# doubleailes/crust-render

Measured on AMD Instinct MI355X. Metric: Mray/s (closest-hit + shadow queries) of the path-tracing integrator, higher is better.
Workload: dtype f32; 1 GPU; samples/cornellbox.usda 1920x1080, 512 spp per step per GPU-share (x1 GPUs), depth 32, triangle r=1, variance 0; 14 steps = 7168 spp; rays_total=33550217735, closest_hit=33550217735, camera_rays=14863564800, target_spp=1024

## Files before the change

crust-render_amd/__init__.py:

```python
import ctypes as C
import os
import subprocess

import numpy as np

_HERE = os.path.dirname(os.path.abspath(__file__))
LIB_PATH = os.environ.get("CRT_AMD_LIB") or os.path.join(_HERE, "libcrt_amd.so")
CSRC = os.path.join(_HERE, "csrc")

MASK_CAMERA, MASK_SHADOW, MASK_INDIRECT, MASK_ALL = 1, 2, 4, 0xFFFFFFFF
INVALID_ID = 0xFFFFFFFF
INF = float("inf")

CRT_OK = 0
_ERRORS = {-1: "CRT_ERR_BAD_ARG", -2: "CRT_ERR_BAD_ID", -3: "CRT_ERR_NO_DEVICE", -4: "CRT_ERR_STACK",
           -5: "CRT_ERR_UNSUPPORTED", -6: "CRT_ERR_NO_MEMORY"}


class CrtError(RuntimeError):
    def __init__(self, code, what=""):
        detail = ""
        try:
            detail = _lib.crt_last_error().decode() if _lib is not None else ""
        except Exception:
            pass
        super().__init__(f"{what}: {_ERRORS.get(code, code)}" + (f" [{detail}]" if detail else ""))
        self.code = code


def build_native(force=False):
    if force:
        subprocess.check_call(["make", "-C", CSRC, "clean"], stdout=subprocess.DEVNULL)
    subprocess.check_call(["make", "-C", CSRC, "-j8", "-s"])
    return LIB_PATH


class CrtRay(C.Structure):
    _fields_ = [("origin", C.c_float * 3), ("_pad0", C.c_float), ("dir", C.c_float * 3), ("_pad1", C.c_float),
                ("time", C.c_float), ("mask", C.c_uint32), ("_pad2", C.c_uint32 * 2)]


class CrtRayHit(C.Structure):
    _fields_ = [("t", C.c_float), ("normal", C.c_float * 3), ("front_face", C.c_uint32), ("u", C.c_float),
                ("v", C.c_float), ("geom_id", C.c_uint32), ("prim_id", C.c_uint32), ("_pad", C.c_uint32)]


class CrtTravStats(C.Structure):
    _fields_ = [("queries", C.c_uint64 * 2), ("nodes", C.c_uint64 * 2), ("leaves", C.c_uint64 * 2),
                ("packets", C.c_uint64 * 2), ("prims", C.c_uint64 * 2), ("accepted_hits", C.c_uint64),
                ("instance_descents", C.c_uint64), ("rays", C.c_uint64),
                ("phase_waves", C.c_uint64 * 8), ("phase_lanes", C.c_uint64 * 8),
                ("phase_cycles", C.c_uint64 * 8)]

    PHASES = ("loop", "fetch+setup", "node", "packet", "scalar prim", "instance exit", "emit", "f64 fallback")

    def utilisation(self):
        return {n: (int(self.phase_waves[k]), (self.phase_lanes[k] / (64.0 * self.phase_waves[k])) if self.phase_waves[k] else 0.0)
                for k, n in enumerate(self.PHASES)}

    def as_dict(self):
        d = {k: [int(getattr(self, k)[0]), int(getattr(self, k)[1])] for k in ("queries", "nodes", "leaves", "packets",
                                                                                "prims")}
        d.update(accepted_hits=int(self.accepted_hits), instance_descents=int(self.instance_descents),
                 rays=int(self.rays))
        return d

    def algorithmic_bytes(self):
        n = sum
        return (80 * int(self.rays) + 128 * n(self.nodes) + 16 * n(self.leaves) + 192 * n(self.packets) +
                128 * int(self.accepted_hits) + 112 * int(self.instance_descents))


_MAT_FIELDS = [
    ("kind", C.c_uint32), ("thin_walled", C.c_uint32),
    ("base_weight", C.c_float), ("base_color", C.c_float * 3), ("base_diffuse_roughness", C.c_float),
    ("base_metalness", C.c_float),
    ("specular_weight", C.c_float), ("specular_color", C.c_float * 3), ("specular_roughness", C.c_float),
    ("specular_ior", C.c_float), ("specular_roughness_anisotropy", C.c_float),
    ("transmission_weight", C.c_float), ("transmission_color", C.c_float * 3), ("transmission_depth", C.c_float),
    ("transmission_scatter", C.c_float * 3), ("transmission_scatter_anisotropy", C.c_float),
    ("transmission_dispersion_scale", C.c_float), ("transmission_dispersion_abbe_number", C.c_float),
    ("subsurface_weight", C.c_float), ("subsurface_color", C.c_float * 3), ("subsurface_radius", C.c_float),
    ("subsurface_radius_scale", C.c_float * 3), ("subsurface_scatter_anisotropy", C.c_float),
    ("fuzz_weight", C.c_float), ("fuzz_color", C.c_float * 3), ("fuzz_roughness", C.c_float),
    ("coat_weight", C.c_float), ("coat_color", C.c_float * 3), ("coat_roughness", C.c_float),
    ("coat_roughness_anisotropy", C.c_float), ("coat_ior", C.c_float), ("coat_darkening", C.c_float),
    ("thin_film_weight", C.c_float), ("thin_film_thickness", C.c_float), ("thin_film_ior", C.c_float),
    ("emission_luminance", C.c_float), ("emission_color", C.c_float * 3),
    ("geometry_opacity", C.c_float),
]


class CrtMaterial(C.Structure):
    _fields_ = _MAT_FIELDS


MAT_OPENPBR, MAT_EMISSIVE = 0, 1
LIGHT_SPHERE, LIGHT_RECT, LIGHT_DISTANT, LIGHT_DOME = 0, 1, 2, 3
STRATEGY = {"power": 0, "mis": 0, "balance": 1, "light": 2, "bsdf": 3}
FILTER = {"box": 0, "triangle": 1}


class CrtLight(C.Structure):
    _fields_ = [("kind", C.c_uint32), ("geom_id", C.c_uint32), ("radiance", C.c_float * 3),
                ("center", C.c_float * 3), ("radius", C.c_float), ("origin", C.c_float * 3),
                ("edge_u", C.c_float * 3), ("edge_v", C.c_float * 3), ("normal", C.c_float * 3)]


class CrtCamera(C.Structure):
    _fields_ = [("origin", C.c_float * 3), ("lower_left", C.c_float * 3), ("horizontal", C.c_float * 3),
                ("vertical", C.c_float * 3), ("u", C.c_float * 3), ("v", C.c_float * 3), ("lens_radius", C.c_float)]


class CrtRenderSettings(C.Structure):
    _fields_ = [("width", C.c_uint32), ("height", C.c_uint32), ("max_depth", C.c_uint32), ("frame", C.c_int32),
                ("strategy", C.c_int32), ("filter_kind", C.c_int32), ("filter_radius", C.c_float),
                ("variance_threshold", C.c_float), ("min_spp", C.c_uint32)]


class CrtRayStats(C.Structure):
    _fields_ = [(n, C.c_uint64) for n in ("camera_rays", "closest_hit", "shadow_rays", "vertices", "rr_tested",
                                          "rr_killed", "ended_escaped", "ended_depth")]

    def total_rays(self):
        return int(self.closest_hit) + int(self.shadow_rays)

    def as_dict(self):
        return {n: int(getattr(self, n)) for n, _ in self._fields_}


ABI_SYMBOLS = [
    "crt_builder_new", "crt_builder_free", "crt_reserve", "crt_count", "crt_attach_triangles", "crt_attach_sphere",
    "crt_attach_instance", "crt_attach_empty", "crt_set_triangles", "crt_set_sphere", "crt_set_instance", "crt_commit",
    "crt_scene_retain", "crt_scene_release", "crt_scene_bounds", "crt_scene_geometry_count", "crt_scene_has_motion",
    "crt_scene_primitive_count", "crt_scene_primitive_breakdown", "crt_scene_unique_primitive_breakdown", "crt_scene_memory_footprint", "crt_scene_tree",
    "crt_shard_pixels", "crt_intersect1", "crt_occluded1", "crt_intersect_n", "crt_occluded_n", "crt_intersect_n_stats",
    "crt_occluded_n_stats", "crt_material_default", "crt_camera_new", "crt_renderer_new", "crt_renderer_free",
    "crt_renderer_pixel_count", "crt_renderer_pixel_indices", "crt_render_samples", "crt_film_resolve",
    "crt_film_read", "crt_film_clear", "crt_renderer_active_pixels", "crt_renderer_sample_counts", "crt_render_stats", "crt_renderer_profile", "crt_renderer_profile_read",
    "crt_render_samples_stats", "crt_version", "crt_last_error", "crt_device_info",
    "crt_scene_primitive_extents", "crt_scene_traversal_error", "crt_thread_release", "crt_renderer_shade_class_stats", "crt_renderer_pipeline", "crt_renderer_lanes", "crt_scene_image_check",
    "crt_scene_engine_select",
    "crt_material_scatter_n", "crt_material_eval_n", "crt_material_emitted_n", "crt_light_sample_n", "crt_light_pdf_n",
    "crt_light_escaped_n",
    "crt_shard_padded_count", "crt_gather_plan_new", "crt_gather_plan_free", "crt_gather_plan_padded_count",
    "crt_gather_plan_assemble", "crt_renderer_set_lanes",
]

_lib = None


def lib():
    global _lib
    if _lib is not None:
        return _lib
    if not os.path.exists(LIB_PATH):
        raise RuntimeError(f"{LIB_PATH} is missing: run __graft_entry__.build() (hipcc, gfx950). "
                           "crust-render_amd has no CPU fallback.")
    import torch
    L = C.CDLL(LIB_PATH)
    fp, up, vp = C.POINTER(C.c_float), C.POINTER(C.c_uint32), C.c_void_p
    L.crt_version.restype = C.c_char_p
    L.crt_last_error.restype = C.c_char_p
    L.crt_device_info.argtypes = [C.c_char_p, C.c_size_t, C.POINTER(C.c_int), C.POINTER(C.c_size_t)]
    L.crt_builder_new.restype = vp
    L.crt_builder_free.argtypes = [vp]
    L.crt_reserve.argtypes = [vp, C.c_size_t]
    L.crt_count.restype = C.c_size_t
    L.crt_count.argtypes = [vp]
    L.crt_attach_triangles.argtypes = [vp, fp, C.c_size_t, up, C.c_size_t, fp, C.c_size_t, C.c_uint32, up]
    L.crt_attach_sphere.argtypes = [vp, fp, C.c_float, C.c_uint32, up]
    L.crt_attach_instance.argtypes = [vp, vp, fp, fp, C.c_uint32, up]
    L.crt_attach_empty.argtypes = [vp, C.c_uint32, up]
    L.crt_set_triangles.argtypes = [vp, C.c_uint32, fp, C.c_size_t, up, C.c_size_t, fp, C.c_size_t]
    L.crt_set_sphere.argtypes = [vp, C.c_uint32, fp, C.c_float]
    L.crt_set_instance.argtypes = [vp, C.c_uint32, vp, fp, fp]
    L.crt_commit.restype = vp
    L.crt_commit.argtypes = [vp]
    L.crt_scene_retain.argtypes = [vp]
    L.crt_scene_release.argtypes = [vp]
    L.crt_scene_bounds.argtypes = [vp, fp]
    L.crt_scene_geometry_count.restype = C.c_uint32
    L.crt_scene_geometry_count.argtypes = [vp]
    L.crt_scene_has_motion.argtypes = [vp]
    L.crt_scene_primitive_count.restype = C.c_size_t
    L.crt_scene_primitive_count.argtypes = [vp]
    L.crt_scene_primitive_breakdown.argtypes = [vp, C.POINTER(C.c_size_t)]
    L.crt_scene_primitive_extents.argtypes = [vp, C.POINTER(C.c_size_t), fp, fp, fp]
    L.crt_scene_traversal_error.argtypes = [vp, vp]
    L.crt_thread_release.restype = None
    L.crt_scene_unique_primitive_breakdown.argtypes = [vp, C.POINTER(C.c_size_t)]
    L.crt_scene_memory_footprint.argtypes = [vp, C.POINTER(C.c_size_t)]
    if hasattr(L, "crt_scene_image_check"):
        L.crt_scene_image_check.argtypes = [vp, C.POINTER(C.c_uint64)]
    if hasattr(L, "crt_scene_engine_select"):
        L.crt_scene_engine_select.argtypes = [vp, C.c_int, C.POINTER(C.c_uint32)]
    L.crt_scene_tree.argtypes = [vp, C.POINTER(C.c_size_t), C.POINTER(vp), C.POINTER(vp), C.POINTER(vp),
                                 C.POINTER(up)]
    L.crt_intersect1.argtypes = [vp, C.POINTER(CrtRay), C.c_float, C.c_float, C.POINTER(CrtRayHit)]
    L.crt_occluded1.argtypes = [vp, C.POINTER(CrtRay), C.c_float, C.c_float]
    L.crt_intersect_n.argtypes = [vp, vp, C.c_size_t, C.c_float, C.c_float, vp, vp]
    L.crt_occluded_n.argtypes = [vp, vp, C.c_size_t, C.c_float, C.c_float, vp, vp]
    L.crt_intersect_n_stats.argtypes = [vp, vp, C.c_size_t, C.c_float, C.c_float, vp, vp, C.POINTER(CrtTravStats)]
    L.crt_occluded_n_stats.argtypes = [vp, vp, C.c_size_t, C.c_float, C.c_float, vp, vp, C.POINTER(CrtTravStats)]
    L.crt_material_default.argtypes = [C.POINTER(CrtMaterial)]
    L.crt_shard_pixels.restype = C.c_size_t
    L.crt_shard_pixels.argtypes = [C.c_uint32, C.c_uint32, C.c_uint32, C.c_uint32, up]
    if hasattr(L, "crt_renderer_new"):
        L.crt_camera_new.argtypes = [C.POINTER(CrtCamera), fp, fp, fp, C.c_float, C.c_float, C.c_float, C.c_float]
        L.crt_renderer_new.restype = vp
        L.crt_renderer_new.argtypes = [vp, C.POINTER(CrtMaterial), C.c_size_t, C.POINTER(CrtLight), C.c_size_t,
                                       C.POINTER(CrtCamera), C.POINTER(CrtRenderSettings), C.c_uint32, C.c_uint32]
        L.crt_renderer_free.argtypes = [vp]
        L.crt_renderer_pixel_count.restype = C.c_size_t
        L.crt_renderer_pixel_count.argtypes = [vp]
        L.crt_renderer_pixel_indices.argtypes = [vp, up]
        L.crt_render_samples.argtypes = [vp, C.c_uint32, C.c_uint32, vp]
        L.crt_film_resolve.argtypes = [vp, vp, vp]
        L.crt_film_read.argtypes = [vp, fp]
        L.crt_film_clear.argtypes = [vp, vp]
        L.crt_render_stats.argtypes = [vp, C.POINTER(CrtRayStats)]
        L.crt_renderer_active_pixels.restype = C.c_size_t
        L.crt_renderer_active_pixels.argtypes = [vp]
        L.crt_renderer_sample_counts.argtypes = [vp, up]
        L.crt_renderer_profile.argtypes = [vp, C.c_int]
        if hasattr(L, "crt_renderer_lanes"):
            L.crt_renderer_lanes.argtypes = [vp]
            L.crt_renderer_lanes.restype = C.c_int
        if hasattr(L, "crt_renderer_set_lanes"):
            L.crt_renderer_set_lanes.argtypes = [vp, C.c_int]
        if hasattr(L, "crt_renderer_pipeline"):
            L.crt_renderer_pipeline.argtypes = [vp, C.POINTER(C.c_uint32)]
        if hasattr(L, "crt_renderer_shade_class_stats"):
            L.crt_renderer_shade_class_stats.argtypes = [vp, C.c_int, C.POINTER(C.c_uint64), C.POINTER(C.c_uint64)]
        L.crt_renderer_profile_read.argtypes = [vp, C.POINTER(C.c_double), C.POINTER(C.c_uint64)]
        L.crt_render_samples_stats.argtypes = [vp, C.c_uint32, C.c_uint32, vp, C.POINTER(CrtTravStats)]
    if hasattr(L, "crt_gather_plan_new"):
        L.crt_shard_padded_count.restype = C.c_size_t
        L.crt_shard_padded_count.argtypes = [C.c_uint32, C.c_uint32, C.c_uint32]
        L.crt_gather_plan_new.restype = vp
        L.crt_gather_plan_new.argtypes = [C.c_uint32, C.c_uint32, C.c_uint32]
        L.crt_gather_plan_free.argtypes = [vp]
        L.crt_gather_plan_padded_count.restype = C.c_size_t
        L.crt_gather_plan_padded_count.argtypes = [vp]
        L.crt_gather_plan_assemble.argtypes = [vp, vp, vp, vp]
    for name in ("crt_material_scatter_n", "crt_material_eval_n", "crt_material_emitted_n", "crt_light_sample_n",
                 "crt_light_pdf_n", "crt_light_escaped_n"):
        if hasattr(L, name):
            getattr(L, name).argtypes = [vp, C.c_size_t, vp, C.c_size_t, vp, vp]
    _lib = L
    return L


def _check(rc, what):
    if rc < 0:
        raise CrtError(rc, what)
    return rc


def _fp(a):
    return a.ctypes.data_as(C.POINTER(C.c_float)) if a is not None else None


def _up(a):
    return a.ctypes.data_as(C.POINTER(C.c_uint32)) if a is not None else None


IDENTITY12 = np.array([1, 0, 0, 0, 1, 0, 0, 0, 1, 0, 0, 0], dtype=np.float32)


def affine(m3=None, t=(0, 0, 0)):
    m = np.eye(3, dtype=np.float32) if m3 is None else np.asarray(m3, dtype=np.float32)
    return np.concatenate([m[:, 0], m[:, 1], m[:, 2], np.asarray(t, dtype=np.float32)]).astype(np.float32)


class Ray:

    def __init__(self, origin, dir, time=0.0, mask=MASK_ALL):
        self.origin, self.dir, self.time, self.mask = origin, dir, time, mask

    def c(self):
        r = CrtRay()
        r.origin[:] = [float(x) for x in self.origin]
        r.dir[:] = [float(x) for x in self.dir]
        r.time = self.time
        r.mask = self.mask
        return r


RAY_DTYPE = np.dtype([("origin", np.float32, 3), ("_p0", np.float32), ("dir", np.float32, 3), ("_p1", np.float32),
                      ("time", np.float32), ("mask", np.uint32), ("_p2", np.uint32, 2)])
HIT_DTYPE = np.dtype([("t", np.float32), ("normal", np.float32, 3), ("front_face", np.uint32), ("u", np.float32),
                      ("v", np.float32), ("geom_id", np.uint32), ("prim_id", np.uint32), ("_pad", np.uint32)])
assert RAY_DTYPE.itemsize == 48 and HIT_DTYPE.itemsize == 40


def pack_rays(rays8):
    rays8 = np.ascontiguousarray(rays8, dtype=np.float32).reshape(-1, 8)
    out = np.zeros(rays8.shape[0], dtype=RAY_DTYPE)
    out["origin"] = rays8[:, 0:3]
    out["dir"] = rays8[:, 3:6]
    out["time"] = rays8[:, 6]
    out["mask"] = rays8[:, 7].view(np.uint32)
    return out


class Scene:

    def __init__(self, handle, keep=()):
        if not handle:
            raise RuntimeError("crt_commit failed: " + lib().crt_last_error().decode())
        self.h = handle
        self._keep = list(keep)

    def __del__(self):
        try:
            if self.h:
                lib().crt_scene_release(self.h)
        except Exception:
            pass

    def intersect(self, ray, t_min, t_max):
        h = CrtRayHit()
        rc = _check(lib().crt_intersect1(self.h, C.byref(ray.c()), t_min, t_max, C.byref(h)), "crt_intersect1")
        return h if rc == 1 else None

    def occluded(self, ray, t_min, t_max):
        return _check(lib().crt_occluded1(self.h, C.byref(ray.c()), t_min, t_max), "crt_occluded1") == 1

    def bounds(self):
        out = np.zeros(6, dtype=np.float32)
        return out if _check(lib().crt_scene_bounds(self.h, _fp(out)), "crt_scene_bounds") == 1 else None

    def geometry_count(self):
        return lib().crt_scene_geometry_count(self.h)

    def has_motion(self):
        return bool(lib().crt_scene_has_motion(self.h))

    def primitive_count(self):
        return lib().crt_scene_primitive_count(self.h)

    def primitive_breakdown(self):
        out = (C.c_size_t * 5)()
        _check(lib().crt_scene_primitive_breakdown(self.h, out), "crt_scene_primitive_breakdown")
        return dict(zip(("triangles", "spheres", "curve_segments", "cubic_curve_spans", "instances"), map(int, out)))

    def primitive_extents(self):
        n, d, mean, mx = C.c_size_t(), C.c_float(), C.c_float(), C.c_float()
        _check(lib().crt_scene_primitive_extents(self.h, C.byref(n), C.byref(d), C.byref(mean), C.byref(mx)),
               "crt_scene_primitive_extents")
        return n.value, d.value, mean.value, mx.value

    def traversal_error(self, stream=None):
        _check(lib().crt_scene_traversal_error(self.h, _stream_ptr(stream)), "crt_scene_traversal_error")

    def unique_primitive_breakdown(self):
        out = (C.c_size_t * 5)()
        _check(lib().crt_scene_unique_primitive_breakdown(self.h, out), "crt_scene_unique_primitive_breakdown")
        return dict(zip(("triangles", "spheres", "curve_segments", "cubic_curve_spans", "instances"), map(int, out)))

    def image_check(self):
        out = (C.c_uint64 * 8)()
        _check(lib().crt_scene_image_check(self.h, out), "crt_scene_image_check")
        return dict(zip(("nodes", "leaf_words_plain", "leaf_words_direct_index", "leaf_words_direct_instance", "instances",
                         "moving_instances", "staged_roots", "direct_leaves"), map(int, out)))

    def engine_select(self, want_wide=-1):
        out = (C.c_uint32 * 8)()
        _check(lib().crt_scene_engine_select(self.h, int(want_wide), out), "crt_scene_engine_select")
        return dict(zip(("wide", "direct", "lds_stack", "window", "ext_cold", "path_cold", "direct_words", "cold"),
                        map(int, out)))

    def memory_footprint(self):
        out = (C.c_size_t * 6)()
        _check(lib().crt_scene_memory_footprint(self.h, out), "crt_scene_memory_footprint")
        return dict(zip(("prim_nodes", "boxed_prims", "bvh_nodes", "leaves", "packets", "indices"), map(int, out)))

    def tree(self):
        counts = (C.c_size_t * 5)()
        pn, pl, pp = C.c_void_p(), C.c_void_p(), C.c_void_p()
        pi = C.POINTER(C.c_uint32)()
        _check(lib().crt_scene_tree(self.h, counts, C.byref(pn), C.byref(pl), C.byref(pp), C.byref(pi)),
               "crt_scene_tree")

        def grab(ptr, n, words):
            if n == 0:
                return np.zeros((0, words), dtype=np.uint32)
            buf = C.cast(ptr, C.POINTER(C.c_uint32 * (n * words))).contents
            return np.frombuffer(buf, dtype=np.uint32).reshape(n, words).copy()

        return (grab(pn, counts[0], 32), grab(pl, counts[1], 4), grab(pp, counts[2], 48),
                grab(pi, counts[3], 1).reshape(-1), dict(nodes=counts[0], leaves=counts[1], packets=counts[2],
                                                         indices=counts[3], prims=counts[4]))

    def intersect_n(self, d_rays, t_min, t_max, d_hits=None, stream=None, stats=None):
        import torch
        n = d_rays.numel() * d_rays.element_size() // 48
        if d_hits is None:
            d_hits = torch.empty(n * 40, dtype=torch.uint8, device=d_rays.device)
        sp = _stream_ptr(stream)
        if stats is None:
            _check(lib().crt_intersect_n(self.h, d_rays.data_ptr(), n, t_min, t_max, d_hits.data_ptr(), sp),
                   "crt_intersect_n")
        else:
            _check(lib().crt_intersect_n_stats(self.h, d_rays.data_ptr(), n, t_min, t_max, d_hits.data_ptr(), sp,
                                               C.byref(stats)), "crt_intersect_n_stats")
        return d_hits

    def occluded_n(self, d_rays, t_min, t_max, d_out=None, stream=None, stats=None):
        import torch
        n = d_rays.numel() * d_rays.element_size() // 48
        if d_out is None:
            d_out = torch.empty(n, dtype=torch.int32, device=d_rays.device)
        sp = _stream_ptr(stream)
        if stats is None:
            _check(lib().crt_occluded_n(self.h, d_rays.data_ptr(), n, t_min, t_max, d_out.data_ptr(), sp),
                   "crt_occluded_n")
        else:
            _check(lib().crt_occluded_n_stats(self.h, d_rays.data_ptr(), n, t_min, t_max, d_out.data_ptr(), sp,
                                              C.byref(stats)), "crt_occluded_n_stats")
        return d_out


def _stream_ptr(stream):
    if stream is None:
        import torch
        return C.c_void_p(torch.cuda.current_stream().cuda_stream)
    if isinstance(stream, int):
        return C.c_void_p(stream)
    return C.c_void_p(stream.cuda_stream)


def rays_to_device(rays8, device="cuda:0"):
    import torch
    rec = pack_rays(rays8)
    return torch.from_numpy(rec.view(np.uint8).reshape(-1)).to(device)


def hits_to_host(d_hits):
    return d_hits.cpu().numpy().view(HIT_DTYPE)


class SceneBuilder:

    def __init__(self):
        self.h = lib().crt_builder_new()
        self._keep = []

    def __del__(self):
        try:
            if self.h:
                lib().crt_builder_free(self.h)
        except Exception:
            pass

    def reserve(self, additional):
        _check(lib().crt_reserve(self.h, additional), "crt_reserve")

    def count(self):
        return lib().crt_count(self.h)

    @staticmethod
    def _mesh(verts, idx, normals):
        verts = np.ascontiguousarray(verts, dtype=np.float32).reshape(-1, 3)
        idx = np.ascontiguousarray(idx, dtype=np.uint32).reshape(-1, 3)
        nrm = None if normals is None else np.ascontiguousarray(normals, dtype=np.float32).reshape(-1, 3)
        return verts, idx, nrm

    def attach_triangles(self, verts, idx, normals=None, mask=MASK_ALL):
        v, i, n = self._mesh(verts, idx, normals)
        gid = C.c_uint32()
        _check(lib().crt_attach_triangles(self.h, _fp(v), v.shape[0], _up(i), i.shape[0], _fp(n),
                                          0 if n is None else n.shape[0], mask, C.byref(gid)), "crt_attach_triangles")
        return gid.value

    def attach_sphere(self, center, radius, mask=MASK_ALL):
        c = np.asarray(center, dtype=np.float32)
        gid = C.c_uint32()
        _check(lib().crt_attach_sphere(self.h, _fp(c), radius, mask, C.byref(gid)), "crt_attach_sphere")
        return gid.value

    def attach_instance(self, scene, l2w=IDENTITY12, l2w_end=None, mask=MASK_ALL):
        a = np.ascontiguousarray(l2w, dtype=np.float32)
        e = None if l2w_end is None else np.ascontiguousarray(l2w_end, dtype=np.float32)
        gid = C.c_uint32()
        _check(lib().crt_attach_instance(self.h, scene.h, _fp(a), _fp(e), mask, C.byref(gid)), "crt_attach_instance")
        self._keep.append(scene)
        return gid.value

    def attach_empty(self, mask=MASK_ALL):
        gid = C.c_uint32()
        _check(lib().crt_attach_empty(self.h, mask, C.byref(gid)), "crt_attach_empty")
        return gid.value

    def set_triangles(self, gid, verts, idx, normals=None):
        v, i, n = self._mesh(verts, idx, normals)
        _check(lib().crt_set_triangles(self.h, gid, _fp(v), v.shape[0], _up(i), i.shape[0], _fp(n),
                                       0 if n is None else n.shape[0]), "crt_set_triangles")

    def set_sphere(self, gid, center, radius):
        c = np.asarray(center, dtype=np.float32)
        _check(lib().crt_set_sphere(self.h, gid, _fp(c), radius), "crt_set_sphere")

    def set_instance(self, gid, scene, l2w=IDENTITY12, l2w_end=None):
        a = np.ascontiguousarray(l2w, dtype=np.float32)
        e = None if l2w_end is None else np.ascontiguousarray(l2w_end, dtype=np.float32)
        _check(lib().crt_set_instance(self.h, gid, scene.h, _fp(a), _fp(e)), "crt_set_instance")
        self._keep.append(scene)

    def commit(self):
        h, self.h = self.h, None
        return Scene(lib().crt_commit(h), self._keep)


def default_material():
    m = CrtMaterial()
    lib().crt_material_default(C.byref(m))
    return m


def diffuse_material(rgb):
    m = default_material()
    m.base_color[:] = [float(x) for x in rgb]
    m.specular_weight = 0.0
    return m


def emissive_material(rgb):
    m = default_material()
    m.kind = MAT_EMISSIVE
    m.emission_color[:] = [float(x) for x in rgb]
    m.emission_luminance = 1.0
    return m


class RenderSettings:

    def __init__(self, width, height, max_depth=32, frame=0, strategy="power", pixel_filter="triangle",
                 filter_radius=None, variance_threshold=0.0, min_spp=32):
        self.width, self.height, self.max_depth, self.frame = int(width), int(height), int(max_depth), int(frame)
        self.strategy, self.pixel_filter = strategy, pixel_filter
        self.filter_radius = filter_radius if filter_radius is not None else (0.5 if pixel_filter == "box" else 1.0)
        self.variance_threshold = variance_threshold
        self.min_spp = int(min_spp)

    def c(self):
        return CrtRenderSettings(self.width, self.height, self.max_depth, self.frame, STRATEGY[self.strategy],
                                 FILTER[self.pixel_filter], float(self.filter_radius), float(self.variance_threshold),
                                 self.min_spp)


def make_camera(lookfrom, lookat, vup, vfov_deg, aspect, aperture, focus_dist):
    c = CrtCamera()
    a = [np.asarray(x, dtype=np.float32) for x in (lookfrom, lookat, vup)]
    lib().crt_camera_new(C.byref(c), _fp(a[0]), _fp(a[1]), _fp(a[2]), float(vfov_deg), float(aspect), float(aperture),
                         float(focus_dist))
    return c


def make_lights(light_dicts):
    arr = (CrtLight * max(len(light_dicts), 1))()
    for k, d in enumerate(light_dicts):
        l = arr[k]
        l.kind = {"sphere": LIGHT_SPHERE, "rect": LIGHT_RECT, "distant": LIGHT_DISTANT,
                  "dome": LIGHT_DOME}[d["kind"]]
        l.geom_id = int(d["geom_id"])
        l.radiance[:] = [float(x) for x in d["radiance"]]
        if d["kind"] == "distant":
            l.normal[:] = [float(x) for x in d["direction"]]
            l.radius = float(d["cos_half_angle"])
            l.center[0] = float(d["solid_angle"])
        elif d["kind"] == "dome":
            pass
        elif d["kind"] == "sphere":
            l.center[:] = [float(x) for x in d["center"]]
            l.radius = float(d["radius"])
        else:
            for f in ("origin", "edge_u", "edge_v", "normal"):
                getattr(l, f)[:] = [float(x) for x in d[f]]
    return arr


class Renderer:

    def __init__(self, scene, materials, lights, camera, settings, rank=0, world=1):
        self.scene = scene
        n = len(materials)
        self._mats = (CrtMaterial * max(n, 1))(*materials)
        self._lights = lights if not isinstance(lights, (list, tuple)) else make_lights(lights)
        self.n_lights = len(lights)
        self.settings = settings
        cs = settings.c()
        self.h = lib().crt_renderer_new(scene.h, self._mats, n, self._lights, self.n_lights, C.byref(camera),
                                        C.byref(cs), rank, world)
        if not self.h:
            raise CrtError(-1, "crt_renderer_new")
        self.n_pix = lib().crt_renderer_pixel_count(self.h)

    def __del__(self):
        try:
            if self.h:
                lib().crt_renderer_free(self.h)
        except Exception:
            pass

    def pixel_indices(self):
        out = np.zeros(self.n_pix, dtype=np.uint32)
        _check(lib().crt_renderer_pixel_indices(self.h, _up(out)), "crt_renderer_pixel_indices")
        return out

    def render_samples(self, sample_begin, sample_count, stream=None):
        _check(lib().crt_render_samples(self.h, sample_begin, sample_count, _stream_ptr(stream)), "crt_render_samples")

    def render_samples_stats(self, sample_begin, sample_count, stream=None):
        st = (CrtTravStats * 2)()
        _check(lib().crt_render_samples_stats(self.h, sample_begin, sample_count, _stream_ptr(stream), st),
               "crt_render_samples_stats")
        return st[0], st[1]

    def film_to(self, d_rgb, stream=None):
        _check(lib().crt_film_resolve(self.h, d_rgb.data_ptr(), _stream_ptr(stream)), "crt_film_resolve")

    def film(self):
        out = np.zeros((self.n_pix, 3), dtype=np.float32)
        _check(lib().crt_film_read(self.h, _fp(out)), "crt_film_read")
        return out

    def image(self):
        img = np.zeros((self.settings.height * self.settings.width, 3), dtype=np.float32)
        img[self.pixel_indices()] = self.film()
        return img.reshape(self.settings.height, self.settings.width, 3)

    def clear(self, stream=None):
        _check(lib().crt_film_clear(self.h, _stream_ptr(stream)), "crt_film_clear")

    def stats(self):
        s = CrtRayStats()
        _check(lib().crt_render_stats(self.h, C.byref(s)), "crt_render_stats")
        return s

    def active_pixels(self):
        return int(lib().crt_renderer_active_pixels(self.h))

    def sample_counts(self):
        out = np.zeros(self.n_pix, dtype=np.uint32)
        _check(lib().crt_renderer_sample_counts(self.h, out.ctypes.data_as(C.POINTER(C.c_uint32))), "crt_renderer_sample_counts")
        return out

    def render_adaptive(self, spp, first=None, batch=4, stream=None):
        first = first or -(-max(self.settings.min_spp, 2) // 4) * 4
        s = 0
        while s < spp and self.active_pixels() > 0:
            n = min(first if s == 0 else batch, spp - s)
            self.render_samples(s, n, stream)
            s += n
        return s

    SHADE_CLASSES = ("emissive / escaped", "base", "coat / fuzz / thin film", "transmissive / subsurface")

    def shade_class_stats(self, enable=None):
        w, l = (C.c_uint64 * 4)(), (C.c_uint64 * 4)()
        _check(lib().crt_renderer_shade_class_stats(self.h, -1 if enable is None else int(bool(enable)), w, l),
               "crt_renderer_shade_class_stats")
        return {n: (int(w[k]), (l[k] / (64.0 * w[k])) if w[k] else 0.0) for k, n in enumerate(self.SHADE_CLASSES)}

    def pipeline(self):
        out = (C.c_uint32 * 3)()
        _check(lib().crt_renderer_pipeline(self.h, out), "crt_renderer_pipeline")
        return dict(fused=bool(out[0]), wide=bool(out[1]), grid=int(out[2]))

    def lanes(self):
        return int(lib().crt_renderer_lanes(self.h)) if hasattr(lib(), "crt_renderer_lanes") else 1

    def set_lanes(self, lanes):
        return _check(lib().crt_renderer_set_lanes(self.h, int(lanes)), "crt_renderer_set_lanes")

    def profile(self, enable=True):
        _check(lib().crt_renderer_profile(self.h, 1 if enable else 0), "crt_renderer_profile")

    def profile_read(self):
        ms = (C.c_double * 4)()
        n = (C.c_uint64 * 4)()
        _check(lib().crt_renderer_profile_read(self.h, ms, n), "crt_renderer_profile_read")
        names = ("extend", "shade", "shadow", "other")
        return {names[k]: dict(ms=float(ms[k]), launches=int(n[k])) for k in range(4)}


def scene_path(name):
    import os
    if str(name).startswith("synthetic:") or os.path.exists(name):
        return name
    base = os.path.join(os.path.dirname(os.path.dirname(os.path.abspath(__file__))), "scenes", name)
    for ext in (".usda", ".usd", ".usda.xz"):
        if os.path.exists(base + ext):
            return base + ext
    raise FileNotFoundError("no scene %r under scenes/" % name)


def load_usda(path, width=None, height=None, max_depth=None, rank=0, world=1, variance=0.0, min_spp=None, dist=None,
              timings=None):
    from . import usda, shard
    import sys
    import time
    t0 = time.perf_counter()
    if str(path).startswith("synthetic:"):
        from . import synthetic
        parts = str(path).split(":")
        kw = dict(side=int(parts[2])) if len(parts) > 2 else {}
        desc = getattr(synthetic, parts[1])(width or 640, height or 360, **kw)
    else:
        desc = shard.import_once(path, width, height, dist)
    me = sys.modules[__name__]
    t1 = time.perf_counter()
    scene, materials, protos = usda.build_world(desc, me, default_material)
    t2 = time.perf_counter()
    if timings is not None:
        timings.update(import_s=t1 - t0, commit_s=t2 - t1)
    s = desc.settings
    settings = RenderSettings(s["width"], s["height"], s["max_depth"] if max_depth is None else max_depth, s["frame"],
                              s["strategy"], s["filter"], s["filter_radius"], float(variance),
                              s["min_spp"] if min_spp is None else min_spp)
    cam = make_camera(**desc.camera)
    r = Renderer(scene, materials, desc.lights, cam, settings, rank, world)
    r._protos = protos
    return r, desc

def render_with_report(path, spp=None, out_exr=None, width=None, height=None, max_depth=None, variance=None,
                       batch=16):
    import sys
    from . import stats as _stats
    st = _stats.RenderStats()
    me = sys.modules[__name__]
    with st.phase("Parse USD stage"):
        desc = usda.load(path, width, height)
    s = desc.settings
    with st.phase("Commit acceleration structure"):
        scene, materials, protos = usda.build_world(desc, me, default_material)
        scene.memory_footprint()
    var = s["variance"] if variance is None else variance
    settings = RenderSettings(s["width"], s["height"], s["max_depth"] if max_depth is None else max_depth, s["frame"],
                              s["strategy"], s["filter"], s["filter_radius"], float(var), s["min_spp"])
    r = Renderer(scene, materials, desc.lights, make_camera(**desc.camera), settings)
    r._protos = protos
    n = int(spp if spp is not None else s["spp"])
    with st.phase("Render"):
        if var > 0:
            r.render_adaptive(n, batch=batch)
        else:
            for b in range(0, n, 32):
                r.render_samples(b, min(32, n - b))
        img = r.image()
    if out_exr:
        with st.phase("Write image"):
            exr.write_exr(out_exr, img[::-1])
    _stats.for_render(scene, r, n, st)
    return img, st


load_scene = load_usda

from . import usda
from . import usdc
from . import shard
from . import exr
from . import stats
from . import shading
from . import synthetic
```

crust-render_amd/csrc/capi.cpp:

```cpp
#include <hip/hip_runtime.h>

#include <cmath>
#include <cstring>
#include <exception>
#include <new>
#include <stdexcept>
#include <unordered_set>

#include "crt_internal.h"

namespace crt {
const char *last_error_text();
}

using namespace crt;

namespace {

Affine affine_from12(const float m[12]) {
  return Affine{f3(m[0], m[1], m[2]), f3(m[3], m[4], m[5]), f3(m[6], m[7], m[8]), f3(m[9], m[10], m[11])};
}

void fill_mesh(Geom &g, const float *verts, size_t n_verts, const uint32_t *indices, size_t n_tris, const float *normals,
               size_t n_normals) {
  g.kind = G_MESH;
  g.verts.assign(verts, verts + (verts ? 3 * n_verts : 0));
  g.idx.assign(indices, indices + (indices ? 3 * n_tris : 0));
  g.has_normals = normals != nullptr;
  g.normals.clear();
  if (normals) g.normals.assign(normals, normals + 3 * n_normals);
  g.scene.reset();
}
void fill_sphere(Geom &g, const float c[3], float r) {
  g = Geom{G_SPHERE, g.mask};
  g.center = f3(c[0], c[1], c[2]);
  g.radius = r;
}
void fill_instance(Geom &g, CrtScene *scene, const float l2w[12], const float *l2w_end) {
  g = Geom{G_INSTANCE, g.mask};
  g.scene = scene->p;
  g.l2w = affine_from12(l2w);
  g.has_end = l2w_end != nullptr;
  if (l2w_end) g.l2w_end = affine_from12(l2w_end);
}

}

extern "C" {

const char *crt_version(void) { return "crt_amd 0.1 (gfx950)"; }
const char *crt_last_error(void) { return crt::last_error_text(); }

int crt_device_info(char *name_out, size_t name_cap, int *cu_count, size_t *hbm_bytes) {
  if (!device_ok()) return CRT_ERR_NO_DEVICE;
  hipDeviceProp_t prop;
  int dev = 0;
  if (hipGetDevice(&dev) != hipSuccess || hipGetDeviceProperties(&prop, dev) != hipSuccess) return CRT_ERR_NO_DEVICE;
  if (name_out && name_cap) {
    std::strncpy(name_out, prop.gcnArchName, name_cap - 1);
    name_out[name_cap - 1] = 0;
  }
  if (cu_count) *cu_count = prop.multiProcessorCount;
  if (hbm_bytes) *hbm_bytes = prop.totalGlobalMem;
  return CRT_OK;
}

CrtBuilder *crt_builder_new(void) { return new (std::nothrow) CrtBuilder(); }
void crt_builder_free(CrtBuilder *b) { delete b; }
int crt_reserve(CrtBuilder *b, size_t additional) {
  if (!b) return CRT_ERR_BAD_ARG;
  return abi_guard("crt_reserve", [&] {
    if (additional > b->b.geoms.max_size() - b->b.geoms.size()) throw std::length_error("capacity overflow");
    b->b.geoms.reserve(b->b.geoms.size() + additional);
    return (int)CRT_OK;
  });
}
size_t crt_count(const CrtBuilder *b) { return b ? b->b.geoms.size() : 0; }

int crt_attach_triangles(CrtBuilder *b, const float *verts, size_t n_verts, const uint32_t *indices, size_t n_tris,
                         const float *normals, size_t n_normals, uint32_t mask, uint32_t *geom_id_out) {
  if (!b || (n_verts && !verts) || (n_tris && !indices)) return CRT_ERR_BAD_ARG;
  return abi_guard("crt_attach_triangles", [&] {
    Geom g;
    g.mask = mask;
    fill_mesh(g, verts, n_verts, indices, n_tris, normals, n_normals);
    b->b.geoms.push_back(std::move(g));
    if (geom_id_out) *geom_id_out = uint32_t(b->b.geoms.size() - 1);
    return (int)CRT_OK;
  });
}
int crt_attach_sphere(CrtBuilder *b, const float center[3], float radius, uint32_t mask, uint32_t *geom_id_out) {
  if (!b || !center) return CRT_ERR_BAD_ARG;
  return abi_guard("crt_attach_sphere", [&] {
    Geom g;
    g.mask = mask;
    fill_sphere(g, center, radius);
    b->b.geoms.push_back(std::move(g));
    if (geom_id_out) *geom_id_out = uint32_t(b->b.geoms.size() - 1);
    return (int)CRT_OK;
  });
}
int crt_attach_instance(CrtBuilder *b, CrtScene *scene, const float l2w[12], const float *l2w_end, uint32_t mask,
                        uint32_t *geom_id_out) {
  if (!b || !scene || !l2w) return CRT_ERR_BAD_ARG;
  return abi_guard("crt_attach_instance", [&] {
    Geom g;
    g.mask = mask;
    fill_instance(g, scene, l2w, l2w_end);
    b->b.geoms.push_back(std::move(g));
    if (geom_id_out) *geom_id_out = uint32_t(b->b.geoms.size() - 1);
    return (int)CRT_OK;
  });
}
int crt_attach_empty(CrtBuilder *b, uint32_t mask, uint32_t *geom_id_out) {
  return crt_attach_triangles(b, nullptr, 0, nullptr, 0, nullptr, 0, mask, geom_id_out);
}
int crt_set_triangles(CrtBuilder *b, uint32_t id, const float *verts, size_t n_verts, const uint32_t *indices,
                      size_t n_tris, const float *normals, size_t n_normals) {
  if (!b || (n_verts && !verts) || (n_tris && !indices)) return CRT_ERR_BAD_ARG;
  if (id >= b->b.geoms.size()) return CRT_ERR_BAD_ID;
  return abi_guard("crt_set_triangles", [&] {
    Geom g;
    g.mask = b->b.geoms[id].mask;
    fill_mesh(g, verts, n_verts, indices, n_tris, normals, n_normals);
    b->b.geoms[id] = std::move(g);
    return (int)CRT_OK;
  });
}
int crt_set_sphere(CrtBuilder *b, uint32_t id, const float center[3], float radius) {
  if (!b || !center) return CRT_ERR_BAD_ARG;
  if (id >= b->b.geoms.size()) return CRT_ERR_BAD_ID;
  fill_sphere(b->b.geoms[id], center, radius);
  return CRT_OK;
}
int crt_set_instance(CrtBuilder *b, uint32_t id, CrtScene *scene, const float l2w[12], const float *l2w_end) {
  if (!b || !scene || !l2w) return CRT_ERR_BAD_ARG;
  if (id >= b->b.geoms.size()) return CRT_ERR_BAD_ID;
  fill_instance(b->b.geoms[id], scene, l2w, l2w_end);
  return CRT_OK;
}

CrtScene *crt_commit(CrtBuilder *b) {
  if (!b) return nullptr;
  CrtScene *s = nullptr;
  try {
    s = new CrtScene();
    s->p = commit(std::move(b->b));
    if (!s->p) { delete s; s = nullptr; }
  } catch (const std::exception &e) {
    set_error_text("commit: %s", e.what());
    delete s;
    s = nullptr;
  } catch (...) {
    set_error_text("commit: unknown failure");
    delete s;
    s = nullptr;
  }
  delete b;
  return s;
}

void crt_scene_retain(CrtScene *s) {
  if (s) s->refs.fetch_add(1);
}
void crt_scene_release(CrtScene *s) {
  if (s && s->refs.fetch_sub(1) == 1) delete s;
}

int crt_scene_bounds(const CrtScene *s, float out[6]) {
  if (!s || !out) return CRT_ERR_BAD_ARG;
  const Bvh &b = s->p->bvh;
  if (!b.has_bbox) return 0;
  out[0] = b.root_bbox.mn.x; out[1] = b.root_bbox.mn.y; out[2] = b.root_bbox.mn.z;
  out[3] = b.root_bbox.mx.x; out[4] = b.root_bbox.mx.y; out[5] = b.root_bbox.mx.z;
  return 1;
}
uint32_t crt_scene_geometry_count(const CrtScene *s) { return s ? s->p->n_geoms : 0; }
int crt_scene_has_motion(const CrtScene *s) { return s ? (s->p->has_motion ? 1 : 0) : 0; }
size_t crt_scene_primitive_count(const CrtScene *s) { return s ? s->p->bvh.prims.size() : 0; }
int crt_scene_primitive_extents(const CrtScene *s, size_t *count, float *scene_diagonal, float *mean_diagonal,
                                float *max_diagonal) {
  if (!s) return CRT_ERR_BAD_ARG;
  const Bvh &b = s->p->bvh;
  auto length = [](F3 v) { return std::sqrt((v.x * v.x + v.y * v.y) + v.z * v.z); };
  float sum = 0.0f, mx = 0.0f;
  for (const Prim &p : b.prims) {
    const Aabb bb = prim_bbox(p);
    const float d = length(bb.mx - bb.mn);
    sum += d;
    mx = d > mx ? d : mx;
  }
  const size_t n = b.prims.size();
  if (count) *count = n;
  if (scene_diagonal) *scene_diagonal = b.has_bbox ? length(b.root_bbox.mx - b.root_bbox.mn) : 0.0f;
  if (mean_diagonal) *mean_diagonal = n == 0 ? 0.0f : sum / float(n);
  if (max_diagonal) *max_diagonal = mx;
  return CRT_OK;
}
int crt_scene_primitive_breakdown(const CrtScene *s, size_t out[5]) {
  if (!s || !out) return CRT_ERR_BAD_ARG;
  out[0] = out[1] = out[2] = out[3] = out[4] = 0;
  for (const Prim &p : s->p->bvh.prims) {
    if (p.kind == PRIM_TRI) out[0]++;
    else if (p.kind == PRIM_SPHERE) out[1]++;
    else out[4]++;
  }
  return CRT_OK;
}
namespace {
void accumulate_unique(const Scene &sc, std::unordered_set<const Scene *> &visited, size_t acc[5]) {
  for (const Prim &p : sc.bvh.prims) {
    if (p.kind == PRIM_TRI) acc[0]++;
    else if (p.kind == PRIM_SPHERE) acc[1]++;
    else {
      acc[4]++;
      if (visited.insert(p.scene.get()).second) accumulate_unique(*p.scene, visited, acc);
    }
  }
}
}
int crt_scene_unique_primitive_breakdown(const CrtScene *s, size_t out[5]) {
  if (!s || !out) return CRT_ERR_BAD_ARG;
  out[0] = out[1] = out[2] = out[3] = out[4] = 0;
  std::unordered_set<const Scene *> visited;
  accumulate_unique(*s->p, visited, out);
  return CRT_OK;
}
int crt_scene_image_check(CrtScene *s, uint64_t out[8]) {
  if (!s || !out) return CRT_ERR_BAD_ARG;
  try {
    return scene_image_check(*s->p, out);
  } catch (const std::exception &e) {
    set_error_text("crt_scene_image_check: %s", e.what());
    return CRT_ERR_BAD_ARG;
  }
}
int crt_scene_engine_select(CrtScene *s, int want_wide, uint32_t out[8]) {
  if (!s || !out) return CRT_ERR_BAD_ARG;
  try {
    return scene_engine_select(*s->p, want_wide, out);
  } catch (const std::exception &e) {
    set_error_text("crt_scene_engine_select: %s", e.what());
    return CRT_ERR_BAD_ARG;
  }
}
int crt_scene_memory_footprint(CrtScene *s, size_t out[6]) {
  if (!s || !out) return CRT_ERR_BAD_ARG;
  int rc = s->p->ensure_device();
  if (rc != CRT_OK) return rc;
  const DeviceImage &d = *s->p->dev;
  out[0] = d.bytes[4];
  out[1] = d.bytes[5] + d.bytes[6];
  out[2] = d.bytes[0];
  out[3] = d.bytes[1];
  out[4] = d.bytes[2];
  out[5] = d.bytes[3];
  return CRT_OK;
}
int crt_scene_tree(const CrtScene *s, size_t counts[5], const void **nodes128, const void **leaves16,
                   const void **packets192, const uint32_t **indices) {
  if (!s || !counts) return CRT_ERR_BAD_ARG;
  const Bvh &b = s->p->bvh;
  counts[0] = b.wide.size(); counts[1] = b.leaves.size(); counts[2] = b.packets.size();
  counts[3] = b.indices.size(); counts[4] = b.prims.size();
  if (nodes128) *nodes128 = b.wide.data();
  if (leaves16) *leaves16 = b.leaves.data();
  if (packets192) *packets192 = b.packets.data();
  if (indices) *indices = b.indices.data();
  return CRT_OK;
}

int crt_intersect_n(CrtScene *s, const CrtRay *d_rays, size_t n, float t_min, float t_max, CrtRayHit *d_hits,
                    void *stream) {
  if (!s || (n && (!d_rays || !d_hits))) return CRT_ERR_BAD_ARG;
  int rc = s->p->ensure_device();
  if (rc != CRT_OK) return rc;
  return launch_intersect_n(s->p->dev->view, d_rays, n, t_min, t_max, d_hits, stream, nullptr, s->p->dev->err);
}
int crt_occluded_n(CrtScene *s, const CrtRay *d_rays, size_t n, float t_min, float t_max, uint32_t *d_out,
                   void *stream) {
  if (!s || (n && (!d_rays || !d_out))) return CRT_ERR_BAD_ARG;
  int rc = s->p->ensure_device();
  if (rc != CRT_OK) return rc;
  return launch_occluded_n(s->p->dev->view, d_rays, n, t_min, t_max, d_out, stream, nullptr, s->p->dev->err);
}

static int take_error_word(uint32_t *d_err, void *stream) {
  uint32_t h = 0;
  if (hipMemcpyAsync(&h, d_err, sizeof h, hipMemcpyDeviceToHost, (hipStream_t)stream) != hipSuccess) return CRT_ERR_NO_DEVICE;
  if (hipStreamSynchronize((hipStream_t)stream) != hipSuccess) return CRT_ERR_NO_DEVICE;
  if (!h) return CRT_OK;
  (void)hipMemsetAsync(d_err, 0, sizeof h, (hipStream_t)stream);
  set_error_text("traversal error word 0x%x (1 = stack overflow, 2 = instance nesting)", h);
  return CRT_ERR_STACK;
}

int crt_scene_traversal_error(CrtScene *s, void *stream) {
  if (!s) return CRT_ERR_BAD_ARG;
  if (!s->p->dev) return CRT_OK;
  return take_error_word(s->p->dev->err, stream);
}

static int with_stats(CrtScene *s, void *stream, CrtTravStats *host_stats,
                      int (*launch)(const DevScene &, void *, CrtTravStats *, uint32_t *, void *), void *ctx) {
  int rc = s->p->ensure_device();
  if (rc != CRT_OK) return rc;
  CrtTravStats *d = nullptr;
  if (hipMalloc(&d, sizeof(CrtTravStats)) != hipSuccess) return CRT_ERR_NO_DEVICE;
  (void)hipMemsetAsync(d, 0, sizeof(CrtTravStats), (hipStream_t)stream);
  rc = launch(s->p->dev->view, stream, d, s->p->dev->err, ctx);
  CrtTravStats h;
  if (rc == CRT_OK && hipMemcpyAsync(&h, d, sizeof h, hipMemcpyDeviceToHost, (hipStream_t)stream) != hipSuccess)
    rc = CRT_ERR_NO_DEVICE;
  if (hipStreamSynchronize((hipStream_t)stream) != hipSuccess) rc = CRT_ERR_NO_DEVICE;
  (void)hipFree(d);
  if (rc == CRT_OK) rc = take_error_word(s->p->dev->err, stream);
  if (rc == CRT_OK && host_stats) {
    for (int k = 0; k < 2; k++) {
      host_stats->queries[k] += h.queries[k]; host_stats->nodes[k] += h.nodes[k];
      host_stats->leaves[k] += h.leaves[k]; host_stats->packets[k] += h.packets[k];
      host_stats->prims[k] += h.prims[k];
    }
    host_stats->accepted_hits += h.accepted_hits;
    host_stats->instance_descents += h.instance_descents;
    host_stats->rays += h.rays;
    for (int k = 0; k < 8; k++) { host_stats->phase_waves[k] += h.phase_waves[k]; host_stats->phase_lanes[k] += h.phase_lanes[k]; host_stats->phase_cycles[k] += h.phase_cycles[k]; }
  }
  return rc;
}

struct NArgs { const CrtRay *rays; size_t n; float t_min, t_max; void *out; };

int crt_intersect_n_stats(CrtScene *s, const CrtRay *d_rays, size_t n, float t_min, float t_max, CrtRayHit *d_hits,
                          void *stream, CrtTravStats *host_stats) {
  if (!s || (n && (!d_rays || !d_hits))) return CRT_ERR_BAD_ARG;
  NArgs a{d_rays, n, t_min, t_max, d_hits};
  return with_stats(
      s, stream, host_stats,
      [](const DevScene &v, void *st, CrtTravStats *d, uint32_t *e, void *c) {
        NArgs *a = static_cast<NArgs *>(c);
        return launch_intersect_n(v, a->rays, a->n, a->t_min, a->t_max, static_cast<CrtRayHit *>(a->out), st, d, e);
      },
      &a);
}
int crt_occluded_n_stats(CrtScene *s, const CrtRay *d_rays, size_t n, float t_min, float t_max, uint32_t *d_out,
                         void *stream, CrtTravStats *host_stats) {
  if (!s || (n && (!d_rays || !d_out))) return CRT_ERR_BAD_ARG;
  NArgs a{d_rays, n, t_min, t_max, d_out};
  return with_stats(
      s, stream, host_stats,
      [](const DevScene &v, void *st, CrtTravStats *d, uint32_t *e, void *c) {
        NArgs *a = static_cast<NArgs *>(c);
        return launch_occluded_n(v, a->rays, a->n, a->t_min, a->t_max, static_cast<uint32_t *>(a->out), st, d, e);
      },
      &a);
}

}
namespace {
struct Staging {
  struct Rec { CrtRay ray; CrtRayHit hit; uint32_t occ; uint32_t err; };
  Rec *host = nullptr;
  Rec *dev = nullptr;
  hipStream_t stream = nullptr;
  int device = -1;
  bool ok() const { return host && dev && stream; }
  void release() {
    if (stream) (void)hipStreamDestroy(stream);
    if (dev) (void)hipFree(dev);
    if (host) (void)hipHostFree(host);
    host = nullptr; dev = nullptr; stream = nullptr; device = -1;
  }
  bool acquire() {
    int cur = 0;
    if (hipGetDevice(&cur) != hipSuccess) return false;
    if (ok() && device == cur) return true;
    release();
    if (!CRT_HIP_OK(hipHostMalloc(reinterpret_cast<void **>(&host), sizeof(Rec), hipHostMallocDefault)) ||
        !CRT_HIP_OK(hipMalloc(reinterpret_cast<void **>(&dev), sizeof(Rec))) ||
        !CRT_HIP_OK(hipStreamCreateWithFlags(&stream, hipStreamNonBlocking)) ||
        !CRT_HIP_OK(hipMemsetAsync(dev, 0, sizeof(Rec), stream))) {
      release();
      return false;
    }
    device = cur;
    return true;
  }
};
thread_local Staging t_staging;

template <bool ANY>
int query1(CrtScene *s, const CrtRay *ray, float t_min, float t_max, CrtRayHit *hit) {
  int rc = s->p->ensure_device();
  if (rc != CRT_OK) return rc;
  Staging &g = t_staging;
  if (!g.acquire()) return CRT_ERR_NO_DEVICE;
  g.host->ray = *ray;
  if (!CRT_HIP_OK(hipMemcpyAsync(&g.dev->ray, &g.host->ray, sizeof(CrtRay), hipMemcpyHostToDevice, g.stream)))
    return CRT_ERR_NO_DEVICE;
  rc = ANY ? launch_occluded_n(s->p->dev->view, &g.dev->ray, 1, t_min, t_max, &g.dev->occ, g.stream, nullptr, &g.dev->err)
           : launch_intersect_n(s->p->dev->view, &g.dev->ray, 1, t_min, t_max, &g.dev->hit, g.stream, nullptr, &g.dev->err);
  if (rc != CRT_OK) return rc;
  if (!CRT_HIP_OK(hipMemcpyAsync(&g.host->hit, &g.dev->hit, sizeof(CrtRayHit) + 2 * sizeof(uint32_t), hipMemcpyDeviceToHost,
                                 g.stream)) ||
      !CRT_HIP_OK(hipStreamSynchronize(g.stream)))
    return CRT_ERR_NO_DEVICE;
  if (g.host->err) {
    (void)hipMemsetAsync(&g.dev->err, 0, sizeof(uint32_t), g.stream);
    set_error_text("traversal error word 0x%x (1 = stack overflow, 2 = instance nesting)", g.host->err);
    return CRT_ERR_STACK;
  }
  if (ANY) return g.host->occ ? 1 : 0;
  *hit = g.host->hit;
  return hit->geom_id != CRT_INVALID_ID ? 1 : 0;
}
}
extern "C" {

int crt_intersect1(CrtScene *s, const CrtRay *ray, float t_min, float t_max, CrtRayHit *hit) {
  if (!s || !ray || !hit) return CRT_ERR_BAD_ARG;
  return query1<false>(s, ray, t_min, t_max, hit);
}
int crt_occluded1(CrtScene *s, const CrtRay *ray, float t_min, float t_max) {
  if (!s || !ray) return CRT_ERR_BAD_ARG;
  return query1<true>(s, ray, t_min, t_max, nullptr);
}
void crt_thread_release(void) { t_staging.release(); }

size_t crt_shard_pixels(uint32_t width, uint32_t height, uint32_t rank, uint32_t world, uint32_t *out) {
  if (world == 0 || rank >= world) return 0;
  const uint32_t tx = (width + 15) / 16, ty = (height + 15) / 16;
  size_t n = 0;
  for (uint32_t t = 0; t < tx * ty; t++) {
    if (t % world != rank) continue;
    const uint32_t x0 = (t % tx) * 16, y0 = (t / tx) * 16;
    for (uint32_t y = y0; y < y0 + 16 && y < height; y++)
      for (uint32_t x = x0; x < x0 + 16 && x < width; x++) {
        if (out) out[n] = y * width + x;
        n++;
      }
  }
  return n;
}

void crt_material_default(CrtMaterial *m) {
  if (!m) return;
  std::memset(m, 0, sizeof *m);
  m->kind = CRT_MAT_OPENPBR;
  m->base_weight = 1.0f;
  m->base_color[0] = m->base_color[1] = m->base_color[2] = 0.8f;
  m->specular_weight = 1.0f;
  m->specular_color[0] = m->specular_color[1] = m->specular_color[2] = 1.0f;
  m->specular_roughness = 0.3f;
  m->specular_ior = 1.5f;
  m->transmission_color[0] = m->transmission_color[1] = m->transmission_color[2] = 1.0f;
  m->transmission_dispersion_abbe_number = 20.0f;
  m->subsurface_color[0] = m->subsurface_color[1] = m->subsurface_color[2] = 0.8f;
  m->subsurface_radius = 1.0f;
  m->subsurface_radius_scale[0] = 1.0f; m->subsurface_radius_scale[1] = 0.5f; m->subsurface_radius_scale[2] = 0.25f;
  m->fuzz_color[0] = m->fuzz_color[1] = m->fuzz_color[2] = 1.0f;
  m->fuzz_roughness = 0.5f;
  m->coat_color[0] = m->coat_color[1] = m->coat_color[2] = 1.0f;
  m->coat_ior = 1.6f;
  m->coat_darkening = 1.0f;
  m->thin_film_thickness = 0.5f;
  m->thin_film_ior = 1.4f;
  m->emission_color[0] = m->emission_color[1] = m->emission_color[2] = 1.0f;
  m->geometry_opacity = 1.0f;
}

}
```

crust-render_amd/csrc/crt_internal.h:

```cpp
#pragma once

#include <atomic>
#include <cstddef>
#include <cstdint>
#include <memory>
#include <mutex>
#include <vector>

#include "../../include/crt.h"

namespace crt {

struct F3 {
  float x, y, z;
  float operator[](int i) const { return i == 0 ? x : (i == 1 ? y : z); }
  float &at(int i) { return i == 0 ? x : (i == 1 ? y : z); }
};
inline F3 f3(float x, float y, float z) { return F3{x, y, z}; }
inline F3 operator+(F3 a, F3 b) { return {a.x + b.x, a.y + b.y, a.z + b.z}; }
inline F3 operator-(F3 a, F3 b) { return {a.x - b.x, a.y - b.y, a.z - b.z}; }
inline F3 operator*(F3 a, float s) { return {a.x * s, a.y * s, a.z * s}; }
inline F3 operator-(F3 a) { return {-a.x, -a.y, -a.z}; }
inline float sse_min(float a, float b) { return a < b ? a : b; }
inline float sse_max(float a, float b) { return a > b ? a : b; }
inline F3 vmin(F3 a, F3 b) { return {sse_min(a.x, b.x), sse_min(a.y, b.y), sse_min(a.z, b.z)}; }
inline F3 vmax(F3 a, F3 b) { return {sse_max(a.x, b.x), sse_max(a.y, b.y), sse_max(a.z, b.z)}; }
inline float dot(F3 a, F3 b) { return (a.x * b.x + a.y * b.y) + a.z * b.z; }
inline F3 cross(F3 a, F3 b) { return {a.y * b.z - b.y * a.z, a.z * b.x - b.z * a.x, a.x * b.y - b.x * a.y}; }

struct Aabb { F3 mn, mx; };
struct Affine { F3 x, y, z, t; };
struct Mat3 { F3 x, y, z; };

Affine affine_inverse(const Affine &a);
Mat3 mat3_transpose(const Mat3 &m);
F3 affine_point(const Affine &a, F3 p);
F3 affine_vector(const Affine &a, F3 p);
Aabb transformed_aabb(const Aabb &local, const Affine &m);

struct alignas(16) WideNode {
  float bmin[3][4];
  float bmax[3][4];
  uint32_t child[4];
  uint32_t flags;
  uint32_t pad[3];
};
static_assert(sizeof(WideNode) == 128, "bvh.rs:1613-1616");

struct Leaf { uint32_t pkt_first, pkt_count, idx_first, idx_count; };
static_assert(sizeof(Leaf) == 16, "bvh.rs:220-227");

struct alignas(16) Tri4 {
  float v[3][3][4];
  uint32_t prim[4];
  uint32_t active, mask_and, mask_or;
  uint32_t masks[4];
  uint32_t normal_ok;
};
static_assert(sizeof(Tri4) == 192, "triangle.rs:182-196");

enum PrimKind : uint32_t { PRIM_TRI = 0, PRIM_SPHERE = 1, PRIM_INSTANCE = 2 };

struct Scene;

struct Prim {
  PrimKind kind;
  uint32_t geom_id, prim_id, mask;
  F3 v0, v1, v2;
  bool has_normals;
  F3 n0, n1, n2;
  F3 center;
  float radius;
  std::shared_ptr<Scene> scene;
  Affine l2w, w2l;
  Mat3 normal_mat;
  bool has_end;
  Affine l2w_end;
  Aabb bounds;
};

struct Bvh {
  std::vector<WideNode> wide;
  std::vector<Leaf> leaves;
  std::vector<Tri4> packets;
  std::vector<uint32_t> indices;
  std::vector<Prim> prims;
  bool has_bbox = false;
  Aabb root_bbox{};
};

constexpr uint32_t kMaxInstanceLevels = 8;

Aabb prim_bbox(const Prim &p);
void build_bvh(Bvh &out, std::vector<Prim> &&prims);

struct DevPrim {
  uint32_t kind, geom_id, prim_id, mask;
  float d[12];
};
static_assert(sizeof(DevPrim) == 64, "");

struct DevInstance {
  float w2l[12];
  uint32_t root;
  uint32_t flags;
  uint32_t geom_id;
  uint32_t mask;
};
static_assert(sizeof(DevInstance) == 64, "");
struct DevInstanceMotion {
  float l2w[12];
  float l2w_end[12];
};
constexpr uint32_t kIndexInstance = 0x80000000u;

struct DevScene {
  const WideNode *nodes;
  const Leaf *leaves;
  const Tri4 *packets;
  const uint32_t *indices;
  const DevPrim *prims;
  const DevInstance *instances;
  const float *normals;
  uint32_t root;
  uint32_t has_packets;
  uint32_t n_nodes;
  uint32_t pool_stack;
  uint32_t n_packets;
  uint32_t direct_leaves;
  uint32_t cold;
};
enum : uint32_t { kColdUV = 1u, kColdNormal = 2u, kColdTime = 4u, kColdAll = 7u };
constexpr uint32_t kNoPackets = 8u;
constexpr uint32_t kDirectLeafTag = 0x40000000u;
constexpr uint32_t kDirectInstTag = 0x08000000u;
constexpr uint32_t kDirectIndexMask = 0x07ffffffu;
#ifndef CRT_POOL_NODES_WIDE
#define CRT_POOL_NODES_WIDE 26
#endif
#ifndef CRT_POOL_NODES_WIDE_DEEP
#define CRT_POOL_NODES_WIDE_DEEP 12
#endif
#ifndef CRT_DIRECT_INST
#define CRT_DIRECT_INST 1
#endif
#ifndef CRT_POOL_NODES
#define CRT_POOL_NODES 72
#endif
#ifndef CRT_POOL_NODES_DEEP
#define CRT_POOL_NODES_DEEP 16
#endif
#ifndef CRT_WIDE_DIRECT_BUILD
#define CRT_WIDE_DIRECT_BUILD 1
#endif
#ifndef CRT_NOPK_BUILD
#define CRT_NOPK_BUILD 0
#endif
#ifndef CRT_DIRECT_LEAVES
#define CRT_DIRECT_LEAVES 1
#endif

inline bool wide_split(const DevScene &s, bool renderer = false) {
  if (s.direct_leaves != 0 || s.n_packets == 0) return false;
  if (s.pool_stack >= 10u) return renderer && s.n_nodes > 2048u;
  return s.n_nodes <= 1024u;
}

#ifndef CRT_POOL_STACK
#define CRT_POOL_STACK 6
#endif
#ifndef CRT_POOL_STACK_DEEP
#define CRT_POOL_STACK_DEEP 10
#endif
#ifndef CRT_POOL_STACK_WIDE
#define CRT_POOL_STACK_WIDE 3
#endif

struct EngineSelect {
  bool wide = false;
  bool wide_direct = false;
  bool direct = false;
  uint32_t lds_stack = CRT_POOL_STACK;
  uint32_t window = CRT_POOL_NODES;
  int ext_cold = (int)kColdAll;
  int path_cold = (int)kColdAll;
};
inline int select_engine(const DevScene &s, int want_wide, EngineSelect &e, bool renderer = false) {
  const bool has_direct_words = s.direct_leaves != 0;
  if (want_wide == 1 && has_direct_words) return CRT_ERR_UNSUPPORTED;
  if (want_wide == 2 && !(has_direct_words && renderer && CRT_DIRECT_LEAVES != 0 && CRT_WIDE_DIRECT_BUILD != 0)) return CRT_ERR_UNSUPPORTED;
  const bool auto_wide_direct = want_wide < 0 && renderer && has_direct_words && CRT_DIRECT_LEAVES != 0 && CRT_WIDE_DIRECT_BUILD != 0;
  e.wide = auto_wide_direct || (want_wide < 0 ? wide_split(s, renderer) : want_wide != 0);
  e.wide_direct = auto_wide_direct || want_wide == 2;
  e.direct = (!e.wide || e.wide_direct) && CRT_DIRECT_LEAVES != 0 && has_direct_words;
  if (has_direct_words && !e.direct) return CRT_ERR_UNSUPPORTED;
  const bool deep = s.pool_stack >= (uint32_t)CRT_POOL_STACK_DEEP;
  e.lds_stack = e.wide ? (uint32_t)CRT_POOL_STACK_WIDE + 1u + (deep ? 1u : 0u) : (deep ? (uint32_t)CRT_POOL_STACK_DEEP : (uint32_t)CRT_POOL_STACK);
  e.window = e.wide ? (deep ? (uint32_t)CRT_POOL_NODES_WIDE_DEEP : (uint32_t)CRT_POOL_NODES_WIDE)
                    : (deep ? (uint32_t)CRT_POOL_NODES_DEEP : (uint32_t)CRT_POOL_NODES);
  const int cold = (int)(s.cold & kColdAll);
  e.ext_cold = cold == 0 ? 0 : (cold == (int)kColdNormal ? (int)kColdNormal : (int)kColdAll);
  e.path_cold = cold == 0 ? 0 : (int)kColdAll;
  if (CRT_NOPK_BUILD && s.n_packets == 0 && e.direct) e.path_cold = (int)(kColdAll | kNoPackets);
  return CRT_OK;
}
inline bool engine_accepts(const EngineSelect &e, const DevScene &s, int kernel_cold) {
  if (s.direct_leaves != 0 && ((e.wide && !e.wide_direct) || !e.direct)) return false;
  if (e.wide_direct && s.direct_leaves == 0) return false;
  if ((kernel_cold & (int)kNoPackets) && (s.n_packets != 0 || s.direct_leaves == 0)) return false;
  return ((int)(s.cold & kColdAll) & ~kernel_cold) == 0;
}
int wide_request();

struct Knobs {
  int pool_stack_deep = -1;
  int direct_leaves = -1;
  int direct_inst = -1;
  int stage_roots = -1;
  uint32_t cold = 0;
  int inst_order = 1;
  int hot_packets = 1;
  int wide = -1;
  int mat_dedup = 1, partition = -1, simple = 1, prefer_stage = -1, cam_compact = 1, shade_wide = -1, fused = -1;
  int noclassify_from = 1 << 30, tail_from = 12, lanes = 4, grid_mult = 0;
  size_t max_batch_slots = 0, lane_min_paths = (size_t)96 << 20, stage_min_paths = (size_t)96 << 20;
};
Knobs read_knobs();
inline int select_engine_env(const DevScene &s, EngineSelect &e, bool renderer = false) {
  if (select_engine(s, wide_request(), e, renderer) == CRT_OK) return CRT_OK;
  return select_engine(s, -1, e, renderer);
}

struct DeviceImage {
  void *blob = nullptr;
  size_t bytes[7] = {0, 0, 0, 0, 0, 0, 0};
  uint32_t *err = nullptr;
  DevScene view{};
  ~DeviceImage();
};

struct Scene : std::enable_shared_from_this<Scene> {
  Bvh bvh;
  uint32_t n_geoms = 0;
  bool has_motion = false;
  uint32_t depth = 1;
  std::mutex dev_mu;
  std::unique_ptr<DeviceImage> dev;
  int ensure_device();
};

int scene_image_check(const Scene &scene, uint64_t out[8]);
int scene_engine_select(const Scene &scene, int want_wide, uint32_t out[8]);

enum GeomKind { G_MESH, G_SPHERE, G_INSTANCE };
struct Geom {
  GeomKind kind = G_MESH;
  uint32_t mask = CRT_MASK_ALL;
  std::vector<float> verts;
  std::vector<uint32_t> idx;
  bool has_normals = false;
  std::vector<float> normals;
  F3 center{0, 0, 0};
  float radius = 0;
  std::shared_ptr<Scene> scene;
  Affine l2w{};
  bool has_end = false;
  Affine l2w_end{};
};

struct Builder { std::vector<Geom> geoms; };

std::shared_ptr<Scene> commit(Builder &&b);

int launch_intersect_n(const DevScene &s, const CrtRay *d_rays, size_t n, float t_min, float t_max, CrtRayHit *d_hits,
                       void *stream, CrtTravStats *d_stats, uint32_t *d_err);
int launch_occluded_n(const DevScene &s, const CrtRay *d_rays, size_t n, float t_min, float t_max, uint32_t *d_out,
                      void *stream, CrtTravStats *d_stats, uint32_t *d_err);
int device_ok();
void set_error_text(const char *fmt, ...);
template <class F>
inline int abi_guard(const char *what, F &&body) noexcept {
  try { return body(); }
  catch (const std::exception &e) { set_error_text("%s: %s", what, e.what()); }
  catch (...) { set_error_text("%s: unknown failure", what); }
  return CRT_ERR_NO_MEMORY;
}

bool hip_failed(int  err, const char *what, const char *file, int line);
#define CRT_HIP_OK(call) (!::crt::hip_failed((int)(call), #call, __FILE__, __LINE__))

}

struct CrtScene { std::shared_ptr<crt::Scene> p; std::atomic<int> refs{1}; };
struct CrtBuilder { crt::Builder b; };
```

crust-render_amd/csrc/kernels/traverse.hip:

```cpp
#include <cstdlib>

#include "traverse_pool.hip.h"

static_assert(crt::dev::kMaxLevels == (int)crt::kMaxInstanceLevels, "commit's nesting limit is the kernels' frame count");

namespace crt {

using namespace dev;

namespace {

struct Chunk { size_t count; };
__device__ __forceinline__ Chunk my_chunk(size_t n) {
  const size_t blocks = (n + kBlock - 1) / kBlock, G = gridDim.x, b = blockIdx.x;
  if (b >= blocks) return Chunk{0};
  const size_t mine = (blocks - b + G - 1) / G;
  size_t count = mine * kBlock;
  if ((blocks - 1) % G == b) count -= blocks * kBlock - n;
  return Chunk{count};
}
__device__ __forceinline__ size_t dealt_ray(uint32_t k) {
  return ((size_t)(k / kBlock) * gridDim.x + blockIdx.x) * kBlock + (k % kBlock);
}
__device__ __forceinline__ bool lds_take(bool want, uint32_t *next, uint32_t limit, uint32_t &idx) {
  const unsigned long long mask = __ballot(want);
  if (mask == 0) return false;
  const int lane = threadIdx.x & 63;
  const int leader = __ffsll((long long)mask) - 1;
  uint32_t base = 0;
  if (lane == leader) base = atomicAdd(next, (uint32_t)__popcll(mask));
  base = __shfl(base, leader, 64);
  idx = base + (uint32_t)__popcll(mask & ((1ull << lane) - 1ull));
  return want && idx < limit;
}

template <bool STATS, bool WIDE>
__global__ __launch_bounds__(kBlock, WIDE ? 4 : 3) void intersect_n_kernel(DevScene S, const CrtRay *__restrict__ rays, size_t n,
                                                            float t_min, float t_max, CrtRayHit *__restrict__ hits,
                                                            uint32_t *__restrict__ err_out, CrtTravStats *stats) {
  __shared__ __attribute__((aligned(16))) uint32_t engine_lds[WIDE ? kEngineLdsWide : kEngineLdsDwords];
  __shared__ uint32_t next;
  const Chunk ck = my_chunk(n);
  if (ck.count == 0) return;
  if (threadIdx.x == 0) next = 0;
  LaneStats st = {};
  uint32_t err = 0, done = 0;
  auto fetch = [&](bool want, RayIn &in) -> bool {
    uint32_t k;
    if (!lds_take(want, &next, (uint32_t)ck.count, k)) return false;
    const float4 *rp = reinterpret_cast<const float4 *>(rays + dealt_ray(k));
    const float4 o = rp[0], d = rp[1], tm = rp[2];
    in.ox = o.x; in.oy = o.y; in.oz = o.z; in.dx = d.x; in.dy = d.y; in.dz = d.z;
    in.time = tm.x; in.mask = __float_as_uint(tm.y); in.t_min = t_min; in.t_max = t_max; in.slot = k;
    return true;
  };
  auto emit = [&](uint32_t k, bool hit, const Hit &h, float dx, float dy, float dz) {
    const size_t i = dealt_ray(k);
    CrtRayHit out;
    if (hit) {
      const bool front = dot3(dx, dy, dz, h.nx, h.ny, h.nz) < 0.0f;
      out.t = h.t;
      out.normal[0] = front ? h.nx : -h.nx;
      out.normal[1] = front ? h.ny : -h.ny;
      out.normal[2] = front ? h.nz : -h.nz;
      out.front_face = front ? 1u : 0u;
      out.u = h.u; out.v = h.v; out.geom_id = h.geom; out.prim_id = h.prim; out._pad = 0;
    } else {
      out.t = 0.0f; out.normal[0] = out.normal[1] = out.normal[2] = 0.0f; out.front_face = 0;
      out.u = out.v = 0.0f; out.geom_id = CRT_INVALID_ID; out.prim_id = CRT_INVALID_ID; out._pad = 0;
    }
    hits[i] = out;
    done++;
  };
  run_traversal<false, STATS, WIDE>(S, engine_lds, t_min, err, st, fetch, emit);
  if (err) atomicOr(err_out, err);
  if (STATS) flush_stats(st, stats, done);
}

template <bool STATS, bool WIDE>
__global__ __launch_bounds__(kBlock, WIDE ? 4 : 3) void occluded_n_kernel(DevScene S, const CrtRay *__restrict__ rays, size_t n,
                                                           float t_min, float t_max, uint32_t *__restrict__ out,
                                                           uint32_t *__restrict__ err_out, CrtTravStats *stats) {
  __shared__ __attribute__((aligned(16))) uint32_t engine_lds[WIDE ? kEngineLdsWide : kEngineLdsDwords];
  __shared__ uint32_t next;
  const Chunk ck = my_chunk(n);
  if (ck.count == 0) return;
  if (threadIdx.x == 0) next = 0;
  LaneStats st = {};
  uint32_t err = 0, done = 0;
  auto fetch = [&](bool want, RayIn &in) -> bool {
    uint32_t k;
    if (!lds_take(want, &next, (uint32_t)ck.count, k)) return false;
    const float4 *rp = reinterpret_cast<const float4 *>(rays + dealt_ray(k));
    const float4 o = rp[0], d = rp[1], tm = rp[2];
    in.ox = o.x; in.oy = o.y; in.oz = o.z; in.dx = d.x; in.dy = d.y; in.dz = d.z;
    in.time = tm.x; in.mask = __float_as_uint(tm.y); in.t_min = t_min; in.t_max = t_max; in.slot = k;
    return true;
  };
  auto emit = [&](uint32_t k, bool occ, const Hit &, float, float, float) {
    out[dealt_ray(k)] = occ ? 1u : 0u;
    done++;
  };
  run_traversal<true, STATS, WIDE>(S, engine_lds, t_min, err, st, fetch, emit);
  if (err) atomicOr(err_out, err);
  if (STATS) flush_stats(st, stats, done);
}

int query_engine(const DevScene &s, EngineSelect &e) {
  const int rc = select_engine_env(s, e);
  if (rc != CRT_OK) return rc;
  if (!engine_accepts(e, s, (int)kColdAll)) {
    set_error_text("traversal launch refused: the selected engine instance (wide %d, direct %d) cannot decode this image (direct words %u)",
                   (int)e.wide, (int)e.direct, s.direct_leaves);
    return CRT_ERR_UNSUPPORTED;
  }
  return CRT_OK;
}
int grid_for(size_t n, bool wide) {
  static int cus = [] {
    hipDeviceProp_t prop;
    int dev = 0;
    (void)hipGetDevice(&dev);
    if (!CRT_HIP_OK(hipGetDeviceProperties(&prop, dev))) return 256;
    return prop.multiProcessorCount > 0 ? prop.multiProcessorCount : 256;
  }();
  size_t need = (n + kBlock - 1) / kBlock;
  size_t cap = (size_t)cus * (wide ? 4 : 3);
  return (int)(need < cap ? (need ? need : 1) : cap);
}

}

int launch_intersect_n(const DevScene &s, const CrtRay *d_rays, size_t n, float t_min, float t_max, CrtRayHit *d_hits,
                       void *stream, CrtTravStats *d_stats, uint32_t *e) {
  if (n == 0) return CRT_OK;
  if (!e) return CRT_ERR_BAD_ARG;
  EngineSelect eng;
  if (const int rc = query_engine(s, eng)) return rc;
  const bool wide = eng.wide;
  const int grid = grid_for(n, wide);
#define CRT_LAUNCH(ST, W)                                                                                             \
  hipLaunchKernelGGL((intersect_n_kernel<ST, W>), dim3(grid), dim3(kBlock), 0, (hipStream_t)stream, s, d_rays, n, t_min, \
                     t_max, d_hits, e, d_stats)
  if (d_stats) { if (wide) CRT_LAUNCH(true, true); else CRT_LAUNCH(true, false); }
  else { if (wide) CRT_LAUNCH(false, true); else CRT_LAUNCH(false, false); }
#undef CRT_LAUNCH
  return CRT_HIP_OK(hipGetLastError()) ? CRT_OK : CRT_ERR_NO_DEVICE;
}

int launch_occluded_n(const DevScene &s, const CrtRay *d_rays, size_t n, float t_min, float t_max, uint32_t *d_out,
                      void *stream, CrtTravStats *d_stats, uint32_t *e) {
  if (n == 0) return CRT_OK;
  if (!e) return CRT_ERR_BAD_ARG;
  EngineSelect eng;
  if (const int rc = query_engine(s, eng)) return rc;
  const bool wide = eng.wide;
  const int grid = grid_for(n, wide);
#define CRT_LAUNCH(ST, W)                                                                                            \
  hipLaunchKernelGGL((occluded_n_kernel<ST, W>), dim3(grid), dim3(kBlock), 0, (hipStream_t)stream, s, d_rays, n, t_min, \
                     t_max, d_out, e, d_stats)
  if (d_stats) { if (wide) CRT_LAUNCH(true, true); else CRT_LAUNCH(true, false); }
  else { if (wide) CRT_LAUNCH(false, true); else CRT_LAUNCH(false, false); }
#undef CRT_LAUNCH
  return CRT_HIP_OK(hipGetLastError()) ? CRT_OK : CRT_ERR_NO_DEVICE;
}

}
```

crust-render_amd/csrc/kernels/traverse.hip.h:

```cpp
#pragma once

#include <hip/hip_runtime.h>

#include "../crt_internal.h"

namespace crt {
namespace dev {

constexpr int kBlock = 256;
#ifndef CRT_LDS_NODE_STRIDE
#define CRT_LDS_NODE_STRIDE 28
#endif
constexpr int kLdsNodeStride = CRT_LDS_NODE_STRIDE;
constexpr int kMaxLevels = 8;
constexpr uint32_t kLeafTag = 0x80000000u;
constexpr uint32_t kInvalid = 0xFFFFFFFFu;

struct Hit {
  float t, u, v;
  float nx, ny, nz;
  uint32_t geom, prim;
};

struct LaneStats {
  uint32_t queries[2], nodes[2], leaves[2], packets[2], prims[2];
  uint32_t accepted, descents;
  uint32_t ph_wave[8], ph_lane[8];
  unsigned long long ph_cyc[8];
};
#define CRT_PHASE(k)                                                        \
  if (STATS) {                                                              \
    const unsigned long long m_ = __ballot(1);                              \
    st.ph_lane[k]++;                                                        \
    if ((int)(threadIdx.x & 63) == __ffsll((long long)m_) - 1) st.ph_wave[k]++; \
  }

__device__ __forceinline__ void flush_stats(const LaneStats &st, CrtTravStats *out, uint32_t rays) {
  auto wave_sum = [](uint32_t v) {
    for (int off = 32; off > 0; off >>= 1) v += __shfl_down(v, off, 64);
    return v;
  };
  const bool lead = (threadIdx.x & 63) == 0;
  auto add = [&](uint64_t *dst, uint32_t v) {
    v = wave_sum(v);
    if (lead && v) atomicAdd((unsigned long long *)dst, (unsigned long long)v);
  };
  for (int k = 0; k < 2; k++) {
    add(&out->queries[k], st.queries[k]); add(&out->nodes[k], st.nodes[k]); add(&out->leaves[k], st.leaves[k]);
    add(&out->packets[k], st.packets[k]); add(&out->prims[k], st.prims[k]);
  }
  add(&out->accepted_hits, st.accepted); add(&out->instance_descents, st.descents); add(&out->rays, rays);
  for (int k = 0; k < 8; k++) { add(&out->phase_waves[k], st.ph_wave[k]); add(&out->phase_lanes[k], st.ph_lane[k]); }
  if (lead)
    for (int k = 0; k < 8; k++)
      if (st.ph_cyc[k]) atomicAdd((unsigned long long *)&out->phase_cycles[k], st.ph_cyc[k]);
}

__device__ __forceinline__ float absf(float x) { return __uint_as_float(__float_as_uint(x) & 0x7fffffffu); }
__device__ __forceinline__ float copysgn(float mag, float sgn) {
  return __uint_as_float((__float_as_uint(mag) & 0x7fffffffu) | (__float_as_uint(sgn) & 0x80000000u));
}
__device__ __forceinline__ float sel3(float x, float y, float z, int k) { return k == 0 ? x : (k == 1 ? y : z); }
__device__ __forceinline__ float dot3(float ax, float ay, float az, float bx, float by, float bz) {
  return (ax * bx + ay * by) + az * bz;
}

struct RayCtx {
  float ox, oy, oz, dx, dy, dz;
  float ix, iy, iz;
  int kx, ky, kz;
  float sx, sy, sz;
  float okx, oky, okz;
};

__device__ __forceinline__ void setup_ray(RayCtx &r, bool with_shear) {
  const float TINY = 1e-20f, HUGE_ = 1e20f;
  r.ix = absf(r.dx) < TINY ? copysgn(HUGE_, r.dx) : 1.0f / r.dx;
  r.iy = absf(r.dy) < TINY ? copysgn(HUGE_, r.dy) : 1.0f / r.dy;
  r.iz = absf(r.dz) < TINY ? copysgn(HUGE_, r.dz) : 1.0f / r.dz;
  if (with_shear) {
    const float ax = absf(r.dx), ay = absf(r.dy), az = absf(r.dz);
    int kz;
    if (ax > ay) kz = (ax > az) ? 0 : 2;
    else if (ay > az) kz = 1;
    else kz = 2;
    int kx = kz == 2 ? 0 : kz + 1;
    int ky = kx == 2 ? 0 : kx + 1;
    const float dkz = sel3(r.dx, r.dy, r.dz, kz);
    if (dkz < 0.0f) { int t = kx; kx = ky; ky = t; }
    r.kx = kx; r.ky = ky; r.kz = kz;
    r.sx = sel3(r.dx, r.dy, r.dz, kx) / dkz;
    r.sy = sel3(r.dx, r.dy, r.dz, ky) / dkz;
    r.sz = 1.0f / dkz;
    r.okx = sel3(r.ox, r.oy, r.oz, kx);
    r.oky = sel3(r.ox, r.oy, r.oz, ky);
    r.okz = sel3(r.ox, r.oy, r.oz, kz);
  }
}

__device__ __forceinline__ bool tri_scalar(const RayCtx &r, const float *v , float t_min, float t_max,
                                           float &to, float &uo, float &vo) {
  const float a0 = v[0] - r.ox, a1 = v[1] - r.oy, a2 = v[2] - r.oz;
  const float b0 = v[3] - r.ox, b1 = v[4] - r.oy, b2 = v[5] - r.oz;
  const float c0 = v[6] - r.ox, c1 = v[7] - r.oy, c2 = v[8] - r.oz;
  const float akx = sel3(a0, a1, a2, r.kx), aky = sel3(a0, a1, a2, r.ky), akz = sel3(a0, a1, a2, r.kz);
  const float bkx = sel3(b0, b1, b2, r.kx), bky = sel3(b0, b1, b2, r.ky), bkz = sel3(b0, b1, b2, r.kz);
  const float ckx = sel3(c0, c1, c2, r.kx), cky = sel3(c0, c1, c2, r.ky), ckz = sel3(c0, c1, c2, r.kz);
  const float ax = akx - r.sx * akz, ay = aky - r.sy * akz;
  const float bx = bkx - r.sx * bkz, by = bky - r.sy * bkz;
  const float cx = ckx - r.sx * ckz, cy = cky - r.sy * ckz;
  float e0 = bx * cy - by * cx;
  float e1 = cx * ay - cy * ax;
  float e2 = ax * by - ay * bx;
  if (e0 == 0.0f || e1 == 0.0f || e2 == 0.0f) {
    e0 = (float)((double)bx * (double)cy - (double)by * (double)cx);
    e1 = (float)((double)cx * (double)ay - (double)cy * (double)ax);
    e2 = (float)((double)ax * (double)by - (double)ay * (double)bx);
  }
  if ((e0 < 0.0f || e1 < 0.0f || e2 < 0.0f) && (e0 > 0.0f || e1 > 0.0f || e2 > 0.0f)) return false;
  const float det = e0 + e1 + e2;
  if (det == 0.0f) return false;
  const float az = r.sz * akz, bz = r.sz * bkz, cz = r.sz * ckz;
  const float t_scaled = e0 * az + e1 * bz + e2 * cz;
  if (det < 0.0f && (t_scaled > t_min * det || t_scaled < t_max * det)) return false;
  if (det > 0.0f && (t_scaled < t_min * det || t_scaled > t_max * det)) return false;
  const float inv_det = 1.0f / det;
  to = t_scaled * inv_det;
  uo = e1 * inv_det;
  vo = e2 * inv_det;
  return true;
}

__device__ __forceinline__ void tri_normal(const DevScene &S, uint32_t prim_abs, float u, float v, float &nx, float &ny,
                                           float &nz) {
  const DevPrim *p = &S.prims[prim_abs];
  const uint32_t slot = __float_as_uint(p->d[9]);
  float x, y, z;
  if (slot != kInvalid) {
    const float *n = S.normals + 9 * (size_t)slot;
    const float w = 1.0f - u - v;
    x = (n[0] * w + n[3] * u) + n[6] * v;
    y = (n[1] * w + n[4] * u) + n[7] * v;
    z = (n[2] * w + n[5] * u) + n[8] * v;
  } else {
    const float e1x = p->d[3] - p->d[0], e1y = p->d[4] - p->d[1], e1z = p->d[5] - p->d[2];
    const float e2x = p->d[6] - p->d[0], e2y = p->d[7] - p->d[1], e2z = p->d[8] - p->d[2];
    x = e1y * e2z - e2y * e1z;
    y = e1z * e2x - e2z * e1x;
    z = e1x * e2y - e2x * e1y;
  }
  const float len = sqrtf(dot3(x, y, z, x, y, z));
  nx = x / len; ny = y / len; nz = z / len;
}

__device__ __forceinline__ void motion_w2l(const DevInstanceMotion &in, float time, float w2l[12]) {
  float m[12];
#pragma unroll
  for (int i = 0; i < 12; i++) m[i] = in.l2w[i] * (1.0f - time) + in.l2w_end[i] * time;
  const float t0x = m[4] * m[8] - m[7] * m[5], t0y = m[5] * m[6] - m[8] * m[3], t0z = m[3] * m[7] - m[6] * m[4];
  const float t1x = m[7] * m[2] - m[1] * m[8], t1y = m[8] * m[0] - m[2] * m[6], t1z = m[6] * m[1] - m[0] * m[7];
  const float t2x = m[1] * m[5] - m[4] * m[2], t2y = m[2] * m[3] - m[5] * m[0], t2z = m[0] * m[4] - m[3] * m[1];
  const float det = dot3(m[6], m[7], m[8], t2x, t2y, t2z);
  const float inv = 1.0f / det;
  w2l[0] = t0x * inv; w2l[1] = t1x * inv; w2l[2] = t2x * inv;
  w2l[3] = t0y * inv; w2l[4] = t1y * inv; w2l[5] = t2y * inv;
  w2l[6] = t0z * inv; w2l[7] = t1z * inv; w2l[8] = t2z * inv;
  float rx = w2l[0] * m[9], ry = w2l[1] * m[9], rz = w2l[2] * m[9];
  rx = rx + w2l[3] * m[10]; ry = ry + w2l[4] * m[10]; rz = rz + w2l[5] * m[10];
  rx = rx + w2l[6] * m[11]; ry = ry + w2l[7] * m[11]; rz = rz + w2l[8] * m[11];
  w2l[9] = -rx; w2l[10] = -ry; w2l[11] = -rz;
}

__device__ __forceinline__ void instance_normal(const DevScene &S, uint32_t inst, float time, float &nx, float &ny, float &nz) {
  const DevInstance &in = S.instances[inst];
  float nm[9];
  if ((in.flags & 2u) && time > 0.0f) {
    float w2l[12];
    motion_w2l(*reinterpret_cast<const DevInstanceMotion *>(S.normals + (in.flags >> 2)), time, w2l);
    nm[0] = w2l[0]; nm[1] = w2l[3]; nm[2] = w2l[6];
    nm[3] = w2l[1]; nm[4] = w2l[4]; nm[5] = w2l[7];
    nm[6] = w2l[2]; nm[7] = w2l[5]; nm[8] = w2l[8];
  } else {
    nm[0] = in.w2l[0]; nm[1] = in.w2l[3]; nm[2] = in.w2l[6];
    nm[3] = in.w2l[1]; nm[4] = in.w2l[4]; nm[5] = in.w2l[7];
    nm[6] = in.w2l[2]; nm[7] = in.w2l[5]; nm[8] = in.w2l[8];
  }
  float x = nm[0] * nx, y = nm[1] * nx, z = nm[2] * nx;
  x = x + nm[3] * ny; y = y + nm[4] * ny; z = z + nm[5] * ny;
  x = x + nm[6] * nz; y = y + nm[7] * nz; z = z + nm[8] * nz;
  const float len = sqrtf(dot3(x, y, z, x, y, z));
  nx = x / len; ny = y / len; nz = z / len;
}

constexpr int kLdsPacketDwords = 48;
#ifndef CRT_LDS_NODE_MAX
#define CRT_LDS_NODE_MAX 1000000
#endif
__device__ __forceinline__ uint32_t stage_nodes(const DevScene &S, uint32_t *lds_nodes, int cap, uint32_t &n_pk) {
  uint32_t n = S.n_nodes < (uint32_t)cap ? S.n_nodes : (uint32_t)cap;
  if (S.n_packets > 0 && n > (uint32_t)CRT_LDS_NODE_MAX) n = (uint32_t)CRT_LDS_NODE_MAX;
  const uint32_t room = ((uint32_t)cap - n) * (uint32_t)kLdsNodeStride / (uint32_t)kLdsPacketDwords;
  n_pk = S.n_packets < room ? S.n_packets : room;
  for (uint32_t w = threadIdx.x; w < n * 8u; w += blockDim.x) {
    const uint32_t node = w >> 3, part = w & 7u;
    if (part == 7u) continue;
    const float4 v = reinterpret_cast<const float4 *>(S.nodes + node)[part];
    *reinterpret_cast<float4 *>(lds_nodes + (size_t)node * kLdsNodeStride + part * 4) = v;
  }
  float4 *pk_dst = reinterpret_cast<float4 *>(lds_nodes + (size_t)n * kLdsNodeStride);
  const float4 *pk_src = reinterpret_cast<const float4 *>(S.packets);
  for (uint32_t w = threadIdx.x; w < n_pk * 12u; w += blockDim.x) pk_dst[w] = pk_src[w];
  __syncthreads();
  return n;
}

struct Frame {
  float ox, oy, oz, dx, dy, dz;
  uint32_t cursor, cend, base, inst, geom, has_packets;
};

struct RayIn {
  float ox, oy, oz, dx, dy, dz, time, t_min, t_max;
  uint32_t mask;
  uint32_t slot;
};

}
}
```

crust-render_amd/csrc/kernels/traverse_pool.hip.h:

```cpp
#pragma once

#include "traverse.hip.h"

namespace crt {
namespace dev {

#ifndef CRT_ROOT_REJECT
#define CRT_ROOT_REJECT 1
#endif
#ifndef CRT_DEFER_NORMAL
#define CRT_DEFER_NORMAL 1
#endif
#ifndef CRT_LDS_ROOT
#define CRT_LDS_ROOT 1
#endif
#ifndef CRT_EMIT_REFILL
#define CRT_EMIT_REFILL 0
#endif
#ifndef CRT_FETCH_MIN
#define CRT_FETCH_MIN 40
#endif
#ifndef CRT_NODE_SWAP
#define CRT_NODE_SWAP 0
#endif
#ifndef CRT_STACK_RING
#define CRT_STACK_RING 0
#endif
#ifndef CRT_SPILL_UNROLLED
#define CRT_SPILL_UNROLLED 1
#endif
#ifndef CRT_RARE_MIN
#define CRT_RARE_MIN 24
#endif
constexpr int kPoolStack = CRT_POOL_STACK;
constexpr int kPoolStackDeep = CRT_POOL_STACK_DEEP;
#ifndef CRT_POOL_SPILL
#define CRT_POOL_SPILL (255 - (kPoolStack > kPoolStackDeep ? kPoolStack : kPoolStackDeep))
#endif
constexpr int kPoolSpill = CRT_POOL_SPILL;
static_assert(kPoolStack + kPoolSpill <= 255 && kPoolStackDeep + kPoolSpill <= 255, "sp must fit the ctl word's 8 bits");
constexpr int kFetchMin = CRT_FETCH_MIN;
#ifndef CRT_EMIT_BIAS
#define CRT_EMIT_BIAS 16
#endif
#ifndef CRT_SCALAR_BIAS
#define CRT_SCALAR_BIAS 0
#endif
#ifndef CRT_EXIT_BIAS
#define CRT_EXIT_BIAS 0
#endif
#ifndef CRT_PACKET_BIAS
#define CRT_PACKET_BIAS 0
#endif
constexpr int kPacketBias = CRT_PACKET_BIAS;
constexpr int kEmitBias = CRT_EMIT_BIAS, kScalarBias = CRT_SCALAR_BIAS, kExitBias = CRT_EXIT_BIAS;
constexpr int kRareMin = CRT_RARE_MIN;
#ifndef CRT_STICKY_MIN
#define CRT_STICKY_MIN 24
#endif
constexpr int kStickyMin = CRT_STICKY_MIN;

template <int ROWS>
constexpr int pool_lds_dwords(int stack, bool umask = false) { return (4 + 4 + 2 + (umask ? 4 : 5) + stack) * ROWS * 64; }

enum : uint32_t { PH_FREE = 0, PH_NODE = 1, PH_PACKET = 2, PH_SCALAR = 3, PH_EXIT = 4, PH_EMIT = 5 };

__device__ __forceinline__ uint32_t ctl_pack(uint32_t sp, uint32_t base, uint32_t level, uint32_t hp, uint32_t kz,
                                             uint32_t swap, uint32_t lo) {
  return sp | (base << 8) | (level << 16) | (hp << 19) | (kz << 20) | (swap << 22) | (lo << 24);
}
__device__ __forceinline__ uint32_t ctl_sp(uint32_t c, uint32_t sp, uint32_t lo) { return (c & 0x00ffff00u) | (sp & 0xffu) | (lo << 24); }

__device__ __forceinline__ int wave_count(bool p) {
  int n = (int)__popcll(__ballot(p));
  asm volatile("" : "+s"(n));
  return n;
}

template <bool ANY, bool STATS, int ROWS, bool DIRECT, bool LEAN, int COLD, bool UMASK, class Fetch, class Emit>
__device__ void traverse_pool(const DevScene &S, uint32_t *lds , float t_min,
                              uint32_t umask ,
                              const uint32_t *lds_nodes , uint32_t n_lds,
                              uint32_t n_lds_pk , uint32_t pstack,
                              uint32_t &err, LaneStats &st, Fetch fetch, Emit emit) {
  const int lane = threadIdx.x & 63;
  constexpr int RL = ROWS * 64;
  constexpr bool NOPK = (COLD & (int)kNoPackets) != 0;
  float4 *f0 = reinterpret_cast<float4 *>(lds);
  float4 *f1 = reinterpret_cast<float4 *>(lds + 4 * RL);
  float2 *f2 = reinterpret_cast<float2 *>(lds + 8 * RL);
  uint32_t *w = lds + 10 * RL;
  enum { W_CTL = 0, W_CUR, W_AUX, W_CURSOR, W_MASK };
  enum { B_SLOT = 0, B_BU, B_BV, B_BDEFER, B_BGEOM, B_BINST };
  uint32_t *stk = lds + (UMASK ? 14 : 15) * RL;
  auto at = [&](int row) { return row * 64 + lane; };
  auto W = [&](int plane, int row) -> uint32_t & { return w[plane * RL + row * 64 + lane]; };
  auto STK = [&](int e, int row) -> uint32_t & { return stk[e * RL + row * 64 + lane]; };

  float side_d[ROWS][4];
  float side_n[ROWS][4];
  uint32_t best[ROWS][6];
  Frame frames[ROWS][kMaxLevels];
  uint32_t spill[ROWS][kPoolSpill];

  auto cold_dead = [&](auto &arr, int f) {
    if ((void *)&arr == (void *)&side_n) return !(COLD & kColdNormal);
    if ((void *)&arr == (void *)&side_d) return f == 3 && !(COLD & kColdTime);
    if ((void *)&arr == (void *)&best) return (f == B_BU || f == B_BV) && !(COLD & kColdUV);
    return false;
  };
  auto rd = [&](auto &arr, int row, int f) {
    auto r = arr[0][f];
    if (cold_dead(arr, f)) return (decltype(r))0;
#pragma unroll
    for (int k = 1; k < ROWS; k++) r = row == k ? arr[k][f] : r;
    return r;
  };
  auto wr = [&](auto &arr, int row, int f, auto val) {
    if (cold_dead(arr, f)) return;
#pragma unroll
    for (int k = 0; k < ROWS; k++) arr[k][f] = row == k ? (decltype(arr[k][f] + 0))val : arr[k][f];
  };
  const uint32_t ring_inv = (65536u + pstack - 1u) / pstack;
  auto slot_of = [&](uint32_t e, uint32_t lo) -> int {
    if (!CRT_STACK_RING || lo == 0u) return (int)e;
    return (int)(e - ((e * ring_inv) >> 16) * pstack);
  };
  auto push = [&](int row, uint32_t &sp, uint32_t &lo, uint32_t x) {
    if (CRT_STACK_RING) {
      if (sp - lo == pstack) {
        if (lo >= (uint32_t)kPoolSpill) { err |= 1u; return; }
        spill[row][lo] = STK(slot_of(lo, lo), row);
        lo++;
      }
      STK(slot_of(sp, lo), row) = x;
      sp++;
      return;
    }
    if (sp < pstack) STK((int)sp, row) = x;
    else if (sp - pstack < (uint32_t)kPoolSpill) spill[row][sp - pstack] = x;
    else { err |= 1u; return; }
    sp++;
  };
  auto pop = [&](int row, uint32_t &sp, uint32_t &lo) -> uint32_t {
    sp--;
    if (CRT_STACK_RING) {
      if (sp >= lo) return STK(slot_of(sp, lo), row);
      lo--;
      return spill[row][sp];
    }
    return sp < pstack ? STK((int)sp, row) : spill[row][sp - pstack];
  };
  constexpr bool direct_leaves = DIRECT;
  auto leaf_word = [&](uint32_t e, uint32_t level, uint32_t &cur, uint32_t &cursor, uint32_t &rem) -> uint32_t {
    if (direct_leaves && (e & kDirectLeafTag)) {
      cursor = (CRT_DIRECT_INST && (e & kDirectInstTag)) ? (kIndexInstance | (e & kDirectIndexMask)) : (e & kDirectIndexMask);
      rem = (e >> 28) & 3u;
      if (STATS) { st.leaves[level > 0 ? 1 : 0]++; st.prims[level > 0 ? 1 : 0] += rem; }
      return PH_SCALAR;
    }
    cur = e & ~kLeafTag;
    cursor = 0;
    return PH_PACKET;
  };
  auto advance = [&](int row, uint32_t &sp, uint32_t &lo, uint32_t base, uint32_t level, uint32_t &rem, uint32_t &cur,
                     uint32_t &cursor) -> uint32_t {
    if (rem > 0) return PH_SCALAR;
    for (;;) {
      if (sp == base) return level > 0 ? PH_EXIT : PH_EMIT;
      const uint32_t e = pop(row, sp, lo);
      if (e & kLeafTag) {
        if (e == kInvalid) continue;
        return leaf_word(e, level, cur, cursor, rem);
      }
      cur = e;
      return PH_NODE;
    }
  };
  auto unpack_k = [&](uint32_t c, int &kx, int &ky, int &kz) {
    kz = (int)((c >> 20) & 3u);
    kx = kz == 2 ? 0 : kz + 1;
    ky = kx == 2 ? 0 : kx + 1;
    if ((c >> 22) & 1u) { const int t = kx; kx = ky; ky = t; }
  };
  auto store_ray = [&](int row, RayCtx &r, bool with_shear, float closest, uint32_t &kz_out, uint32_t &swap_out) {
    r.kx = 0; r.ky = 1; r.kz = 2; r.sx = r.sy = r.sz = 0.0f;
    setup_ray(r, with_shear);
    kz_out = (uint32_t)r.kz;
    const int kx0 = r.kz == 2 ? 0 : r.kz + 1;
    swap_out = (r.kx != kx0) ? 1u : 0u;
    f0[at(row)] = make_float4(r.ox, r.oy, r.oz, closest);
    f1[at(row)] = make_float4(r.ix, r.iy, r.iz, r.sx);
    f2[at(row)] = make_float2(r.sy, r.sz);
  };

  auto setup_new = [&](int row, const RayIn &in) -> uint32_t {
    RayCtx r;
    r.ox = in.ox; r.oy = in.oy; r.oz = in.oz; r.dx = in.dx; r.dy = in.dy; r.dz = in.dz;
    uint32_t kz, swap;
    store_ray(row, r, !NOPK && S.has_packets != 0, in.t_max, kz, swap);
    const bool empty = S.root == kInvalid;
    W(W_CTL, row) = ctl_pack(0, 0, 0, S.has_packets ? 1u : 0u, kz, swap, 0);
    W(W_CUR, row) = S.root;
    W(W_AUX, row) = 0; W(W_CURSOR, row) = 0; wr(best, row, B_SLOT, in.slot);
    if (!UMASK) W(W_MASK, row) = in.mask;
    wr(best, row, B_BU, 0); wr(best, row, B_BV, 0); wr(best, row, B_BDEFER, kInvalid); wr(best, row, B_BGEOM, kInvalid);
    wr(best, row, B_BINST, kInvalid);
    wr(side_d, row, 0, in.dx); wr(side_d, row, 1, in.dy); wr(side_d, row, 2, in.dz); wr(side_d, row, 3, in.time);
    if (STATS) st.queries[0]++;
    return empty ? PH_EMIT : PH_NODE;
  };

  uint32_t ph[ROWS];
#pragma unroll
  for (int row = 0; row < ROWS; row++) ph[row] = PH_FREE;
  bool more = true;
  unsigned long long t_mark = STATS ? (unsigned long long)clock64() : 0ull;
  auto lap = [&](int k) {
    if (STATS) {
      const unsigned long long now = (unsigned long long)clock64();
      st.ph_cyc[k] += now - t_mark;
      t_mark = now;
    }
  };

  for (;;) {
    uint32_t have = 0;
#pragma unroll
    for (int row = 0; row < ROWS; row++) have |= 1u << ph[row];
    const int n_free = wave_count(have & (1u << PH_FREE));
    if (more && n_free >= kFetchMin) {
      lap(0);
      const bool want = (have & (1u << PH_FREE)) != 0;
      RayIn in;
      const bool got = fetch(want, in);
      if (got) {
        CRT_PHASE(1)
        int row = 0;
#pragma unroll
        for (int k = ROWS - 1; k >= 0; k--)
          if (ph[k] == PH_FREE) row = k;
        const uint32_t first = setup_new(row, in);
#pragma unroll
        for (int k = 0; k < ROWS; k++)
          if (k == row) ph[k] = first;
      }
      if (__ballot(want && !got)) more = false;
      lap(1);
      continue;
    }

    const int n_node = wave_count(have & (1u << PH_NODE));
    const int n_pkt = wave_count(have & (1u << PH_PACKET));
    const int n_sc = wave_count(have & (1u << PH_SCALAR));
    const int n_exit = wave_count(have & (1u << PH_EXIT));
    const int n_emit = wave_count(have & (1u << PH_EMIT));
    uint32_t q;
    {
      int best_rare = n_sc - kScalarBias;
      uint32_t q_rare = PH_SCALAR;
      if (n_exit - kExitBias > best_rare) { best_rare = n_exit - kExitBias; q_rare = PH_EXIT; }
      if (n_emit - kEmitBias > best_rare) { best_rare = n_emit - kEmitBias; q_rare = PH_EMIT; }
      if (best_rare >= kRareMin) q = q_rare;
      else if (n_node + n_pkt > 0) q = (n_node > 0 && (n_pkt == 0 || n_node + kPacketBias >= n_pkt)) ? PH_NODE : PH_PACKET;
      else {
        best_rare = n_sc; q_rare = PH_SCALAR;
        if (n_exit > best_rare) { best_rare = n_exit; q_rare = PH_EXIT; }
        if (n_emit > best_rare) { best_rare = n_emit; q_rare = PH_EMIT; }
        if (best_rare > 0) q = q_rare;
        else break;
      }
    }
    bool mine = (have & (1u << q)) != 0;
    int row = 0;
#pragma unroll
    for (int k = ROWS - 1; k >= 0; k--)
      if (ph[k] == q) row = k;
    uint32_t next = q;
    if (mine) { CRT_PHASE(0) }
    lap(0);

    if (q == PH_NODE) {
      float4 g0 = f0[at(row)], g1 = f1[at(row)];
      uint32_t c = W(W_CTL, row);
      uint32_t cur = W(W_CUR, row), cursor = 0, rem = 0;
      uint32_t sp = c & 0xffu, lo = c >> 24;
      uint32_t base = (c >> 8) & 0xffu, level = (c >> 16) & 7u;
      bool act = mine;
      auto retire = [&]() {
        W(W_CTL, row) = ctl_sp(c, sp, lo);
        W(W_CUR, row) = cur;
        if (next == PH_PACKET) W(W_CURSOR, row) = 0;
        if (next == PH_SCALAR) {
          W(W_CURSOR, row) = cursor;
          W(W_AUX, row) = (W(W_AUX, row) & 0xffu) | (rem << 8);
        }
      };
      for (;;) {
        if (act) {
          CRT_PHASE(2)
          const float closest = g0.w;
          if (STATS) st.nodes[level > 0 ? 1 : 0]++;
          float4 mnx, mny, mnz, mxx, mxy, mxz;
          uint4 ch;
          if (cur < n_lds) {
            const float4 *nb = reinterpret_cast<const float4 *>(lds_nodes + (size_t)cur * kLdsNodeStride);
            mnx = nb[0]; mny = nb[1]; mnz = nb[2]; mxx = nb[3]; mxy = nb[4]; mxz = nb[5];
            ch = *reinterpret_cast<const uint4 *>(nb + 6);
            asm volatile("" : "+v"(mnx.x), "+v"(mxx.x), "+v"(ch.x));
          } else {
            const WideNode *nd = &S.nodes[cur];
            const float4 *nb = reinterpret_cast<const float4 *>(nd);
            mnx = nb[0]; mny = nb[1]; mnz = nb[2]; mxx = nb[3]; mxy = nb[4]; mxz = nb[5];
            ch = *reinterpret_cast<const uint4 *>(nd->child);
          }
          const float lo_x[4] = {mnx.x, mnx.y, mnx.z, mnx.w}, lo_y[4] = {mny.x, mny.y, mny.z, mny.w},
                      lo_z[4] = {mnz.x, mnz.y, mnz.z, mnz.w};
          const float hi_x[4] = {mxx.x, mxx.y, mxx.z, mxx.w}, hi_y[4] = {mxy.x, mxy.y, mxy.z, mxy.w},
                      hi_z[4] = {mxz.x, mxz.y, mxz.z, mxz.w};
          const uint32_t child[4] = {ch.x, ch.y, ch.z, ch.w};
          float key[4];
          uint32_t ent[4];
#pragma unroll
          for (int l = 0; l < 4; l++) {
            const float t0x = (lo_x[l] - g0.x) * g1.x, t1x = (hi_x[l] - g0.x) * g1.x;
            const float t0y = (lo_y[l] - g0.y) * g1.y, t1y = (hi_y[l] - g0.y) * g1.y;
            const float t0z = (lo_z[l] - g0.z) * g1.z, t1z = (hi_z[l] - g0.z) * g1.z;
            const float tn = fmaxf(fmaxf(fmaxf(fminf(t0x, t1x), fminf(t0y, t1y)), fminf(t0z, t1z)), t_min);
            const float tf = fminf(fminf(fminf(fmaxf(t0x, t1x), fmaxf(t0y, t1y)), fmaxf(t0z, t1z)), closest);
            key[l] = tn;
            ent[l] = (tn <= tf) ? child[l] : kInvalid;
          }
          uint32_t on[4], lf4[4], pos[4];
#pragma unroll
          for (int i = 0; i < 4; i++) { on[i] = ent[i] != kInvalid ? 1u : 0u; lf4[i] = (on[i] && (ent[i] & kLeafTag)) ? 1u : 0u; }
          uint32_t n_tot;
          if (ANY) {
            const uint32_t in0 = on[0] & ~lf4[0], in1 = on[1] & ~lf4[1], in2 = on[2] & ~lf4[2], in3 = on[3] & ~lf4[3];
            const uint32_t n_in = in0 + in1 + in2 + in3;
            pos[0] = lf4[0] ? n_in + lf4[1] + lf4[2] + lf4[3] : 0u;
            pos[1] = lf4[1] ? n_in + lf4[2] + lf4[3] : in0;
            pos[2] = lf4[2] ? n_in + lf4[3] : in0 + in1;
            pos[3] = lf4[3] ? n_in : in0 + in1 + in2;
            n_tot = on[0] + on[1] + on[2] + on[3];
          } else {
#pragma unroll
            for (int i = 0; i < 4; i++) pos[i] = 0;
#pragma unroll
            for (int i = 0; i < 4; i++) {
#pragma unroll
              for (int j = i + 1; j < 4; j++) {
                const uint32_t a = key[i] <= key[j] ? 1u : 0u;
                const uint32_t t = lf4[i] ^ lf4[j];
                const uint32_t x = (t & lf4[i]) | (~t & a);
                pos[i] += on[j] & x;
                pos[j] += on[i] & (x ^ 1u);
              }
            }
            n_tot = on[0] + on[1] + on[2] + on[3];
          }
          if (n_tot == 0) {
            next = advance(row, sp, lo, base, level, rem, cur, cursor);
          } else {
            uint32_t top_e = 0;
            if (lo == 0u && sp + n_tot - 1 <= pstack) {
#pragma unroll
              for (int i = 0; i < 4; i++) {
                if (on[i]) {
                  if (pos[i] == n_tot - 1) top_e = ent[i];
                  else STK((int)(sp + pos[i]), row) = ent[i];
                }
              }
              sp += n_tot - 1;
            } else if (!CRT_STACK_RING && CRT_SPILL_UNROLLED) {
              const bool fits = sp + n_tot - 1 <= pstack + (uint32_t)kPoolSpill;
              if (!fits) err |= 1u;
#pragma unroll
              for (int i = 0; i < 4; i++) {
                if (on[i]) {
                  if (pos[i] == n_tot - 1) top_e = ent[i];
                  else if (fits) {
                    const uint32_t at = sp + pos[i];
                    if (at < pstack) STK((int)at, row) = ent[i];
                    else spill[row][at - pstack] = ent[i];
                  }
                }
              }
              if (fits) sp += n_tot - 1;
            } else {
              for (uint32_t k = 0; k < n_tot; k++) {
                uint32_t e = 0;
#pragma unroll
                for (int i = 0; i < 4; i++)
                  if (on[i] && pos[i] == k) e = ent[i];
                if (k == n_tot - 1) top_e = e;
                else push(row, sp, lo, e);
              }
            }
            if (top_e & kLeafTag) {
              if (top_e == kInvalid) next = advance(row, sp, lo, base, level, rem, cur, cursor);
              else next = leaf_word(top_e, level, cur, cursor, rem);
            } else {
              cur = top_e;
              next = PH_NODE;
            }
          }
          act = next == PH_NODE;
        }
        if (CRT_NODE_SWAP && ROWS == 2) {
          if (mine && !act) {
            retire();
#pragma unroll
            for (int k = 0; k < ROWS; k++)
              if (k == row) ph[k] = next;
            const uint32_t ph_other = row == 0 ? ph[ROWS - 1] : ph[0];
            if (ph_other == PH_NODE) {
              row ^= 1;
              g0 = f0[at(row)]; g1 = f1[at(row)];
              c = W(W_CTL, row);
              cur = W(W_CUR, row); cursor = 0; rem = 0;
              sp = c & 0xffu; lo = c >> 24; base = (c >> 8) & 0xffu; level = (c >> 16) & 7u;
              next = PH_NODE;
              act = true;
            } else {
              mine = false;
            }
          }
        }
        if (wave_count(act) < kStickyMin) break;
      }
      if (mine) retire();
    } else if (q == PH_PACKET) {
      const float4 g0 = f0[at(row)], g1 = f1[at(row)];
      const float2 g2 = f2[at(row)];
      const uint32_t c = W(W_CTL, row), rmask = UMASK ? umask : W(W_MASK, row);
      uint32_t cur = W(W_CUR, row), k = W(W_CURSOR, row), aux = W(W_AUX, row);
      uint32_t sp = c & 0xffu, lo = c >> 24;
      const uint32_t base = (c >> 8) & 0xffu, level = (c >> 16) & 7u;
      int kx, ky, kz;
      unpack_k(c, kx, ky, kz);
      float closest = g0.w;
      float bu = 0.0f, bv = 0.0f;
      uint32_t bdefer = kInvalid;
      bool accepted = false, occluded = false;
      uint32_t cursor = 0, rem = 0;
      bool act = mine;
      for (;;) {
        if (act) {
          Leaf lf;
          {
            uint4 lw = *reinterpret_cast<const uint4 *>(&S.leaves[cur]);
            asm volatile("" : "+v"(lw.x), "+v"(lw.y), "+v"(lw.z), "+v"(lw.w));
            lf.pkt_first = lw.x; lf.pkt_count = lw.y; lf.idx_first = lw.z; lf.idx_count = lw.w;
          }
          const int sl = level > 0 ? 1 : 0;
          if (STATS && k == 0) { st.leaves[sl]++; st.packets[sl] += lf.pkt_count; st.prims[sl] += lf.idx_count; }
          if (!NOPK && k < lf.pkt_count) {
            const uint32_t pki = lf.pkt_first + k;
            const bool pk_lds = pki < n_lds_pk;
            const Tri4 *pk = &S.packets[pki];
            const Tri4 *pk_l = reinterpret_cast<const Tri4 *>(lds_nodes + (size_t)n_lds * kLdsNodeStride) + (pk_lds ? pki : 0u);
            uint4 prim4;
            uint32_t normal_ok, m;
            float4 A_x, A_y, A_z, B_x, B_y, B_z, C_x, C_y, C_z;
            auto load_vertices = [&](const Tri4 *q) {
              const float4 *pl = reinterpret_cast<const float4 *>(q);
              A_x = pl[0 + kx]; A_y = pl[0 + ky]; A_z = pl[0 + kz];
              B_x = pl[3 + kx]; B_y = pl[3 + ky]; B_z = pl[3 + kz];
              C_x = pl[6 + kx]; C_y = pl[6 + ky]; C_z = pl[6 + kz];
            };
            if (!LEAN) {
              uint4 meta, mtail;
              auto load_packet = [&](const Tri4 *q) {
                load_vertices(q);
                const uint4 *pw = reinterpret_cast<const uint4 *>(q);
                prim4 = pw[9]; meta = pw[10]; mtail = pw[11];
              };
#define CRT_PACKET_ARRIVED                                                                                          \
  asm volatile("" : "+v"(A_x.x), "+v"(A_y.x), "+v"(A_z.x), "+v"(B_x.x), "+v"(B_y.x), "+v"(B_z.x), "+v"(C_x.x), \
               "+v"(C_y.x), "+v"(C_z.x), "+v"(prim4.x), "+v"(meta.x), "+v"(mtail.x))
              if (pk_lds) { load_packet(pk_l); CRT_PACKET_ARRIVED; }
              else { load_packet(pk); CRT_PACKET_ARRIVED; }
#undef CRT_PACKET_ARRIVED
              normal_ok = mtail.w;
              if (rmask & meta.y) m = meta.x;
              else if ((rmask & meta.z) == 0) m = 0;
              else {
                const uint32_t lane_mask[4] = {meta.w, mtail.x, mtail.y, mtail.z};
                m = 0;
#pragma unroll
                for (int l = 0; l < 4; l++)
                  if ((meta.x & (1u << l)) && (lane_mask[l] & rmask)) m |= 1u << l;
              }
            } else {
              uint4 meta;
              if (pk_lds) { meta = *reinterpret_cast<const uint4 *>(&pk_l->active); asm volatile("" : "+v"(meta.x)); }
              else meta = *reinterpret_cast<const uint4 *>(&pk->active);
              if (rmask & meta.y) m = meta.x;
              else if ((rmask & meta.z) == 0) m = 0;
              else {
                m = 0;
#pragma unroll
                for (int l = 0; l < 4; l++)
                  if ((meta.x & (1u << l)) && ((pk_lds ? pk_l->masks[l] : pk->masks[l]) & rmask)) m |= 1u << l;
              }
              if (m != 0) {
                auto load_rest = [&](const Tri4 *q) {
                  prim4 = *reinterpret_cast<const uint4 *>(q->prim);
                  normal_ok = q->normal_ok;
                  load_vertices(q);
                };
                if (pk_lds) { load_rest(pk_l); asm volatile("" : "+v"(A_x.x), "+v"(B_x.x), "+v"(C_x.x), "+v"(prim4.x)); }
                else load_rest(pk);
              }
            }
            if (m != 0) {
              CRT_PHASE(3)
              RayCtx r;
              r.ox = g0.x; r.oy = g0.y; r.oz = g0.z;
              r.kx = kx; r.ky = ky; r.kz = kz; r.sx = g1.w; r.sy = g2.x; r.sz = g2.y;
              r.okx = sel3(g0.x, g0.y, g0.z, kx); r.oky = sel3(g0.x, g0.y, g0.z, ky); r.okz = sel3(g0.x, g0.y, g0.z, kz);
              const uint32_t prim_of[4] = {prim4.x, prim4.y, prim4.z, prim4.w};
              const float vax[4] = {A_x.x, A_x.y, A_x.z, A_x.w}, vay[4] = {A_y.x, A_y.y, A_y.z, A_y.w},
                          vaz[4] = {A_z.x, A_z.y, A_z.z, A_z.w};
              const float vbx[4] = {B_x.x, B_x.y, B_x.z, B_x.w}, vby[4] = {B_y.x, B_y.y, B_y.z, B_y.w},
                          vbz[4] = {B_z.x, B_z.y, B_z.z, B_z.w};
              const float vcx[4] = {C_x.x, C_x.y, C_x.z, C_x.w}, vcy[4] = {C_y.x, C_y.y, C_y.z, C_y.w},
                          vcz[4] = {C_z.x, C_z.y, C_z.z, C_z.w};
              uint32_t fallback = 0, hits = 0;
              float ht[4], hu[4], hv[4];
              const float entry_closest = closest;
#pragma unroll
              for (int l = 0; l < 4; l++) {
                const float akz = vaz[l] - r.okz, bkz = vbz[l] - r.okz, ckz = vcz[l] - r.okz;
                const float ax = (vax[l] - r.okx) - r.sx * akz, ay = (vay[l] - r.oky) - r.sy * akz;
                const float bx = (vbx[l] - r.okx) - r.sx * bkz, by = (vby[l] - r.oky) - r.sy * bkz;
                const float cx = (vcx[l] - r.okx) - r.sx * ckz, cy = (vcy[l] - r.oky) - r.sy * ckz;
                const float e0 = bx * cy - by * cx;
                const float e1 = cx * ay - cy * ax;
                const float e2 = ax * by - ay * bx;
                const bool zero = (e0 == 0.0f) | (e1 == 0.0f) | (e2 == 0.0f);
                const bool neg = (e0 < 0.0f) | (e1 < 0.0f) | (e2 < 0.0f);
                const bool pos = (e0 > 0.0f) | (e1 > 0.0f) | (e2 > 0.0f);
                const float det = e0 + e1 + e2;
                const float t_scaled = e0 * (r.sz * akz) + e1 * (r.sz * bkz) + e2 * (r.sz * ckz);
                const float abs_det = absf(det);
                const float ts = det < 0.0f ? -t_scaled : t_scaled;
                const bool in_range = (ts >= t_min * abs_det) & (ts <= entry_closest * abs_det);
                const bool lane_on = (m >> l) & 1u;
                if (lane_on && zero) fallback |= 1u << l;
                if (lane_on && !zero && !(neg && pos) && det != 0.0f && in_range) hits |= 1u << l;
                const float inv_det = 1.0f / det;
                ht[l] = t_scaled * inv_det;
                hu[l] = e1 * inv_det;
                hv[l] = e2 * inv_det;
              }
              if (ANY) {
                if (hits) occluded = true;
              } else {
#pragma unroll
                for (int l = 0; l < 4; l++) {
                  if (!((hits >> l) & 1u)) continue;
                  if (ht[l] > closest) continue;
                  if (!((normal_ok >> l) & 1u)) continue;
                  closest = ht[l]; bu = hu[l]; bv = hv[l];
                  bdefer = prim_of[l];
                  accepted = true;
                  if (STATS) st.accepted++;
                }
              }
              if (fallback && !occluded) {
#pragma unroll
                for (int l = 0; l < 4; l++) {
                  if (!((fallback >> l) & 1u)) continue;
                  const uint32_t pi = prim_of[l];
                  const DevPrim *p = &S.prims[pi];
                  if ((rmask & p->mask) == 0) continue;
                  CRT_PHASE(7)
                  float t, u, v;
                  if (!tri_scalar(r, p->d, t_min, closest, t, u, v)) continue;
                  if (ANY) { occluded = true; break; }
                  if (!((normal_ok >> l) & 1u)) continue;
                  closest = t; bu = u; bv = v; bdefer = pi;
                  accepted = true;
                  if (STATS) st.accepted++;
                }
              }
            }
            k++;
          }
          if (occluded) {
            next = PH_EMIT;
            act = false;
          } else if (k < lf.pkt_count) {
            next = PH_PACKET;
          } else {
            cursor = lf.idx_first;
            rem = lf.idx_count;
            next = PH_SCALAR;
            act = false;
          }
        }
        if (wave_count(act) < kStickyMin) break;
      }
      if (mine) {
        if (accepted) {
          f0[at(row)].w = closest;
          wr(best, row, B_BU, __float_as_uint(bu)); wr(best, row, B_BV, __float_as_uint(bv)); wr(best, row, B_BDEFER, bdefer);
          wr(best, row, B_BINST, kInvalid);
          aux |= 1u << level;
        }
        if (occluded) aux |= 1u;
        if (next == PH_PACKET) {
          cursor = k;
        } else if (next == PH_SCALAR) {
          next = advance(row, sp, lo, base, level, rem, cur, cursor);
          aux = (aux & 0xffu) | (rem << 8);
        }
        W(W_CTL, row) = ctl_sp(c, sp, lo);
        W(W_CUR, row) = cur;
        W(W_CURSOR, row) = cursor;
        W(W_AUX, row) = aux;
      }
    } else if (q == PH_SCALAR) {
      if (mine) {
        CRT_PHASE(4)
        const float4 g0 = f0[at(row)];
        uint32_t c = W(W_CTL, row);
        uint32_t sp = c & 0xffu, lo = c >> 24;
        uint32_t base = (c >> 8) & 0xffu, level = (c >> 16) & 7u;
        const uint32_t hp = (c >> 19) & 1u;
        uint32_t cur = W(W_CUR, row);
        uint32_t cursor = W(W_CURSOR, row);
        uint32_t aux = W(W_AUX, row);
        const uint32_t rmask = UMASK ? umask : W(W_MASK, row);
        uint32_t rem = aux >> 8;
        float closest = g0.w;
        const float dx = rd(side_d, row, 0), dy = rd(side_d, row, 1), dz = rd(side_d, row, 2), time = rd(side_d, row, 3);
        bool occluded = false;
        const uint32_t pi = (CRT_DIRECT_INST && direct_leaves && (cursor & kIndexInstance)) ? cursor : S.indices[cursor];
        cursor++;
        rem--;
        if (pi & kIndexInstance) {
          const uint32_t inst = pi & ~kIndexInstance;
          const DevInstance *in = &S.instances[inst];
          const uint4 ih = *reinterpret_cast<const uint4 *>(&in->root);
          if ((rmask & ih.w) != 0) {
            if (level + 1 >= (uint32_t)kMaxLevels) err |= 2u;
            else {
              float w2l[12];
              if ((ih.y & 2u) && time > 0.0f) motion_w2l(*reinterpret_cast<const DevInstanceMotion *>(S.normals + (ih.y >> 2)), time, w2l);
              else {
#pragma unroll
                for (int i = 0; i < 12; i++) w2l[i] = in->w2l[i];
              }
              float px = w2l[0] * g0.x, py = w2l[1] * g0.x, pz = w2l[2] * g0.x;
              px = px + w2l[3] * g0.y; py = py + w2l[4] * g0.y; pz = pz + w2l[5] * g0.y;
              px = px + w2l[6] * g0.z; py = py + w2l[7] * g0.z; pz = pz + w2l[8] * g0.z;
              px = px + w2l[9]; py = py + w2l[10]; pz = pz + w2l[11];
              float qx = w2l[0] * dx, qy = w2l[1] * dx, qz = w2l[2] * dx;
              qx = qx + w2l[3] * dy; qy = qy + w2l[4] * dy; qz = qz + w2l[5] * dy;
              qx = qx + w2l[6] * dz; qy = qy + w2l[7] * dz; qz = qz + w2l[8] * dz;
              RayCtx r;
              r.ox = px; r.oy = py; r.oz = pz; r.dx = qx; r.dy = qy; r.dz = qz;
              bool enter = true;
              if (CRT_ROOT_REJECT && DIRECT) {
                float4 mnx, mny, mnz, mxx, mxy, mxz;
                uint4 ch;
                if (CRT_LDS_ROOT && ih.x < n_lds) {
                  const float4 *nb = reinterpret_cast<const float4 *>(lds_nodes + (size_t)ih.x * kLdsNodeStride);
                  mnx = nb[0]; mny = nb[1]; mnz = nb[2]; mxx = nb[3]; mxy = nb[4]; mxz = nb[5];
                  ch = *reinterpret_cast<const uint4 *>(nb + 6);
                  asm volatile("" : "+v"(mnx.x), "+v"(mxx.x), "+v"(ch.x));
                } else {
                  const float4 *nb = reinterpret_cast<const float4 *>(&S.nodes[ih.x]);
                  mnx = nb[0]; mny = nb[1]; mnz = nb[2]; mxx = nb[3]; mxy = nb[4]; mxz = nb[5];
                  ch = *reinterpret_cast<const uint4 *>(nb + 6);
                }
                const float TINY = 1e-20f, HUGE_ = 1e20f;
                const float ix = absf(qx) < TINY ? copysgn(HUGE_, qx) : 1.0f / qx;
                const float iy = absf(qy) < TINY ? copysgn(HUGE_, qy) : 1.0f / qy;
                const float iz = absf(qz) < TINY ? copysgn(HUGE_, qz) : 1.0f / qz;
                const float lo_x[4] = {mnx.x, mnx.y, mnx.z, mnx.w}, lo_y[4] = {mny.x, mny.y, mny.z, mny.w},
                            lo_z[4] = {mnz.x, mnz.y, mnz.z, mnz.w};
                const float hi_x[4] = {mxx.x, mxx.y, mxx.z, mxx.w}, hi_y[4] = {mxy.x, mxy.y, mxy.z, mxy.w},
                            hi_z[4] = {mxz.x, mxz.y, mxz.z, mxz.w};
                const uint32_t child[4] = {ch.x, ch.y, ch.z, ch.w};
                enter = false;
#pragma unroll
                for (int l = 0; l < 4; l++) {
                  const float t0x = (lo_x[l] - px) * ix, t1x = (hi_x[l] - px) * ix;
                  const float t0y = (lo_y[l] - py) * iy, t1y = (hi_y[l] - py) * iy;
                  const float t0z = (lo_z[l] - pz) * iz, t1z = (hi_z[l] - pz) * iz;
                  const float tn = fmaxf(fmaxf(fmaxf(fminf(t0x, t1x), fminf(t0y, t1y)), fminf(t0z, t1z)), t_min);
                  const float tf = fminf(fminf(fminf(fmaxf(t0x, t1x), fmaxf(t0y, t1y)), fmaxf(t0z, t1z)), closest);
                  enter |= (tn <= tf) && child[l] != kInvalid;
                }
              }
              if (STATS) { st.descents++; st.queries[1]++; }
              if (!enter) {
                if (STATS) st.nodes[1]++;
              } else {
                Frame f;
                f.ox = g0.x; f.oy = g0.y; f.oz = g0.z; f.dx = dx; f.dy = dy; f.dz = dz;
                f.cursor = cursor; f.cend = rem; f.base = base; f.inst = inst; f.geom = ih.z; f.has_packets = hp;
                frames[row][level] = f;
                wr(side_d, row, 0, qx); wr(side_d, row, 1, qy); wr(side_d, row, 2, qz);
                level++;
                aux &= ~(1u << level);
                base = sp;
                cursor = 0;
                rem = 0;
                uint32_t kz, swap;
                store_ray(row, r, !NOPK && (ih.y & 1u) != 0, closest, kz, swap);
                c = ctl_pack(sp, base, level, ih.y & 1u, kz, swap, 0);
                push(row, sp, lo, ih.x);
              }
            }
          }
        } else {
        const DevPrim *p = &S.prims[pi];
        const uint4 hd = *reinterpret_cast<const uint4 *>(p);
        if ((rmask & hd.w) != 0) {
          if (hd.x == PRIM_SPHERE) {
            const float4 s = *reinterpret_cast<const float4 *>(p->d);
            const float ocx = g0.x - s.x, ocy = g0.y - s.y, ocz = g0.z - s.z;
            const float a = dot3(dx, dy, dz, dx, dy, dz);
            const float half_b = dot3(ocx, ocy, ocz, dx, dy, dz);
            const float cc = dot3(ocx, ocy, ocz, ocx, ocy, ocz) - s.w * s.w;
            const float disc = half_b * half_b - a * cc;
            if (!(disc < 0.0f)) {
              const float sqrt_d = sqrtf(disc);
              float root = (-half_b - sqrt_d) / a;
              bool ok = true;
              if (root <= t_min || root >= closest) {
                root = (-half_b + sqrt_d) / a;
                if (root <= t_min || root >= closest) ok = false;
              }
              if (ok) {
                if (ANY) occluded = true;
                else {
                  closest = root;
                  f0[at(row)].w = root;
                  wr(side_n, row, 0, ((g0.x + root * dx) - s.x) / s.w);
                  wr(side_n, row, 1, ((g0.y + root * dy) - s.y) / s.w);
                  wr(side_n, row, 2, ((g0.z + root * dz) - s.z) / s.w);
                  wr(side_n, row, 3, __uint_as_float(0u));
                  wr(best, row, B_BU, 0); wr(best, row, B_BV, 0); wr(best, row, B_BDEFER, kInvalid); wr(best, row, B_BGEOM, hd.y);
                  wr(best, row, B_BINST, kInvalid);
                  aux |= 1u << level;
                  if (STATS) st.accepted++;
                }
              }
            }
          } else {
            RayCtx rr;
            rr.ox = g0.x; rr.oy = g0.y; rr.oz = g0.z; rr.dx = dx; rr.dy = dy; rr.dz = dz;
            setup_ray(rr, true);
            float t, u, v;
            if (tri_scalar(rr, p->d, t_min, closest, t, u, v)) {
              if (ANY) occluded = true;
              else {
                const float e1x = p->d[3] - p->d[0], e1y = p->d[4] - p->d[1], e1z = p->d[5] - p->d[2];
                const float e2x = p->d[6] - p->d[0], e2y = p->d[7] - p->d[1], e2z = p->d[8] - p->d[2];
                const bool flat = (e1y * e2z - e2y * e1z) == 0.0f && (e1z * e2x - e2z * e1x) == 0.0f &&
                                  (e1x * e2y - e2x * e1y) == 0.0f;
                if (!(flat && __float_as_uint(p->d[9]) == kInvalid)) {
                  closest = t;
                  f0[at(row)].w = t;
                  wr(best, row, B_BU, __float_as_uint(u)); wr(best, row, B_BV, __float_as_uint(v)); wr(best, row, B_BDEFER, pi);
                  wr(best, row, B_BINST, kInvalid);
                  aux |= 1u << level;
                  if (STATS) st.accepted++;
                }
              }
            }
          }
        }
        }
        if (occluded) { aux |= 1u; next = PH_EMIT; }
        else next = advance(row, sp, lo, base, level, rem, cur, cursor);
        aux = (aux & 0xffu) | (rem << 8);
        W(W_CTL, row) = (c & 0x00ff0000u) | sp | (base << 8) | (lo << 24);
        W(W_CUR, row) = cur;
        W(W_CURSOR, row) = cursor;
        W(W_AUX, row) = aux;
      }
    } else if (q == PH_EXIT) {
      if (mine) {
        CRT_PHASE(5)
        const uint32_t c = W(W_CTL, row);
        uint32_t sp = c & 0xffu, lo = c >> 24;
        uint32_t level = (c >> 16) & 7u;
        uint32_t aux = W(W_AUX, row);
        uint32_t cur = W(W_CUR, row);
        const float closest = f0[at(row)].w;
        const float time = rd(side_d, row, 3);
        const bool inner_found = (aux >> level) & 1u;
        level--;
        const Frame f = frames[row][level];
        if (inner_found && CRT_DEFER_NORMAL && level == 0) {
          wr(best, row, B_BINST, f.inst); wr(best, row, B_BGEOM, f.geom);
          aux |= 1u;
          if (STATS) st.accepted++;
        } else if (inner_found) {
          float bnx, bny, bnz;
          uint32_t bprim;
          const uint32_t bdefer = rd(best, row, B_BDEFER);
          if (bdefer != kInvalid) {
            tri_normal(S, bdefer, __uint_as_float(rd(best, row, B_BU)), __uint_as_float(rd(best, row, B_BV)), bnx, bny, bnz);
            bprim = S.prims[bdefer].prim_id;
          } else {
            bnx = rd(side_n, row, 0); bny = rd(side_n, row, 1); bnz = rd(side_n, row, 2);
            bprim = __float_as_uint(rd(side_n, row, 3));
          }
          instance_normal(S, f.inst, time, bnx, bny, bnz);
          wr(side_n, row, 0, bnx); wr(side_n, row, 1, bny); wr(side_n, row, 2, bnz);
          wr(side_n, row, 3, __uint_as_float(bprim));
          wr(best, row, B_BDEFER, kInvalid); wr(best, row, B_BGEOM, f.geom);
          wr(best, row, B_BINST, kInvalid);
          aux |= 1u << level;
          if (STATS) st.accepted++;
        }
        RayCtx r;
        r.ox = f.ox; r.oy = f.oy; r.oz = f.oz; r.dx = f.dx; r.dy = f.dy; r.dz = f.dz;
        wr(side_d, row, 0, f.dx); wr(side_d, row, 1, f.dy); wr(side_d, row, 2, f.dz);
        uint32_t kz, swap;
        store_ray(row, r, !NOPK && f.has_packets != 0, closest, kz, swap);
        uint32_t cursor = f.cursor;
        uint32_t rem = f.cend;
        next = advance(row, sp, lo, f.base, level, rem, cur, cursor);
        W(W_CTL, row) = ctl_pack(sp, f.base, level, f.has_packets ? 1u : 0u, kz, swap, lo);
        W(W_CUR, row) = cur;
        W(W_CURSOR, row) = cursor;
        W(W_AUX, row) = (aux & 0xffu) | (rem << 8);
      }
    } else {
      if (mine) {
        CRT_PHASE(6)
        const uint32_t aux = W(W_AUX, row);
        const uint32_t slot = rd(best, row, B_SLOT);
        const bool is_hit = (aux & 1u) != 0;
        Hit hit;
        hit.t = 0.0f; hit.u = 0.0f; hit.v = 0.0f; hit.nx = hit.ny = hit.nz = 0.0f; hit.geom = kInvalid; hit.prim = kInvalid;
        if (!ANY && is_hit) {
          hit.t = f0[at(row)].w;
          hit.u = __uint_as_float(rd(best, row, B_BU)); hit.v = __uint_as_float(rd(best, row, B_BV));
          const uint32_t bdefer = rd(best, row, B_BDEFER);
          if (bdefer != kInvalid) {
            tri_normal(S, bdefer, hit.u, hit.v, hit.nx, hit.ny, hit.nz);
            const DevPrim *p = &S.prims[bdefer];
            hit.geom = p->geom_id; hit.prim = p->prim_id;
          } else {
            hit.nx = rd(side_n, row, 0); hit.ny = rd(side_n, row, 1); hit.nz = rd(side_n, row, 2);
            hit.geom = rd(best, row, B_BGEOM); hit.prim = __float_as_uint(rd(side_n, row, 3));
          }
          const uint32_t binst = rd(best, row, B_BINST);
          if (CRT_DEFER_NORMAL && binst != kInvalid) {
            instance_normal(S, binst, rd(side_d, row, 3), hit.nx, hit.ny, hit.nz);
            hit.geom = rd(best, row, B_BGEOM);
          }
        }
        emit(slot, is_hit, hit, rd(side_d, row, 0), rd(side_d, row, 1), rd(side_d, row, 2));
        next = PH_FREE;
      }
      if (CRT_EMIT_REFILL && more) {
        RayIn in;
        const bool got = fetch(mine, in);
        if (got) next = setup_new(row, in);
        if (__ballot(mine && !got)) more = false;
      }
    }
    if (mine) {
#pragma unroll
      for (int k = 0; k < ROWS; k++)
        if (k == row) ph[k] = next;
    }
    lap(q == PH_NODE ? 2 : q == PH_PACKET ? 3 : q == PH_SCALAR ? 4 : q == PH_EXIT ? 5 : 6);
  }
}

#ifndef CRT_POOL_ROWS
#define CRT_POOL_ROWS 2
#endif
constexpr int kPoolNodes = CRT_POOL_NODES;
constexpr int kPoolNodesDeep = CRT_POOL_NODES_DEEP;
constexpr int kEngineLdsFlat = (kBlock / 64) * pool_lds_dwords<CRT_POOL_ROWS>(kPoolStack) + kPoolNodes * kLdsNodeStride;
constexpr int kEngineLdsDeep = (kBlock / 64) * pool_lds_dwords<CRT_POOL_ROWS>(kPoolStackDeep) + kPoolNodesDeep * kLdsNodeStride;
constexpr int kEngineLdsDwords = kEngineLdsFlat > kEngineLdsDeep ? kEngineLdsFlat : kEngineLdsDeep;
constexpr int kPoolStackWide = CRT_POOL_STACK_WIDE;
constexpr int kPoolNodesWide = CRT_POOL_NODES_WIDE;
#ifndef CRT_POOL_NODES_WIDE_DEEP
#define CRT_POOL_NODES_WIDE_DEEP 12
#endif
__host__ __device__ constexpr int wide_stack(bool deep_tree, bool umask) { return kPoolStackWide + (deep_tree ? 1 : 0) + (umask ? 1 : 0); }
__host__ __device__ constexpr int wide_nodes(bool deep_tree) { return deep_tree ? CRT_POOL_NODES_WIDE_DEEP : kPoolNodesWide; }
constexpr int wide_arena(bool deep_tree, bool umask) {
  return (kBlock / 64) * pool_lds_dwords<CRT_POOL_ROWS>(wide_stack(deep_tree, umask), umask) + wide_nodes(deep_tree) * kLdsNodeStride;
}
constexpr int imax(int a, int b) { return a > b ? a : b; }
constexpr int kEngineLdsWide = imax(imax(wide_arena(false, false), wide_arena(false, true)), imax(wide_arena(true, false), wide_arena(true, true)));
static_assert(kEngineLdsWide * 4 + 512 <= 40 * 1024, "four workgroups of the wide split per CU");
template <bool ANY, bool STATS, int WIDE, int COLD = (int)kColdAll, bool UMASK = false, class Fetch, class Emit>
__device__ __forceinline__ void run_traversal(const DevScene &S, uint32_t *lds, float t_min, uint32_t &err, LaneStats &st,
                                              Fetch fetch, Emit emit, uint32_t umask = 0u) {
  const bool deep_tree = S.pool_stack >= (uint32_t)kPoolStackDeep;
  const uint32_t pstack = WIDE ? (uint32_t)wide_stack(deep_tree, UMASK)
                               : (deep_tree ? (uint32_t)kPoolStackDeep : (uint32_t)kPoolStack);
  const int pnodes = WIDE ? wide_nodes(deep_tree) : (deep_tree ? kPoolNodesDeep : kPoolNodes);
  const int wave_dwords = pool_lds_dwords<CRT_POOL_ROWS>((int)pstack, UMASK);
  uint32_t *lds_nodes = lds + (kBlock / 64) * wave_dwords;
  uint32_t n_lds_pk;
  const uint32_t n_lds = stage_nodes(S, lds_nodes, pnodes, n_lds_pk);
  uint32_t *wave_lds = lds + (threadIdx.x >> 6) * wave_dwords;
#ifndef CRT_WIDE_LEAN
#define CRT_WIDE_LEAN 1
#endif
#define CRT_ENGINE(D) traverse_pool<ANY, STATS, CRT_POOL_ROWS, D, (WIDE && CRT_WIDE_LEAN != 0), COLD, UMASK>(S, wave_lds, t_min, umask, lds_nodes, n_lds, n_lds_pk, pstack, err, st, fetch, emit)
  if ((COLD & (int)kNoPackets) != 0 || WIDE == 2) CRT_ENGINE(true);
  else if (CRT_DIRECT_LEAVES != 0 && !WIDE && S.direct_leaves != 0) CRT_ENGINE(true);
  else CRT_ENGINE(false);
#undef CRT_ENGINE
}

}
}
```

crust-render_amd/csrc/scene.cpp:

```cpp
#include <hip/hip_runtime.h>

#include <cstdarg>
#include <cstdio>
#include <cmath>
#include <cstring>
#include <algorithm>
#include <utility>
#include <unordered_map>

#include <cstdlib>
#include "crt_internal.h"

namespace crt {

static F3 mat3_mul(const Mat3 &m, F3 r) {
  F3 res = m.x * r.x;
  res = res + m.y * r.y;
  res = res + m.z * r.z;
  return res;
}
Mat3 mat3_transpose(const Mat3 &m) {
  return {f3(m.x.x, m.y.x, m.z.x), f3(m.x.y, m.y.y, m.z.y), f3(m.x.z, m.y.z, m.z.z)};
}
static Mat3 mat3_inverse(const Mat3 &m) {
  F3 t0 = cross(m.y, m.z), t1 = cross(m.z, m.x), t2 = cross(m.x, m.y);
  float det = dot(m.z, t2);
  float inv = 1.0f / det;
  return mat3_transpose(Mat3{t0 * inv, t1 * inv, t2 * inv});
}
Affine affine_inverse(const Affine &a) {
  Mat3 inv = mat3_inverse(Mat3{a.x, a.y, a.z});
  F3 t = -mat3_mul(inv, a.t);
  return {inv.x, inv.y, inv.z, t};
}
F3 affine_point(const Affine &a, F3 p) { return mat3_mul(Mat3{a.x, a.y, a.z}, p) + a.t; }
F3 affine_vector(const Affine &a, F3 p) { return mat3_mul(Mat3{a.x, a.y, a.z}, p); }

Aabb transformed_aabb(const Aabb &local, const Affine &m) {
  const float inf = __builtin_inff();
  F3 mn = f3(inf, inf, inf), mx = f3(-inf, -inf, -inf);
  for (int i = 0; i < 8; i++) {
    F3 corner = f3((i & 1) == 0 ? local.mn.x : local.mx.x, (i & 2) == 0 ? local.mn.y : local.mx.y,
                   (i & 4) == 0 ? local.mn.z : local.mx.z);
    F3 p = affine_point(m, corner);
    mn = vmin(mn, p);
    mx = vmax(mx, p);
  }
  constexpr float PAD = 1e-4f;
  for (int a = 0; a < 3; a++)
    if (mx[a] - mn[a] < PAD) { mn.at(a) -= PAD; mx.at(a) += PAD; }
  return {mn, mx};
}

std::shared_ptr<Scene> commit(Builder &&b) {
  auto scene = std::make_shared<Scene>();
  scene->n_geoms = uint32_t(b.geoms.size());
  size_t total = 0;
  for (const Geom &g : b.geoms) total += g.kind == G_MESH ? g.idx.size() / 3 : 1;
  std::vector<Prim> prims;
  prims.reserve(total);
  bool has_motion = false;
  uint32_t depth = 1;
  for (size_t gi = 0; gi < b.geoms.size(); gi++) {
    Geom &g = b.geoms[gi];
    const uint32_t geom_id = uint32_t(gi);
    switch (g.kind) {
      case G_MESH: {
        const size_t nv = g.verts.size() / 3, nn = g.normals.size() / 3, nt = g.idx.size() / 3;
        auto vert = [&](const std::vector<float> &a, size_t i) { return f3(a[3 * i], a[3 * i + 1], a[3 * i + 2]); };
        for (size_t t = 0; t < nt; t++) {
          size_t i0 = g.idx[3 * t], i1 = g.idx[3 * t + 1], i2 = g.idx[3 * t + 2];
          if (i0 >= nv || i1 >= nv || i2 >= nv) continue;
          Prim p{};
          p.kind = PRIM_TRI;
          p.geom_id = geom_id;
          p.prim_id = uint32_t(t);
          p.mask = g.mask;
          p.v0 = vert(g.verts, i0);
          p.v1 = vert(g.verts, i1);
          p.v2 = vert(g.verts, i2);
          if (g.has_normals && i0 < nn && i1 < nn && i2 < nn) {
            p.has_normals = true;
            p.n0 = vert(g.normals, i0);
            p.n1 = vert(g.normals, i1);
            p.n2 = vert(g.normals, i2);
          }
          prims.push_back(std::move(p));
        }
        break;
      }
      case G_SPHERE: {
        Prim p{};
        p.kind = PRIM_SPHERE;
        p.geom_id = geom_id;
        p.mask = g.mask;
        p.center = g.center;
        p.radius = g.radius;
        prims.push_back(std::move(p));
        break;
      }
      case G_INSTANCE: {
        if (!g.scene || !g.scene->bvh.has_bbox) break;
        const Aabb inner = g.scene->bvh.root_bbox;
        Prim p{};
        p.kind = PRIM_INSTANCE;
        p.geom_id = geom_id;
        p.mask = g.mask;
        p.scene = g.scene;
        p.l2w = g.l2w;
        p.w2l = affine_inverse(g.l2w);
        p.normal_mat = mat3_transpose(Mat3{p.w2l.x, p.w2l.y, p.w2l.z});
        p.has_end = g.has_end;
        p.l2w_end = g.l2w_end;
        if (g.has_end) {
          Aabb a = transformed_aabb(inner, g.l2w), e = transformed_aabb(inner, g.l2w_end);
          p.bounds = Aabb{vmin(a.mn, e.mn), vmax(a.mx, e.mx)};
        } else {
          p.bounds = transformed_aabb(inner, g.l2w);
        }
        has_motion |= g.has_end || g.scene->has_motion;
        if (g.scene->depth + 1 > depth) depth = g.scene->depth + 1;
        prims.push_back(std::move(p));
        break;
      }
    }
  }
  if (depth > kMaxInstanceLevels) {
    set_error_text("commit: %u levels of instance nesting, the kernels carry %u", depth, kMaxInstanceLevels);
    return nullptr;
  }
  scene->depth = depth;
  scene->has_motion = has_motion;
  build_bvh(scene->bvh, std::move(prims));
  return scene;
}

DeviceImage::~DeviceImage() {
  if (blob) (void)hipFree(blob);
}

static thread_local char g_last_error[512] = "";
const char *last_error_text() { return g_last_error; }
bool hip_failed(int err, const char *what, const char *file, int line) {
  if (err == (int)hipSuccess) return false;
  std::snprintf(g_last_error, sizeof g_last_error, "%s -> %s (%d) at %s:%d", what, hipGetErrorString((hipError_t)err), err,
                file, line);
  return true;
}

void set_error_text(const char *fmt, ...) {
  va_list ap;
  va_start(ap, fmt);
  std::vsnprintf(g_last_error, sizeof g_last_error, fmt, ap);
  va_end(ap);
}

Knobs read_knobs() {
  Knobs k;
  auto num = [](const char *name, long long &out) {
    const char *e = getenv(name);
    if (!e || !*e) return false;
    char *end = nullptr;
    const long long v = strtoll(e, &end, 10);
    if (end == e) return false;
    out = v;
    return true;
  };
  long long v;
  if (num("CRT_POOL_STACK_RT", v)) k.pool_stack_deep = v >= CRT_POOL_STACK_DEEP ? 1 : 0;
  if (num("CRT_DIRECT_LEAVES", v)) k.direct_leaves = v != 0;
  if (num("CRT_DIRECT_INST", v)) k.direct_inst = v != 0;
  if (num("CRT_STAGE_ROOTS", v)) k.stage_roots = (int)std::min<long long>(std::max<long long>(v, 0), 1 << 20);
  if (num("CRT_COLD", v)) k.cold = (uint32_t)v & kColdAll;
  if (num("CRT_INST_ORDER", v)) k.inst_order = v != 0;
  if (num("CRT_HOT_PACKETS", v)) k.hot_packets = v != 0;
  if (num("CRT_WIDE", v)) k.wide = v == 2 ? 2 : (v != 0);
  if (num("CRT_MAT_DEDUP", v)) k.mat_dedup = v != 0;
  if (num("CRT_PARTITION", v)) k.partition = v != 0;
  if (num("CRT_SIMPLE", v)) k.simple = v != 0;
  if (num("CRT_PREFER_STAGE", v)) k.prefer_stage = v != 0;
  if (num("CRT_CAM_COMPACT", v)) k.cam_compact = v != 0;
  if (num("CRT_SHADE_WIDE", v)) k.shade_wide = v != 0;
  if (num("CRT_FUSED", v)) k.fused = v != 0;
  if (num("CRT_NOCLASSIFY_FROM", v)) k.noclassify_from = (int)std::min<long long>(std::max<long long>(v, 0), 1 << 30);
  if (num("CRT_TAIL_FROM", v)) k.tail_from = (int)std::min<long long>(std::max<long long>(v, 0), 1 << 30);
  if (num("CRT_LANES", v)) k.lanes = (int)std::min<long long>(std::max<long long>(v, 1), 4);
  if (num("CRT_GRID_MULT", v)) k.grid_mult = (int)std::min<long long>(std::max<long long>(v, 0), 64);
  if (num("CRT_MAX_BATCH_SLOTS", v)) k.max_batch_slots = v > 0 ? (size_t)v : 0;
  if (num("CRT_LANE_MIN_PATHS", v)) k.lane_min_paths = v > 0 ? (size_t)v : 1;
  if (num("CRT_STAGE_MIN_PATHS", v)) k.stage_min_paths = v > 0 ? (size_t)v : 1;
  return k;
}
int wide_request() { return read_knobs().wide; }

int device_ok() {
  static int ok = [] {
    int n = 0;
    if (!CRT_HIP_OK(hipGetDeviceCount(&n)) || n <= 0) return 0;
    return 1;
  }();
  return ok;
}

namespace {
struct Flat {
  std::vector<WideNode> nodes;
  std::vector<Leaf> leaves;
  std::vector<Tri4> packets;
  std::vector<uint32_t> indices;
  std::vector<DevPrim> prims;
  std::vector<DevInstance> instances;
  std::vector<std::pair<uint32_t, DevInstanceMotion>> moving;
  std::vector<float> normals;
  struct Placed { uint32_t root; uint32_t has_packets; };
  std::unordered_map<const Scene *, Placed> placed;
};

void put_affine(float out[12], const Affine &a) {
  const float v[12] = {a.x.x, a.x.y, a.x.z, a.y.x, a.y.y, a.y.z, a.z.x, a.z.y, a.z.z, a.t.x, a.t.y, a.t.z};
  std::memcpy(out, v, sizeof v);
}
uint32_t f2u(float f) { uint32_t u; std::memcpy(&u, &f, 4); return u; }
float u2f(uint32_t u) { float f; std::memcpy(&f, &u, 4); return f; }

Flat::Placed place(Flat &f, const Scene &s) {
  auto it = f.placed.find(&s);
  if (it != f.placed.end()) return it->second;
  const Bvh &b = s.bvh;
  std::vector<Flat::Placed> inner(b.prims.size(), Flat::Placed{CRT_INVALID_ID, 0});
  for (size_t i = 0; i < b.prims.size(); i++)
    if (b.prims[i].kind == PRIM_INSTANCE) inner[i] = place(f, *b.prims[i].scene);

  const uint32_t node0 = uint32_t(f.nodes.size()), leaf0 = uint32_t(f.leaves.size());
  const uint32_t pkt0 = uint32_t(f.packets.size()), idx0 = uint32_t(f.indices.size());
  const uint32_t prim0 = uint32_t(f.prims.size());
  for (WideNode n : b.wide) {
    for (int l = 0; l < 4; l++) {
      if (!(n.flags & (1u << l))) continue;
      n.child[l] += (n.flags & (1u << (4 + l))) ? leaf0 : node0;
    }
    f.nodes.push_back(n);
  }
  for (Leaf l : b.leaves) {
    l.pkt_first += pkt0;
    l.idx_first += idx0;
    f.leaves.push_back(l);
  }
  for (Tri4 p : b.packets) {
    for (int l = 0; l < 4; l++)
      if (p.active & (1u << l)) p.prim[l] += prim0;
    f.packets.push_back(p);
  }
  std::vector<uint32_t> inst_slot(b.prims.size(), CRT_INVALID_ID);
  {
    uint32_t next_slot = uint32_t(f.instances.size());
    if (read_knobs().inst_order)
    for (uint32_t i : b.indices)
      if (b.prims[i].kind == PRIM_INSTANCE && inst_slot[i] == CRT_INVALID_ID) inst_slot[i] = next_slot++;
    for (size_t i = 0; i < b.prims.size(); i++)
      if (b.prims[i].kind == PRIM_INSTANCE && inst_slot[i] == CRT_INVALID_ID) inst_slot[i] = next_slot++;
    f.instances.resize(next_slot);
  }
  for (size_t i = 0; i < b.prims.size(); i++) {
    const Prim &p = b.prims[i];
    DevPrim d{};
    d.kind = p.kind;
    d.geom_id = p.geom_id;
    d.prim_id = p.prim_id;
    d.mask = p.mask;
    if (p.kind == PRIM_TRI) {
      const float v[9] = {p.v0.x, p.v0.y, p.v0.z, p.v1.x, p.v1.y, p.v1.z, p.v2.x, p.v2.y, p.v2.z};
      std::memcpy(d.d, v, sizeof v);
      uint32_t slot = 0xFFFFFFFFu;
      if (p.has_normals) {
        slot = uint32_t(f.normals.size() / 9);
        const float n[9] = {p.n0.x, p.n0.y, p.n0.z, p.n1.x, p.n1.y, p.n1.z, p.n2.x, p.n2.y, p.n2.z};
        f.normals.insert(f.normals.end(), n, n + 9);
      }
      d.d[9] = u2f(slot);
    } else if (p.kind == PRIM_SPHERE) {
      d.d[0] = p.center.x; d.d[1] = p.center.y; d.d[2] = p.center.z; d.d[3] = p.radius;
    } else {
      DevInstance in{};
      put_affine(in.w2l, p.w2l);
      in.root = inner[i].root;
      in.flags = (inner[i].has_packets ? 1u : 0u) | (p.has_end ? 2u : 0u);
      in.geom_id = p.geom_id;
      in.mask = p.mask;
      d.d[0] = u2f(inst_slot[i]);
      f.instances[inst_slot[i]] = in;
      if (p.has_end) {
        DevInstanceMotion mo{};
        put_affine(mo.l2w, p.l2w);
        put_affine(mo.l2w_end, p.l2w_end);
        f.moving.emplace_back(inst_slot[i], mo);
      }
    }
    f.prims.push_back(d);
  }
  for (uint32_t i : b.indices)
    f.indices.push_back(b.prims[i].kind == PRIM_INSTANCE ? (kIndexInstance | inst_slot[i]) : (i + prim0));
  Flat::Placed me{b.wide.empty() ? CRT_INVALID_ID : node0, b.packets.empty() ? 0u : 1u};
  f.placed.emplace(&s, me);
  return me;
}
}

namespace {
struct FlatImage {
  Flat f;
  Flat::Placed me{CRT_INVALID_ID, 0};
  uint32_t pool_stack = 6;
  bool direct = false;
  std::vector<uint32_t> leaf_of_word;
  uint32_t n_staged_roots = 0;
  uint32_t n_top_packets = 0;
  uint32_t cold = kColdAll;
};

uint32_t instance_levels(const Scene &s) {
  uint32_t d = 0;
  for (const Prim &p : s.bvh.prims)
    if (p.kind == PRIM_INSTANCE && p.scene) d = std::max(d, 1u + instance_levels(*p.scene));
  return d;
}

int flatten_image(const Scene &scene, FlatImage &im) {
  Flat &f = im.f;
  im.me = place(f, scene);
  Flat::Placed &me = im.me;
  {
    const size_t n_top = scene.bvh.packets.size(), n_all = f.packets.size();
    im.n_top_packets = uint32_t(n_top);
    if (n_top && n_top < n_all) {
      std::rotate(f.packets.begin(), f.packets.end() - n_top, f.packets.end());
      for (Leaf &l : f.leaves)
        if (l.pkt_count) l.pkt_first = l.pkt_first >= n_all - n_top ? uint32_t(l.pkt_first - (n_all - n_top)) : uint32_t(l.pkt_first + n_top);
    }
    const Knobs knobs = read_knobs();
    if (knobs.hot_packets && n_top > 1) {
      std::vector<std::pair<float, uint32_t>> order;
      for (const WideNode &n : f.nodes)
        for (int l = 0; l < 4; l++) {
          if (!(n.flags & (1u << l)) || !(n.flags & (1u << (4 + l)))) continue;
          const Leaf &lf = f.leaves[n.child[l]];
          if (!lf.pkt_count || lf.pkt_first >= n_top) continue;
          const float dx = n.bmax[0][l] - n.bmin[0][l], dy = n.bmax[1][l] - n.bmin[1][l], dz = n.bmax[2][l] - n.bmin[2][l];
          order.emplace_back(-((dx * dy + dy * dz) + dz * dx), n.child[l]);
        }
      std::stable_sort(order.begin(), order.end());
      std::vector<Tri4> hot;
      hot.reserve(n_top);
      for (const auto &o : order) {
        Leaf &lf = f.leaves[o.second];
        const uint32_t at = uint32_t(hot.size());
        hot.insert(hot.end(), f.packets.begin() + lf.pkt_first, f.packets.begin() + lf.pkt_first + lf.pkt_count);
        lf.pkt_first = at;
      }
      if (hot.size() == n_top) std::copy(hot.begin(), hot.end(), f.packets.begin());
      else return CRT_ERR_BAD_ARG;
    }
  }
  const bool many_instances = f.instances.size() >= 64;
  const bool large_tree = f.nodes.size() > 2048;
  uint32_t pool_stack = (many_instances || large_tree) ? 10u : 6u;
  const Knobs knobs = read_knobs();
  if (knobs.pool_stack_deep >= 0) pool_stack = knobs.pool_stack_deep ? (uint32_t)CRT_POOL_STACK_DEEP : (uint32_t)CRT_POOL_STACK;
  im.pool_stack = pool_stack;
  const bool deep = pool_stack >= 10u;
  if (!f.nodes.empty()) {
    std::vector<uint32_t> new_idx(f.nodes.size(), CRT_INVALID_ID), order;
    order.reserve(f.nodes.size());
    auto number = [&](uint32_t n) {
      if (new_idx[n] != CRT_INVALID_ID) return;
      new_idx[n] = uint32_t(order.size());
      order.push_back(n);
    };
    auto bfs_tree = [&](uint32_t root) {
      number(root);
      std::vector<uint32_t> q{root};
      for (size_t h = 0; h < q.size(); h++) {
        const WideNode &n = f.nodes[q[h]];
        for (int l = 0; l < 4; l++)
          if ((n.flags & (1u << l)) && !(n.flags & (1u << (4 + l)))) { number(n.child[l]); q.push_back(n.child[l]); }
      }
    };
    std::vector<std::pair<uint32_t, uint32_t>> inner_roots;
    {
      std::unordered_map<uint32_t, uint32_t> count;
      for (const DevInstance &in : f.instances)
        if (in.root != CRT_INVALID_ID) count[in.root]++;
      for (const auto &kv : count) inner_roots.emplace_back(kv.second, kv.first);
      std::sort(inner_roots.begin(), inner_roots.end(), [](const auto &a, const auto &b) {
        return a.first != b.first ? a.first > b.first : a.second < b.second;
      });
    }
    const size_t window = deep ? CRT_POOL_NODES_DEEP : std::min<size_t>(CRT_POOL_NODES, CRT_POOL_NODES_WIDE);
    size_t n_staged_roots = std::min(inner_roots.size(), window / 2);
    if (knobs.stage_roots >= 0) n_staged_roots = std::min(n_staged_roots, (size_t)knobs.stage_roots);
    im.n_staged_roots = uint32_t(n_staged_roots);
    if (me.root != CRT_INVALID_ID) number(me.root);
    for (size_t k = 0; k < n_staged_roots; k++) number(inner_roots[k].second);
    if (me.root != CRT_INVALID_ID) bfs_tree(me.root);
    for (const auto &r : inner_roots) bfs_tree(r.second);
    std::vector<WideNode> renum(order.size());
    for (size_t k = 0; k < order.size(); k++) {
      WideNode n = f.nodes[order[k]];
      for (int l = 0; l < 4; l++)
        if ((n.flags & (1u << l)) && !(n.flags & (1u << (4 + l)))) n.child[l] = new_idx[n.child[l]];
      renum[k] = n;
    }
    f.nodes.swap(renum);
    for (DevInstance &in : f.instances)
      if (in.root != CRT_INVALID_ID) in.root = new_idx[in.root];
    if (me.root != CRT_INVALID_ID) me.root = new_idx[me.root];
  }
  if (f.nodes.size() >= (size_t(1) << 31) || f.leaves.size() >= (size_t(1) << 30) || f.indices.size() >= (size_t(1) << 31)) {
    set_error_text("scene image: %zu nodes / %zu leaves / %zu list entries exceed the child word's index range",
                   f.nodes.size(), f.leaves.size(), f.indices.size());
    return CRT_ERR_UNSUPPORTED;
  }
  bool direct = many_instances || f.packets.empty();
  if (knobs.direct_leaves >= 0) direct = knobs.direct_leaves != 0;
  if (!CRT_DIRECT_LEAVES) direct = false;
  im.direct = direct;
  bool direct_inst = CRT_DIRECT_INST != 0;
  if (knobs.direct_inst >= 0) direct_inst = direct_inst && knobs.direct_inst != 0;
  im.leaf_of_word.assign(f.nodes.size() * 4, CRT_INVALID_ID);
  for (size_t ni = 0; ni < f.nodes.size(); ni++) {
    WideNode &n = f.nodes[ni];
    for (int l = 0; l < 4; l++) {
      if (!(n.flags & (1u << l))) n.child[l] = CRT_INVALID_ID;
      else if (n.flags & (1u << (4 + l))) {
        im.leaf_of_word[ni * 4 + l] = n.child[l];
        const Leaf &lf = f.leaves[n.child[l]];
        if (direct && lf.pkt_count == 0 && lf.idx_count >= 1 && lf.idx_count <= 3) {
          const uint32_t e0 = f.indices[lf.idx_first];
          bool run = direct_inst && (e0 & kIndexInstance) && ((e0 & ~kIndexInstance) + lf.idx_count <= kDirectIndexMask);
          for (uint32_t k = 1; run && k < lf.idx_count; k++) run = f.indices[lf.idx_first + k] == e0 + k;
          if (run) {
            n.child[l] = 0x80000000u | kDirectLeafTag | (lf.idx_count << 28) | kDirectInstTag | (e0 & ~kIndexInstance);
            continue;
          }
          if (lf.idx_first <= kDirectIndexMask) {
            n.child[l] = 0x80000000u | kDirectLeafTag | (lf.idx_count << 28) | lf.idx_first;
            continue;
          }
        }
        n.child[l] |= 0x80000000u;
      }
    }
  }
  {
    uint32_t cold = 0;
    for (const DevPrim &d : f.prims) {
      if (d.kind == PRIM_SPHERE) cold |= kColdNormal;
      if (d.kind == PRIM_TRI && f2u(d.d[9]) != 0xFFFFFFFFu) cold |= kColdUV;
    }
    if (instance_levels(scene) > 1) cold |= kColdNormal;
    if (!f.moving.empty()) cold |= kColdTime;
    cold |= knobs.cold;
    im.cold = cold;
  }
  for (const auto &mv : f.moving) {
    const size_t at = (f.normals.size() + 3) & ~size_t(3);
    if (at + 24 >= (size_t(1) << 30)) {
      set_error_text("scene image: %zu normal floats leave no room to address a moving instance's placements", f.normals.size());
      return CRT_ERR_UNSUPPORTED;
    }
    f.normals.resize(at + 24);
    std::memcpy(&f.normals[at], &mv.second, sizeof(DevInstanceMotion));
    f.instances[mv.first].flags |= uint32_t(at) << 2;
  }
  return CRT_OK;
}
}

int scene_image_check(const Scene &scene, uint64_t out[8]) {
  FlatImage im;
  int rc = flatten_image(scene, im);
  if (rc != CRT_OK) return rc;
  const Flat &f = im.f;
  auto fail = [&](const char *what, size_t a, size_t b) {
    set_error_text("scene image check: %s (%zu, %zu)", what, a, b);
    return CRT_ERR_BAD_ARG;
  };
  uint64_t n_plain = 0, n_dindex = 0, n_dinst = 0;
  std::vector<uint32_t> parents(f.nodes.size(), 0), leaf_refs(f.leaves.size(), 0);
  for (size_t ni = 0; ni < f.nodes.size(); ni++)
    for (int l = 0; l < 4; l++) {
      const uint32_t w = f.nodes[ni].child[l], lo = im.leaf_of_word[ni * 4 + l];
      const bool valid = (f.nodes[ni].flags >> l) & 1u, leaf = (f.nodes[ni].flags >> (4 + l)) & 1u;
      if (!valid) { if (w != CRT_INVALID_ID) return fail("an empty lane is not the empty word", ni, l); continue; }
      if (!leaf) {
        if ((w & 0x80000000u) || w >= f.nodes.size()) return fail("inner child out of range", ni, w);
        parents[w]++;
        continue;
      }
      if (lo >= f.leaves.size() || !(w & 0x80000000u) || w == CRT_INVALID_ID) return fail("leaf word without its leaf", ni, l);
      leaf_refs[lo]++;
      const Leaf &lf = f.leaves[lo];
      if (!(w & kDirectLeafTag)) {
        if ((w & 0x7fffffffu) != lo) return fail("plain leaf word names another leaf", ni, lo);
        n_plain++;
        continue;
      }
      if (!im.direct || lf.pkt_count != 0) return fail("direct word for a leaf that has packets, or with direct leaves off", ni, lo);
      const uint32_t count = (w >> 28) & 3u;
      if (count != lf.idx_count || count == 0) return fail("direct word's count", count, lf.idx_count);
      for (uint32_t k = 0; k < count; k++) {
        const uint32_t want = f.indices[lf.idx_first + k];
        const uint32_t got = (w & kDirectInstTag) ? (kIndexInstance | ((w & kDirectIndexMask) + k))
                                                  : f.indices[(w & kDirectIndexMask) + k];
        if (got != want) return fail("direct word's entries differ from the leaf's list", got, want);
      }
      (w & kDirectInstTag) ? n_dinst++ : n_dindex++;
    }
  for (size_t k = 0; k < f.leaves.size(); k++)
    if (leaf_refs[k] != 1) return fail("a leaf is not referenced exactly once", k, leaf_refs[k]);
  for (const Leaf &lf : f.leaves)
    if (lf.pkt_count && size_t(lf.pkt_first) + lf.pkt_count > f.packets.size()) return fail("a leaf's packet range", lf.pkt_first, lf.pkt_count);
  if (im.me.root != CRT_INVALID_ID) {
    std::vector<uint32_t> q{im.me.root};
    for (size_t h = 0; h < q.size(); h++)
      for (int l = 0; l < 4; l++) {
        const uint32_t lo = im.leaf_of_word[size_t(q[h]) * 4 + l];
        const bool valid = (f.nodes[q[h]].flags >> l) & 1u, leaf = (f.nodes[q[h]].flags >> (4 + l)) & 1u;
        if (valid && !leaf) q.push_back(f.nodes[q[h]].child[l]);
        else if (valid && f.leaves[lo].pkt_count && f.leaves[lo].pkt_first + f.leaves[lo].pkt_count > im.n_top_packets)
          return fail("a packet of the queried tree lies behind the instanced trees' packets", f.leaves[lo].pkt_first, im.n_top_packets);
      }
  }
  std::vector<uint8_t> is_root(f.nodes.size(), 0);
  if (im.me.root != CRT_INVALID_ID) { if (im.me.root != 0) return fail("the queried scene's root is not node 0", im.me.root, 0); is_root[0] = 1; }
  uint32_t staged = 0;
  for (size_t k = 0; k < f.instances.size(); k++) {
    const DevInstance &in = f.instances[k];
    if (in.root == CRT_INVALID_ID) continue;
    if (in.root >= f.nodes.size()) return fail("instance root out of range", k, in.root);
    if (!is_root[in.root] && in.root >= 1 && in.root <= im.n_staged_roots) staged++;
    is_root[in.root] = 1;
  }
  if (staged != im.n_staged_roots) return fail("instanced roots are not numbered right behind node 0", staged, im.n_staged_roots);
  for (size_t k = 0; k < f.nodes.size(); k++)
    if (parents[k] != (is_root[k] ? 0u : 1u)) return fail("node numbering is not a permutation of the trees", k, parents[k]);
  for (uint32_t e : f.indices) {
    if (e & kIndexInstance) { if ((e & ~kIndexInstance) >= f.instances.size()) return fail("list entry: instance slot", e, f.instances.size()); }
    else if (e >= f.prims.size()) return fail("list entry: primitive", e, f.prims.size());
  }
  uint64_t moving = 0;
  for (const auto &mv : f.moving) {
    const DevInstance &in = f.instances[mv.first];
    const size_t at = in.flags >> 2;
    if (!(in.flags & 2u) || (at & 3u) || at + 24 > f.normals.size() ||
        std::memcmp(&f.normals[at], &mv.second, sizeof(DevInstanceMotion)) != 0)
      return fail("a moving instance's placements are not where its flags word says", mv.first, at);
    moving++;
  }
  for (size_t k = 0; k < f.instances.size(); k++)
    if (!(f.instances[k].flags & 2u) && (f.instances[k].flags >> 2) != 0) return fail("a static instance carries a placement offset", k, 0);
  out[0] = f.nodes.size(); out[1] = n_plain; out[2] = n_dindex; out[3] = n_dinst;
  out[4] = f.instances.size(); out[5] = moving; out[6] = im.n_staged_roots; out[7] = im.direct ? 1 : 0;
  return CRT_OK;
}

namespace {
void fill_view_fields(const FlatImage &im, DevScene &v) {
  v.root = im.me.root;
  v.has_packets = im.me.has_packets;
  v.n_nodes = uint32_t(im.f.nodes.size());
  v.n_packets = uint32_t(im.f.packets.size());
  v.direct_leaves = im.direct ? 1u : 0u;
  v.pool_stack = im.pool_stack;
  v.cold = im.cold;
}
}

int scene_engine_select(const Scene &scene, int want_wide, uint32_t out[8]) {
  FlatImage im;
  int rc = flatten_image(scene, im);
  if (rc != CRT_OK) return rc;
  DevScene v{};
  fill_view_fields(im, v);
  EngineSelect e;
  const bool renderer = want_wide <= -3;
  rc = want_wide <= -2 && want_wide != -4 ? select_engine_env(v, e, renderer) : select_engine(v, want_wide == -4 ? -1 : want_wide, e, renderer);
  if (rc != CRT_OK) {
    set_error_text("select_engine: the %s kernels cannot decode this image (direct child words: %s)",
                   want_wide > 0 ? "four-wave" : "three-wave", v.direct_leaves ? "yes" : "no");
    return rc;
  }
  uint32_t n_direct = 0, need_cold = 0;
  for (const WideNode &n : im.f.nodes)
    for (int l = 0; l < 4; l++) {
      const uint32_t w = n.child[l];
      if (w != CRT_INVALID_ID && (w & 0x80000000u) && (w & kDirectLeafTag)) n_direct++;
    }
  for (const DevPrim &d : im.f.prims) {
    if (d.kind == PRIM_SPHERE) need_cold |= kColdNormal;
    if (d.kind == PRIM_TRI && f2u(d.d[9]) != 0xFFFFFFFFu) need_cold |= kColdUV;
  }
  if (instance_levels(scene) > 1) need_cold |= kColdNormal;
  if (!im.f.moving.empty()) need_cold |= kColdTime;
  auto fail = [&](const char *what) {
    set_error_text("engine select check: %s (wide %d, direct %d, direct words %u, cold %u / kernel %d %d)", what, (int)e.wide,
                   (int)e.direct, n_direct, need_cold, e.ext_cold, e.path_cold);
    return CRT_ERR_BAD_ARG;
  };
  if (n_direct && ((e.wide && !e.wide_direct) || !e.direct)) return fail("the image holds direct child words the selected instance cannot read");
  if (e.wide_direct && !v.direct_leaves) return fail("the direct-engine instances of the four-wave kernels selected for an image without direct words");
  if (n_direct && !v.direct_leaves) return fail("direct words in an image whose view says there are none");
  if ((need_cold & ~(uint32_t)e.ext_cold) || (need_cold & ~(uint32_t)e.path_cold)) return fail("the image needs cold state the selected kernels do not keep");
  if (!engine_accepts(e, v, e.ext_cold) || !engine_accepts(e, v, e.path_cold)) return fail("engine_accepts disagrees with select_engine");
  out[0] = e.wide ? (e.wide_direct ? 2u : 1u) : 0u; out[1] = e.direct; out[2] = e.lds_stack; out[3] = e.window;
  out[4] = (uint32_t)e.ext_cold; out[5] = (uint32_t)e.path_cold; out[6] = n_direct; out[7] = v.cold;
  return CRT_OK;
}

int Scene::ensure_device() {
  std::lock_guard<std::mutex> lock(dev_mu);
  if (dev) return CRT_OK;
  if (!device_ok()) return CRT_ERR_NO_DEVICE;
  FlatImage im;
  const int rc = flatten_image(*this, im);
  if (rc != CRT_OK) return rc;
  Flat &f = im.f;
  auto img = std::make_unique<DeviceImage>();
  constexpr int NA = 7;
  const size_t sz[NA] = {f.nodes.size() * sizeof(WideNode), f.leaves.size() * sizeof(Leaf),
                         f.packets.size() * sizeof(Tri4),   f.indices.size() * sizeof(uint32_t),
                         f.prims.size() * sizeof(DevPrim),  f.instances.size() * sizeof(DevInstance),
                         f.normals.size() * sizeof(float)};
  const void *src[NA] = {f.nodes.data(), f.leaves.data(), f.packets.data(), f.indices.data(),
                         f.prims.data(), f.instances.data(), f.normals.data()};
  size_t off[NA], total = 0;
  for (int i = 0; i < NA; i++) {
    off[i] = total;
    total += (sz[i] + 255) & ~size_t(255);
    img->bytes[i] = sz[i];
  }
  const size_t err_off = total;
  total += 256;
  if (!CRT_HIP_OK(hipMalloc(&img->blob, total))) return CRT_ERR_NO_DEVICE;
  if (!CRT_HIP_OK(hipMemset(static_cast<char *>(img->blob) + err_off, 0, 256))) return CRT_ERR_NO_DEVICE;
  img->err = reinterpret_cast<uint32_t *>(static_cast<char *>(img->blob) + err_off);
  for (int i = 0; i < NA; i++)
    if (sz[i] && !CRT_HIP_OK(hipMemcpy(static_cast<char *>(img->blob) + off[i], src[i], sz[i], hipMemcpyHostToDevice)))
      return CRT_ERR_NO_DEVICE;
  char *base = static_cast<char *>(img->blob);
  img->view.nodes = reinterpret_cast<const WideNode *>(base + off[0]);
  img->view.leaves = reinterpret_cast<const Leaf *>(base + off[1]);
  img->view.packets = reinterpret_cast<const Tri4 *>(base + off[2]);
  img->view.indices = reinterpret_cast<const uint32_t *>(base + off[3]);
  img->view.prims = reinterpret_cast<const DevPrim *>(base + off[4]);
  img->view.instances = reinterpret_cast<const DevInstance *>(base + off[5]);
  img->view.normals = reinterpret_cast<const float *>(base + off[6]);
  fill_view_fields(im, img->view);
  dev = std::move(img);
  return CRT_OK;
}

}
```

include/crt.h:

```cpp
#ifndef CRT_H
#define CRT_H

#include <stddef.h>
#include <stdint.h>

#ifdef __cplusplus
extern "C" {
#endif

#define CRT_INVALID_ID 0xFFFFFFFFu
#define CRT_MASK_CAMERA 1u
#define CRT_MASK_SHADOW 2u
#define CRT_MASK_INDIRECT 4u
#define CRT_MASK_ALL 0xFFFFFFFFu

typedef enum {
  CRT_OK = 0,
  CRT_ERR_BAD_ARG = -1,
  CRT_ERR_BAD_ID = -2,
  CRT_ERR_NO_DEVICE = -3,
  CRT_ERR_STACK = -4,
  CRT_ERR_UNSUPPORTED = -5,
  CRT_ERR_NO_MEMORY = -6
} CrtStatus;

typedef struct CrtRay {
  float origin[3]; float _pad0;
  float dir[3];    float _pad1;
  float time;
  uint32_t mask;
  uint32_t _pad2[2];
} CrtRay;

typedef struct CrtRayHit {
  float t;
  float normal[3];
  uint32_t front_face;
  float u, v;
  uint32_t geom_id;
  uint32_t prim_id;
  uint32_t _pad;
} CrtRayHit;

typedef struct CrtTravStats {
  uint64_t queries[2], nodes[2], leaves[2], packets[2], prims[2];
  uint64_t accepted_hits, instance_descents, rays;
  uint64_t phase_waves[8], phase_lanes[8];
  uint64_t phase_cycles[8];
} CrtTravStats;

typedef struct CrtBuilder CrtBuilder;
typedef struct CrtScene CrtScene;

CrtBuilder *crt_builder_new(void);
void crt_builder_free(CrtBuilder *b);
int crt_reserve(CrtBuilder *b, size_t additional);
size_t crt_count(const CrtBuilder *b);
int crt_attach_triangles(CrtBuilder *b, const float *verts, size_t n_verts, const uint32_t *indices, size_t n_tris,
                         const float *normals, size_t n_normals, uint32_t mask, uint32_t *geom_id_out);
int crt_attach_sphere(CrtBuilder *b, const float center[3], float radius, uint32_t mask, uint32_t *geom_id_out);
int crt_attach_instance(CrtBuilder *b, CrtScene *scene, const float l2w[12], const float *l2w_end, uint32_t mask,
                        uint32_t *geom_id_out);
int crt_attach_empty(CrtBuilder *b, uint32_t mask, uint32_t *geom_id_out);
int crt_set_triangles(CrtBuilder *b, uint32_t id, const float *verts, size_t n_verts, const uint32_t *indices,
                      size_t n_tris, const float *normals, size_t n_normals);
int crt_set_sphere(CrtBuilder *b, uint32_t id, const float center[3], float radius);
int crt_set_instance(CrtBuilder *b, uint32_t id, CrtScene *scene, const float l2w[12], const float *l2w_end);
CrtScene *crt_commit(CrtBuilder *b);

void crt_scene_retain(CrtScene *s);
void crt_scene_release(CrtScene *s);
int crt_scene_bounds(const CrtScene *s, float out_min_max[6]);
uint32_t crt_scene_geometry_count(const CrtScene *s);
int crt_scene_has_motion(const CrtScene *s);
size_t crt_scene_primitive_count(const CrtScene *s);
int crt_scene_primitive_breakdown(const CrtScene *s, size_t out[5]);
int crt_scene_unique_primitive_breakdown(const CrtScene *s, size_t out[5]);
int crt_scene_primitive_extents(const CrtScene *s, size_t *count, float *scene_diagonal, float *mean_diagonal,
                                float *max_diagonal);
int crt_scene_image_check(CrtScene *s, uint64_t out[8]);
int crt_scene_engine_select(CrtScene *s, int want_wide, uint32_t out[8]);
int crt_scene_memory_footprint(CrtScene *s, size_t out[6]);
int crt_scene_tree(const CrtScene *s, size_t counts[5], const void **nodes128, const void **leaves16,
                   const void **packets192, const uint32_t **indices);

int crt_intersect1(CrtScene *s, const CrtRay *ray, float t_min, float t_max, CrtRayHit *hit);
int crt_occluded1(CrtScene *s, const CrtRay *ray, float t_min, float t_max);
void crt_thread_release(void);
int crt_intersect_n(CrtScene *s, const CrtRay *d_rays, size_t n, float t_min, float t_max, CrtRayHit *d_hits,
                    void *stream);
int crt_occluded_n(CrtScene *s, const CrtRay *d_rays, size_t n, float t_min, float t_max, uint32_t *d_out,
                   void *stream);
int crt_scene_traversal_error(CrtScene *s, void *stream);
int crt_intersect_n_stats(CrtScene *s, const CrtRay *d_rays, size_t n, float t_min, float t_max, CrtRayHit *d_hits,
                          void *stream, CrtTravStats *host_stats);
int crt_occluded_n_stats(CrtScene *s, const CrtRay *d_rays, size_t n, float t_min, float t_max, uint32_t *d_out,
                         void *stream, CrtTravStats *host_stats);

enum { CRT_MAT_OPENPBR = 0, CRT_MAT_EMISSIVE = 1 };
typedef struct CrtMaterial {
  uint32_t kind;
  uint32_t thin_walled;
  float base_weight; float base_color[3]; float base_diffuse_roughness; float base_metalness;
  float specular_weight; float specular_color[3]; float specular_roughness; float specular_ior;
  float specular_roughness_anisotropy;
  float transmission_weight; float transmission_color[3]; float transmission_depth; float transmission_scatter[3];
  float transmission_scatter_anisotropy; float transmission_dispersion_scale; float transmission_dispersion_abbe_number;
  float subsurface_weight; float subsurface_color[3]; float subsurface_radius; float subsurface_radius_scale[3];
  float subsurface_scatter_anisotropy;
  float fuzz_weight; float fuzz_color[3]; float fuzz_roughness;
  float coat_weight; float coat_color[3]; float coat_roughness; float coat_roughness_anisotropy; float coat_ior;
  float coat_darkening;
  float thin_film_weight; float thin_film_thickness; float thin_film_ior;
  float emission_luminance; float emission_color[3];
  float geometry_opacity;
} CrtMaterial;
void crt_material_default(CrtMaterial *m);

enum { CRT_LIGHT_SPHERE = 0, CRT_LIGHT_RECT = 1, CRT_LIGHT_DISTANT = 2, CRT_LIGHT_DOME = 3 };
typedef struct CrtLight {
  uint32_t kind; uint32_t geom_id;
  float radiance[3];
  float center[3]; float radius;
  float origin[3]; float edge_u[3]; float edge_v[3]; float normal[3];
} CrtLight;

typedef struct CrtCamera {
  float origin[3], lower_left[3], horizontal[3], vertical[3], u[3], v[3];
  float lens_radius;
} CrtCamera;
void crt_camera_new(CrtCamera *c, const float lookfrom[3], const float lookat[3], const float vup[3], float vfov_deg,
                    float aspect, float aperture, float focus_dist);


typedef struct CrtShadeQuery {
  float ray_dir[3]; uint32_t material;
  float p[3]; float t;
  float normal[3]; uint32_t front_face;
  float wi[3]; float cos_theta_o;
  uint32_t sampler_pattern, sampler_index;
  uint32_t _pad[2];
} CrtShadeQuery;
typedef struct CrtScatterSample {
  float origin[3]; uint32_t some;
  float dir[3]; float pdf;
  float value[3]; uint32_t flags;
} CrtScatterSample;
typedef struct CrtBsdfEval { float value[3]; float pdf; uint32_t some; uint32_t _pad[3]; } CrtBsdfEval;
typedef struct CrtLightQuery {
  float from[3]; uint32_t light;
  float u, v; uint32_t _pad[2];
  float point[3]; uint32_t _pad2;
} CrtLightQuery;
typedef struct CrtLightSample {
  float direction[3]; float distance;
  float radiance[3]; float pdf;
  uint32_t some; uint32_t _pad[3];
} CrtLightSample;

int crt_material_scatter_n(const CrtMaterial *d_materials, size_t n_materials, const CrtShadeQuery *d_queries, size_t n,
                           CrtScatterSample *d_out, void *stream);
int crt_material_eval_n(const CrtMaterial *d_materials, size_t n_materials, const CrtShadeQuery *d_queries, size_t n,
                        CrtBsdfEval *d_out, void *stream);
int crt_material_emitted_n(const CrtMaterial *d_materials, size_t n_materials, const CrtShadeQuery *d_queries, size_t n,
                           float *d_rgb, void *stream);
int crt_light_sample_n(const CrtLight *d_lights, size_t n_lights, const CrtLightQuery *d_queries, size_t n,
                       CrtLightSample *d_out, void *stream);
int crt_light_pdf_n(const CrtLight *d_lights, size_t n_lights, const CrtLightQuery *d_queries, size_t n, float *d_pdf,
                    void *stream);
int crt_light_escaped_n(const CrtLight *d_lights, size_t n_lights, const CrtLightQuery *d_queries, size_t n,
                        CrtLightSample *d_out, void *stream);

enum { CRT_STRATEGY_POWER = 0, CRT_STRATEGY_BALANCE = 1, CRT_STRATEGY_LIGHT = 2, CRT_STRATEGY_BSDF = 3 };
enum { CRT_FILTER_BOX = 0, CRT_FILTER_TRIANGLE = 1 };

typedef struct CrtRenderSettings {
  uint32_t width, height;
  uint32_t max_depth;
  int32_t frame;
  int32_t strategy;
  int32_t filter_kind;
  float filter_radius;
  float variance_threshold;
  uint32_t min_spp;
} CrtRenderSettings;

typedef struct CrtRayStats {
  uint64_t camera_rays, closest_hit, shadow_rays, vertices, rr_tested, rr_killed, ended_escaped, ended_depth;
} CrtRayStats;

size_t crt_shard_pixels(uint32_t width, uint32_t height, uint32_t rank, uint32_t world, uint32_t *out);

size_t crt_shard_padded_count(uint32_t width, uint32_t height, uint32_t world);
typedef struct CrtGatherPlan CrtGatherPlan;
CrtGatherPlan *crt_gather_plan_new(uint32_t width, uint32_t height, uint32_t world);
void crt_gather_plan_free(CrtGatherPlan *p);
size_t crt_gather_plan_padded_count(const CrtGatherPlan *p);
int crt_gather_plan_assemble(const CrtGatherPlan *p, const float *d_recv, float *d_frame, void *stream);

typedef struct CrtRenderer CrtRenderer;

CrtRenderer *crt_renderer_new(CrtScene *scene, const CrtMaterial *materials, size_t n_materials,
                              const CrtLight *lights, size_t n_lights, const CrtCamera *camera,
                              const CrtRenderSettings *settings, uint32_t tile_rank, uint32_t tile_world);
void crt_renderer_free(CrtRenderer *r);
size_t crt_renderer_pixel_count(const CrtRenderer *r);
int crt_renderer_pixel_indices(const CrtRenderer *r, uint32_t *out);
int crt_render_samples(CrtRenderer *r, uint32_t sample_begin, uint32_t sample_count, void *stream);
int crt_film_resolve(CrtRenderer *r, float *d_rgb, void *stream);
int crt_film_read(CrtRenderer *r, float *host_rgb);
int crt_film_clear(CrtRenderer *r, void *stream);
size_t crt_renderer_active_pixels(const CrtRenderer *r);
int crt_renderer_sample_counts(CrtRenderer *r, uint32_t *host_out);
int crt_render_stats(CrtRenderer *r, CrtRayStats *out);
int crt_renderer_shade_class_stats(CrtRenderer *r, int enable, uint64_t out_waves[4], uint64_t out_lanes[4]);
int crt_renderer_pipeline(const CrtRenderer *r, uint32_t out[3]);
int crt_renderer_lanes(const CrtRenderer *r);
int crt_renderer_set_lanes(CrtRenderer *r, int lanes);
int crt_renderer_profile(CrtRenderer *r, int enable);
int crt_renderer_profile_read(CrtRenderer *r, double out_ms[4], uint64_t out_launches[4]);
int crt_render_samples_stats(CrtRenderer *r, uint32_t sample_begin, uint32_t sample_count, void *stream,
                             CrtTravStats host_stats[2]);

const char *crt_version(void);
const char *crt_last_error(void);
int crt_device_info(char *name_out, size_t name_cap, int *cu_count, size_t *hbm_bytes);

#ifdef __cplusplus
}
#endif
#endif
```

Measured before the change: 10620 Mray/s.

## Stage BVH leaf records in LDS and recompute ray shear instead of storing it

The traversal kernel now copies BVH leaf records into LDS next to the staged nodes and packets, and reads leaves from LDS when their index falls inside the staged range. Top-level leaves are rotated to the front of the leaf array so the staged window covers them. The per-ray shear values are no longer kept in the LDS ray pool (CRT_LDS_SHEAR=0); they are recomputed from the direction when a packet test starts, freeing two dwords per ray slot for leaves and packets. This trades some extra ALU work per packet phase for fewer global memory loads of leaves, and it may reduce how many packets fit in LDS. A host query, crt_scene_lds_plan, reports the resulting LDS layout.

```diff
diff --git a/crust-render_amd/__init__.py b/crust-render_amd/__init__.py
--- a/crust-render_amd/__init__.py
+++ b/crust-render_amd/__init__.py
@@ -140,7 +140,7 @@
     "crt_film_read", "crt_film_clear", "crt_renderer_active_pixels", "crt_renderer_sample_counts", "crt_render_stats", "crt_renderer_profile", "crt_renderer_profile_read",
     "crt_render_samples_stats", "crt_version", "crt_last_error", "crt_device_info",
     "crt_scene_primitive_extents", "crt_scene_traversal_error", "crt_thread_release", "crt_renderer_shade_class_stats", "crt_renderer_pipeline", "crt_renderer_lanes", "crt_scene_image_check",
-    "crt_scene_engine_select",
+    "crt_scene_engine_select", "crt_scene_lds_plan",
     "crt_material_scatter_n", "crt_material_eval_n", "crt_material_emitted_n", "crt_light_sample_n", "crt_light_pdf_n",
     "crt_light_escaped_n",
     "crt_shard_padded_count", "crt_gather_plan_new", "crt_gather_plan_free", "crt_gather_plan_padded_count",
@@ -195,6 +195,8 @@
         L.crt_scene_image_check.argtypes = [vp, C.POINTER(C.c_uint64)]
     if hasattr(L, "crt_scene_engine_select"):
         L.crt_scene_engine_select.argtypes = [vp, C.c_int, C.POINTER(C.c_uint32)]
+    if hasattr(L, "crt_scene_lds_plan"):
+        L.crt_scene_lds_plan.argtypes = [vp, C.c_int, C.POINTER(C.c_uint32)]
     L.crt_scene_tree.argtypes = [vp, C.POINTER(C.c_size_t), C.POINTER(vp), C.POINTER(vp), C.POINTER(vp),
                                  C.POINTER(up)]
     L.crt_intersect1.argtypes = [vp, C.POINTER(CrtRay), C.c_float, C.c_float, C.POINTER(CrtRayHit)]
@@ -372,6 +374,12 @@
         return dict(zip(("wide", "direct", "lds_stack", "window", "ext_cold", "path_cold", "direct_words", "cold"),
                         map(int, out)))
 
+    def lds_plan(self, want_wide=-1):
+        out = (C.c_uint32 * 8)()
+        _check(lib().crt_scene_lds_plan(self.h, int(want_wide), out), "crt_scene_lds_plan")
+        return dict(zip(("arena_bytes", "pool_bytes", "window", "nodes", "leaves", "packets", "top_leaves", "image_leaves"),
+                        map(int, out)))
+
     def memory_footprint(self):
         out = (C.c_size_t * 6)()
         _check(lib().crt_scene_memory_footprint(self.h, out), "crt_scene_memory_footprint")
diff --git a/crust-render_amd/csrc/capi.cpp b/crust-render_amd/csrc/capi.cpp
--- a/crust-render_amd/csrc/capi.cpp
+++ b/crust-render_amd/csrc/capi.cpp
@@ -241,6 +241,15 @@
     return scene_engine_select(*s->p, want_wide, out);
   } catch (const std::exception &e) {
     set_error_text("crt_scene_engine_select: %s", e.what());
+    return CRT_ERR_BAD_ARG;
+  }
+}
+int crt_scene_lds_plan(CrtScene *s, int want_wide, uint32_t out[8]) {
+  if (!s || !out) return CRT_ERR_BAD_ARG;
+  try {
+    return scene_lds_plan(*s->p, want_wide, out);
+  } catch (const std::exception &e) {
+    set_error_text("crt_scene_lds_plan: %s", e.what());
     return CRT_ERR_BAD_ARG;
   }
 }
diff --git a/crust-render_amd/csrc/crt_internal.h b/crust-render_amd/csrc/crt_internal.h
--- a/crust-render_amd/csrc/crt_internal.h
+++ b/crust-render_amd/csrc/crt_internal.h
@@ -129,6 +129,7 @@
   uint32_t n_packets;
   uint32_t direct_leaves;
   uint32_t cold;
+  uint32_t n_stage_leaves;
 };
 enum : uint32_t { kColdUV = 1u, kColdNormal = 2u, kColdTime = 4u, kColdAll = 7u };
 constexpr uint32_t kNoPackets = 8u;
@@ -220,6 +221,7 @@
   uint32_t cold = 0;
   int inst_order = 1;
   int hot_packets = 1;
+  int lds_leaves = 1;
   int wide = -1;
   int mat_dedup = 1, partition = -1, simple = 1, prefer_stage = -1, cam_compact = 1, shade_wide = -1, fused = -1;
   int noclassify_from = 1 << 30, tail_from = 12, lanes = 4, grid_mult = 0;
@@ -251,6 +253,19 @@
 
 int scene_image_check(const Scene &scene, uint64_t out[8]);
 int scene_engine_select(const Scene &scene, int want_wide, uint32_t out[8]);
+int scene_lds_plan(const Scene &scene, int want_wide, uint32_t out[8]);
+void engine_lds_layout(bool wide, bool deep_tree, bool umask, uint32_t out[5]);
+struct LdsStaged { uint32_t nodes, leaves, packets; };
+constexpr LdsStaged lds_staged(uint32_t n_nodes, uint32_t n_stage_leaves, uint32_t n_packets, uint32_t cap, uint32_t node_dwords,
+                               uint32_t extra, uint32_t node_max) {
+  uint32_t n = n_nodes < cap ? n_nodes : cap;
+  if (n_packets > 0 && n > node_max) n = node_max;
+  uint32_t room = (cap - n) * node_dwords + extra;
+  const uint32_t lf = n_stage_leaves < room / 4u ? n_stage_leaves : room / 4u;
+  room -= lf * 4u;
+  const uint32_t pk = n_packets < room / 48u ? n_packets : room / 48u;
+  return LdsStaged{n, lf, pk};
+}
 
 enum GeomKind { G_MESH, G_SPHERE, G_INSTANCE };
 struct Geom {
diff --git a/crust-render_amd/csrc/kernels/traverse.hip b/crust-render_amd/csrc/kernels/traverse.hip
--- a/crust-render_amd/csrc/kernels/traverse.hip
+++ b/crust-render_amd/csrc/kernels/traverse.hip
@@ -131,6 +131,12 @@
 
 }
 
+void engine_lds_layout(bool wide, bool deep_tree, bool umask, uint32_t out[5]) {
+  const ArenaLayout lay = arena_layout(wide, deep_tree, umask);
+  out[0] = (uint32_t)lay.arena; out[1] = (uint32_t)lay.pools; out[2] = (uint32_t)lay.window;
+  out[3] = (uint32_t)kLdsNodeStride; out[4] = (uint32_t)CRT_LDS_NODE_MAX;
+}
+
 int launch_intersect_n(const DevScene &s, const CrtRay *d_rays, size_t n, float t_min, float t_max, CrtRayHit *d_hits,
                        void *stream, CrtTravStats *d_stats, uint32_t *e) {
   if (n == 0) return CRT_OK;
diff --git a/crust-render_amd/csrc/kernels/traverse.hip.h b/crust-render_amd/csrc/kernels/traverse.hip.h
--- a/crust-render_amd/csrc/kernels/traverse.hip.h
+++ b/crust-render_amd/csrc/kernels/traverse.hip.h
@@ -73,7 +73,15 @@
   float okx, oky, okz;
 };
 
-__device__ __forceinline__ void setup_ray(RayCtx &r, bool with_shear) {
+__device__ __forceinline__ void ray_shear(float dx, float dy, float dz, int kx, int ky, int kz, float &sx, float &sy,
+                                          float &sz) {
+  const float dkz = sel3(dx, dy, dz, kz);
+  sx = sel3(dx, dy, dz, kx) / dkz;
+  sy = sel3(dx, dy, dz, ky) / dkz;
+  sz = 1.0f / dkz;
+}
+
+__device__ __forceinline__ void setup_ray(RayCtx &r, bool with_shear, bool keep_shear = true) {
   const float TINY = 1e-20f, HUGE_ = 1e20f;
   r.ix = absf(r.dx) < TINY ? copysgn(HUGE_, r.dx) : 1.0f / r.dx;
   r.iy = absf(r.dy) < TINY ? copysgn(HUGE_, r.dy) : 1.0f / r.dy;
@@ -89,13 +97,23 @@
     const float dkz = sel3(r.dx, r.dy, r.dz, kz);
     if (dkz < 0.0f) { int t = kx; kx = ky; ky = t; }
     r.kx = kx; r.ky = ky; r.kz = kz;
-    r.sx = sel3(r.dx, r.dy, r.dz, kx) / dkz;
-    r.sy = sel3(r.dx, r.dy, r.dz, ky) / dkz;
-    r.sz = 1.0f / dkz;
+    if (keep_shear) ray_shear(r.dx, r.dy, r.dz, kx, ky, kz, r.sx, r.sy, r.sz);
     r.okx = sel3(r.ox, r.oy, r.oz, kx);
     r.oky = sel3(r.ox, r.oy, r.oz, ky);
     r.okz = sel3(r.ox, r.oy, r.oz, kz);
   }
+}
+
+__device__ __forceinline__ void perm_pack(const RayCtx &r, uint32_t &kz, uint32_t &swap) {
+  kz = (uint32_t)r.kz;
+  const int kx0 = r.kz == 2 ? 0 : r.kz + 1;
+  swap = (r.kx != kx0) ? 1u : 0u;
+}
+__device__ __forceinline__ void perm_unpack(uint32_t kz_bits, uint32_t swap, int &kx, int &ky, int &kz) {
+  kz = (int)kz_bits;
+  kx = kz == 2 ? 0 : kz + 1;
+  ky = kx == 2 ? 0 : kx + 1;
+  if (swap) { const int t = kx; kx = ky; ky = t; }
 }
 
 __device__ __forceinline__ bool tri_scalar(const RayCtx &r, const float *v , float t_min, float t_max,
@@ -193,21 +211,28 @@
 }
 
 constexpr int kLdsPacketDwords = 48;
+constexpr int kLdsLeafDwords = 4;
+static_assert(sizeof(Tri4) == 4 * kLdsPacketDwords && sizeof(Leaf) == 4 * kLdsLeafDwords, "lds_staged's record sizes");
 #ifndef CRT_LDS_NODE_MAX
 #define CRT_LDS_NODE_MAX 1000000
 #endif
-__device__ __forceinline__ uint32_t stage_nodes(const DevScene &S, uint32_t *lds_nodes, int cap, uint32_t &n_pk) {
-  uint32_t n = S.n_nodes < (uint32_t)cap ? S.n_nodes : (uint32_t)cap;
-  if (S.n_packets > 0 && n > (uint32_t)CRT_LDS_NODE_MAX) n = (uint32_t)CRT_LDS_NODE_MAX;
-  const uint32_t room = ((uint32_t)cap - n) * (uint32_t)kLdsNodeStride / (uint32_t)kLdsPacketDwords;
-  n_pk = S.n_packets < room ? S.n_packets : room;
+__device__ __forceinline__ uint32_t stage_nodes(const DevScene &S, uint32_t *lds_nodes, int cap, int extra, uint32_t &n_lf,
+                                                uint32_t &n_pk) {
+  const LdsStaged plan = lds_staged(S.n_nodes, S.n_stage_leaves, S.n_packets, (uint32_t)cap, (uint32_t)kLdsNodeStride,
+                                    (uint32_t)extra, (uint32_t)CRT_LDS_NODE_MAX);
+  const uint32_t n = plan.nodes;
+  n_lf = plan.leaves;
+  n_pk = plan.packets;
   for (uint32_t w = threadIdx.x; w < n * 8u; w += blockDim.x) {
     const uint32_t node = w >> 3, part = w & 7u;
     if (part == 7u) continue;
     const float4 v = reinterpret_cast<const float4 *>(S.nodes + node)[part];
     *reinterpret_cast<float4 *>(lds_nodes + (size_t)node * kLdsNodeStride + part * 4) = v;
   }
-  float4 *pk_dst = reinterpret_cast<float4 *>(lds_nodes + (size_t)n * kLdsNodeStride);
+  float4 *lf_dst = reinterpret_cast<float4 *>(lds_nodes + (size_t)n * kLdsNodeStride);
+  const float4 *lf_src = reinterpret_cast<const float4 *>(S.leaves);
+  for (uint32_t w = threadIdx.x; w < n_lf; w += blockDim.x) lf_dst[w] = lf_src[w];
+  float4 *pk_dst = lf_dst + n_lf;
   const float4 *pk_src = reinterpret_cast<const float4 *>(S.packets);
   for (uint32_t w = threadIdx.x; w < n_pk * 12u; w += blockDim.x) pk_dst[w] = pk_src[w];
   __syncthreads();
diff --git a/crust-render_amd/csrc/kernels/traverse_pool.hip.h b/crust-render_amd/csrc/kernels/traverse_pool.hip.h
--- a/crust-render_amd/csrc/kernels/traverse_pool.hip.h
+++ b/crust-render_amd/csrc/kernels/traverse_pool.hip.h
@@ -60,8 +60,14 @@
 #endif
 constexpr int kStickyMin = CRT_STICKY_MIN;
 
+#ifndef CRT_LDS_SHEAR
+#define CRT_LDS_SHEAR 0
+#endif
+constexpr int kShearDwords = CRT_LDS_SHEAR ? 2 : 0;
 template <int ROWS>
-constexpr int pool_lds_dwords(int stack, bool umask = false) { return (4 + 4 + 2 + (umask ? 4 : 5) + stack) * ROWS * 64; }
+constexpr int pool_lds_dwords(int stack, bool umask = false) { return (4 + 4 + kShearDwords + (umask ? 4 : 5) + stack) * ROWS * 64; }
+template <int ROWS>
+constexpr int pool_lds_budget(int stack, bool umask = false) { return pool_lds_dwords<ROWS>(stack, umask) + (2 - kShearDwords) * ROWS * 64; }
 
 enum : uint32_t { PH_FREE = 0, PH_NODE = 1, PH_PACKET = 2, PH_SCALAR = 3, PH_EXIT = 4, PH_EMIT = 5 };
 
@@ -81,18 +87,20 @@
 __device__ void traverse_pool(const DevScene &S, uint32_t *lds , float t_min,
                               uint32_t umask ,
                               const uint32_t *lds_nodes , uint32_t n_lds,
+                              uint32_t n_lds_lf ,
                               uint32_t n_lds_pk , uint32_t pstack,
                               uint32_t &err, LaneStats &st, Fetch fetch, Emit emit) {
   const int lane = threadIdx.x & 63;
   constexpr int RL = ROWS * 64;
+  const uint32_t *lds_leaves = lds_nodes + (size_t)n_lds * kLdsNodeStride;
   constexpr bool NOPK = (COLD & (int)kNoPackets) != 0;
   float4 *f0 = reinterpret_cast<float4 *>(lds);
   float4 *f1 = reinterpret_cast<float4 *>(lds + 4 * RL);
   float2 *f2 = reinterpret_cast<float2 *>(lds + 8 * RL);
-  uint32_t *w = lds + 10 * RL;
+  uint32_t *w = lds + (8 + kShearDwords) * RL;
   enum { W_CTL = 0, W_CUR, W_AUX, W_CURSOR, W_MASK };
   enum { B_SLOT = 0, B_BU, B_BV, B_BDEFER, B_BGEOM, B_BINST };
-  uint32_t *stk = lds + (UMASK ? 14 : 15) * RL;
+  uint32_t *stk = lds + (8 + kShearDwords + (UMASK ? 4 : 5)) * RL;
   auto at = [&](int row) { return row * 64 + lane; };
   auto W = [&](int plane, int row) -> uint32_t & { return w[plane * RL + row * 64 + lane]; };
   auto STK = [&](int e, int row) -> uint32_t & { return stk[e * RL + row * 64 + lane]; };
@@ -178,20 +186,15 @@
     }
   };
   auto unpack_k = [&](uint32_t c, int &kx, int &ky, int &kz) {
-    kz = (int)((c >> 20) & 3u);
-    kx = kz == 2 ? 0 : kz + 1;
-    ky = kx == 2 ? 0 : kx + 1;
-    if ((c >> 22) & 1u) { const int t = kx; kx = ky; ky = t; }
+    perm_unpack((c >> 20) & 3u, (c >> 22) & 1u, kx, ky, kz);
   };
   auto store_ray = [&](int row, RayCtx &r, bool with_shear, float closest, uint32_t &kz_out, uint32_t &swap_out) {
     r.kx = 0; r.ky = 1; r.kz = 2; r.sx = r.sy = r.sz = 0.0f;
-    setup_ray(r, with_shear);
-    kz_out = (uint32_t)r.kz;
-    const int kx0 = r.kz == 2 ? 0 : r.kz + 1;
-    swap_out = (r.kx != kx0) ? 1u : 0u;
+    setup_ray(r, with_shear, CRT_LDS_SHEAR != 0);
+    perm_pack(r, kz_out, swap_out);
     f0[at(row)] = make_float4(r.ox, r.oy, r.oz, closest);
     f1[at(row)] = make_float4(r.ix, r.iy, r.iz, r.sx);
-    f2[at(row)] = make_float2(r.sy, r.sz);
+    if (CRT_LDS_SHEAR) f2[at(row)] = make_float2(r.sy, r.sz);
   };
 
   auto setup_new = [&](int row, const RayIn &in) -> uint32_t {
@@ -431,14 +434,22 @@
       }
       if (mine) retire();
     } else if (q == PH_PACKET) {
-      const float4 g0 = f0[at(row)], g1 = f1[at(row)];
-      const float2 g2 = f2[at(row)];
+      const float4 g0 = f0[at(row)];
       const uint32_t c = W(W_CTL, row), rmask = UMASK ? umask : W(W_MASK, row);
       uint32_t cur = W(W_CUR, row), k = W(W_CURSOR, row), aux = W(W_AUX, row);
       uint32_t sp = c & 0xffu, lo = c >> 24;
       const uint32_t base = (c >> 8) & 0xffu, level = (c >> 16) & 7u;
       int kx, ky, kz;
       unpack_k(c, kx, ky, kz);
+      float shx = 0.0f, shy = 0.0f, shz = 0.0f;
+      if (!NOPK) {
+        if (CRT_LDS_SHEAR) {
+          const float2 g2 = f2[at(row)];
+          shx = f1[at(row)].w; shy = g2.x; shz = g2.y;
+        } else {
+          ray_shear(rd(side_d, row, 0), rd(side_d, row, 1), rd(side_d, row, 2), kx, ky, kz, shx, shy, shz);
+        }
+      }
       float closest = g0.w;
       float bu = 0.0f, bv = 0.0f;
       uint32_t bdefer = kInvalid;
@@ -449,7 +460,9 @@
         if (act) {
           Leaf lf;
           {
-            uint4 lw = *reinterpret_cast<const uint4 *>(&S.leaves[cur]);
+            uint4 lw;
+            if (cur < n_lds_lf) lw = *reinterpret_cast<const uint4 *>(lds_leaves + (size_t)cur * kLdsLeafDwords);
+            else lw = *reinterpret_cast<const uint4 *>(&S.leaves[cur]);
             asm volatile("" : "+v"(lw.x), "+v"(lw.y), "+v"(lw.z), "+v"(lw.w));
             lf.pkt_first = lw.x; lf.pkt_count = lw.y; lf.idx_first = lw.z; lf.idx_count = lw.w;
           }
@@ -459,7 +472,7 @@
             const uint32_t pki = lf.pkt_first + k;
             const bool pk_lds = pki < n_lds_pk;
             const Tri4 *pk = &S.packets[pki];
-            const Tri4 *pk_l = reinterpret_cast<const Tri4 *>(lds_nodes + (size_t)n_lds * kLdsNodeStride) + (pk_lds ? pki : 0u);
+            const Tri4 *pk_l = reinterpret_cast<const Tri4 *>(lds_leaves + (size_t)n_lds_lf * kLdsLeafDwords) + (pk_lds ? pki : 0u);
             uint4 prim4;
             uint32_t normal_ok, m;
             float4 A_x, A_y, A_z, B_x, B_y, B_z, C_x, C_y, C_z;
@@ -518,7 +531,7 @@
               CRT_PHASE(3)
               RayCtx r;
               r.ox = g0.x; r.oy = g0.y; r.oz = g0.z;
-              r.kx = kx; r.ky = ky; r.kz = kz; r.sx = g1.w; r.sy = g2.x; r.sz = g2.y;
+              r.kx = kx; r.ky = ky; r.kz = kz; r.sx = shx; r.sy = shy; r.sz = shz;
               r.okx = sel3(g0.x, g0.y, g0.z, kx); r.oky = sel3(g0.x, g0.y, g0.z, ky); r.okz = sel3(g0.x, g0.y, g0.z, kz);
               const uint32_t prim_of[4] = {prim4.x, prim4.y, prim4.z, prim4.w};
               const float vax[4] = {A_x.x, A_x.y, A_x.z, A_x.w}, vay[4] = {A_y.x, A_y.y, A_y.z, A_y.w},
@@ -885,8 +898,8 @@
 #endif
 constexpr int kPoolNodes = CRT_POOL_NODES;
 constexpr int kPoolNodesDeep = CRT_POOL_NODES_DEEP;
-constexpr int kEngineLdsFlat = (kBlock / 64) * pool_lds_dwords<CRT_POOL_ROWS>(kPoolStack) + kPoolNodes * kLdsNodeStride;
-constexpr int kEngineLdsDeep = (kBlock / 64) * pool_lds_dwords<CRT_POOL_ROWS>(kPoolStackDeep) + kPoolNodesDeep * kLdsNodeStride;
+constexpr int kEngineLdsFlat = (kBlock / 64) * pool_lds_budget<CRT_POOL_ROWS>(kPoolStack) + kPoolNodes * kLdsNodeStride;
+constexpr int kEngineLdsDeep = (kBlock / 64) * pool_lds_budget<CRT_POOL_ROWS>(kPoolStackDeep) + kPoolNodesDeep * kLdsNodeStride;
 constexpr int kEngineLdsDwords = kEngineLdsFlat > kEngineLdsDeep ? kEngineLdsFlat : kEngineLdsDeep;
 constexpr int kPoolStackWide = CRT_POOL_STACK_WIDE;
 constexpr int kPoolNodesWide = CRT_POOL_NODES_WIDE;
@@ -896,27 +909,35 @@
 __host__ __device__ constexpr int wide_stack(bool deep_tree, bool umask) { return kPoolStackWide + (deep_tree ? 1 : 0) + (umask ? 1 : 0); }
 __host__ __device__ constexpr int wide_nodes(bool deep_tree) { return deep_tree ? CRT_POOL_NODES_WIDE_DEEP : kPoolNodesWide; }
 constexpr int wide_arena(bool deep_tree, bool umask) {
-  return (kBlock / 64) * pool_lds_dwords<CRT_POOL_ROWS>(wide_stack(deep_tree, umask), umask) + wide_nodes(deep_tree) * kLdsNodeStride;
+  return (kBlock / 64) * pool_lds_budget<CRT_POOL_ROWS>(wide_stack(deep_tree, umask), umask) + wide_nodes(deep_tree) * kLdsNodeStride;
 }
 constexpr int imax(int a, int b) { return a > b ? a : b; }
 constexpr int kEngineLdsWide = imax(imax(wide_arena(false, false), wide_arena(false, true)), imax(wide_arena(true, false), wide_arena(true, true)));
 static_assert(kEngineLdsWide * 4 + 512 <= 40 * 1024, "four workgroups of the wide split per CU");
+struct ArenaLayout { int arena, pools, window, stack; };
+constexpr ArenaLayout arena_layout(bool wide, bool deep_tree, bool umask) {
+  const int stack = wide ? wide_stack(deep_tree, umask) : (deep_tree ? kPoolStackDeep : kPoolStack);
+  return ArenaLayout{wide ? kEngineLdsWide : kEngineLdsDwords, (kBlock / 64) * pool_lds_dwords<CRT_POOL_ROWS>(stack, umask),
+                     wide ? wide_nodes(deep_tree) : (deep_tree ? kPoolNodesDeep : kPoolNodes), stack};
+}
+static_assert(arena_layout(false, false, false).pools + kPoolNodes * kLdsNodeStride <= kEngineLdsDwords &&
+              arena_layout(false, true, false).pools + kPoolNodesDeep * kLdsNodeStride <= kEngineLdsDwords, "pools + window fit the arena");
 template <bool ANY, bool STATS, int WIDE, int COLD = (int)kColdAll, bool UMASK = false, class Fetch, class Emit>
 __device__ __forceinline__ void run_traversal(const DevScene &S, uint32_t *lds, float t_min, uint32_t &err, LaneStats &st,
                                               Fetch fetch, Emit emit, uint32_t umask = 0u) {
   const bool deep_tree = S.pool_stack >= (uint32_t)kPoolStackDeep;
-  const uint32_t pstack = WIDE ? (uint32_t)wide_stack(deep_tree, UMASK)
-                               : (deep_tree ? (uint32_t)kPoolStackDeep : (uint32_t)kPoolStack);
-  const int pnodes = WIDE ? wide_nodes(deep_tree) : (deep_tree ? kPoolNodesDeep : kPoolNodes);
-  const int wave_dwords = pool_lds_dwords<CRT_POOL_ROWS>((int)pstack, UMASK);
-  uint32_t *lds_nodes = lds + (kBlock / 64) * wave_dwords;
-  uint32_t n_lds_pk;
-  const uint32_t n_lds = stage_nodes(S, lds_nodes, pnodes, n_lds_pk);
+  const ArenaLayout lay = deep_tree ? arena_layout(WIDE != 0, true, UMASK) : arena_layout(WIDE != 0, false, UMASK);
+  const uint32_t pstack = (uint32_t)lay.stack;
+  const int wave_dwords = lay.pools / (kBlock / 64);
+  uint32_t *lds_nodes = lds + lay.pools;
+  uint32_t n_lds_lf, n_lds_pk;
+  const uint32_t n_lds = stage_nodes(S, lds_nodes, lay.window, lay.arena - lay.pools - lay.window * kLdsNodeStride, n_lds_lf,
+                                     n_lds_pk);
   uint32_t *wave_lds = lds + (threadIdx.x >> 6) * wave_dwords;
 #ifndef CRT_WIDE_LEAN
 #define CRT_WIDE_LEAN 1
 #endif
-#define CRT_ENGINE(D) traverse_pool<ANY, STATS, CRT_POOL_ROWS, D, (WIDE && CRT_WIDE_LEAN != 0), COLD, UMASK>(S, wave_lds, t_min, umask, lds_nodes, n_lds, n_lds_pk, pstack, err, st, fetch, emit)
+#define CRT_ENGINE(D) traverse_pool<ANY, STATS, CRT_POOL_ROWS, D, (WIDE && CRT_WIDE_LEAN != 0), COLD, UMASK>(S, wave_lds, t_min, umask, lds_nodes, n_lds, n_lds_lf, n_lds_pk, pstack, err, st, fetch, emit)
   if ((COLD & (int)kNoPackets) != 0 || WIDE == 2) CRT_ENGINE(true);
   else if (CRT_DIRECT_LEAVES != 0 && !WIDE && S.direct_leaves != 0) CRT_ENGINE(true);
   else CRT_ENGINE(false);
diff --git a/crust-render_amd/csrc/scene.cpp b/crust-render_amd/csrc/scene.cpp
--- a/crust-render_amd/csrc/scene.cpp
+++ b/crust-render_amd/csrc/scene.cpp
@@ -174,6 +174,7 @@
   if (num("CRT_COLD", v)) k.cold = (uint32_t)v & kColdAll;
   if (num("CRT_INST_ORDER", v)) k.inst_order = v != 0;
   if (num("CRT_HOT_PACKETS", v)) k.hot_packets = v != 0;
+  if (num("CRT_LDS_LEAVES", v)) k.lds_leaves = v != 0;
   if (num("CRT_WIDE", v)) k.wide = v == 2 ? 2 : (v != 0);
   if (num("CRT_MAT_DEDUP", v)) k.mat_dedup = v != 0;
   if (num("CRT_PARTITION", v)) k.partition = v != 0;
@@ -315,6 +316,8 @@
   std::vector<uint32_t> leaf_of_word;
   uint32_t n_staged_roots = 0;
   uint32_t n_top_packets = 0;
+  uint32_t n_top_leaves = 0;
+  bool stage_leaves = true;
   uint32_t cold = kColdAll;
 };
 
@@ -329,6 +332,18 @@
   Flat &f = im.f;
   im.me = place(f, scene);
   Flat::Placed &me = im.me;
+  {
+    const size_t n_top = scene.bvh.leaves.size(), n_all = f.leaves.size();
+    im.n_top_leaves = uint32_t(n_top);
+    im.stage_leaves = read_knobs().lds_leaves != 0;
+    if (n_top && n_top < n_all) {
+      std::rotate(f.leaves.begin(), f.leaves.end() - n_top, f.leaves.end());
+      for (WideNode &n : f.nodes)
+        for (int l = 0; l < 4; l++)
+          if ((n.flags & (1u << l)) && (n.flags & (1u << (4 + l))))
+            n.child[l] = n.child[l] >= n_all - n_top ? uint32_t(n.child[l] - (n_all - n_top)) : uint32_t(n.child[l] + n_top);
+    }
+  }
   {
     const size_t n_top = scene.bvh.packets.size(), n_all = f.packets.size();
     im.n_top_packets = uint32_t(n_top);
@@ -573,7 +588,38 @@
   v.direct_leaves = im.direct ? 1u : 0u;
   v.pool_stack = im.pool_stack;
   v.cold = im.cold;
-}
+  v.n_stage_leaves = im.stage_leaves ? uint32_t(im.f.leaves.size()) : 0u;
+}
+}
+
+int scene_lds_plan(const Scene &scene, int want_wide, uint32_t out[8]) {
+  FlatImage im;
+  int rc = flatten_image(scene, im);
+  if (rc != CRT_OK) return rc;
+  DevScene v{};
+  fill_view_fields(im, v);
+  EngineSelect e;
+  const bool renderer = want_wide <= -3;
+  rc = want_wide <= -2 && want_wide != -4 ? select_engine_env(v, e, renderer) : select_engine(v, want_wide == -4 ? -1 : want_wide, e, renderer);
+  if (rc != CRT_OK) {
+    set_error_text("select_engine: the %s kernels cannot decode this image (direct child words: %s)",
+                   want_wide > 0 ? "four-wave" : "three-wave", v.direct_leaves ? "yes" : "no");
+    return rc;
+  }
+  uint32_t lay[5];
+  engine_lds_layout(e.wide, v.pool_stack >= (uint32_t)CRT_POOL_STACK_DEEP, e.wide && renderer, lay);
+  if (lay[1] + lay[2] * lay[3] > lay[0]) {
+    set_error_text("lds plan: ray pools (%u dwords) and node window (%u x %u) exceed the arena (%u)", lay[1], lay[2], lay[3], lay[0]);
+    return CRT_ERR_BAD_ARG;
+  }
+  const LdsStaged st = lds_staged(v.n_nodes, v.n_stage_leaves, v.n_packets, lay[2], lay[3], lay[0] - lay[1] - lay[2] * lay[3], lay[4]);
+  if (lay[1] + st.nodes * lay[3] + st.leaves * 4u + st.packets * 48u > lay[0]) {
+    set_error_text("lds plan: %u nodes, %u leaves and %u packets do not fit the arena (%u dwords)", st.nodes, st.leaves, st.packets, lay[0]);
+    return CRT_ERR_BAD_ARG;
+  }
+  out[0] = lay[0] * 4u; out[1] = lay[1] * 4u; out[2] = lay[2]; out[3] = st.nodes;
+  out[4] = st.leaves; out[5] = st.packets; out[6] = im.n_top_leaves; out[7] = uint32_t(im.f.leaves.size());
+  return CRT_OK;
 }
 
 int scene_engine_select(const Scene &scene, int want_wide, uint32_t out[8]) {
diff --git a/include/crt.h b/include/crt.h
--- a/include/crt.h
+++ b/include/crt.h
@@ -80,6 +80,7 @@
                                 float *max_diagonal);
 int crt_scene_image_check(CrtScene *s, uint64_t out[8]);
 int crt_scene_engine_select(CrtScene *s, int want_wide, uint32_t out[8]);
+int crt_scene_lds_plan(CrtScene *s, int want_wide, uint32_t out[8]);
 int crt_scene_memory_footprint(CrtScene *s, size_t out[6]);
 int crt_scene_tree(const CrtScene *s, size_t counts[5], const void **nodes128, const void **leaves16,
                    const void **packets192, const uint32_t **indices);
diff --git a/profiles/pmc_l1.py b/profiles/pmc_l1.py
--- /dev/null
+++ b/profiles/pmc_l1.py
@@ -0,0 +1,68 @@
+#!/usr/bin/env python3
+import collections, csv, glob, json, re, sys
+
+d, tag = sys.argv[1], sys.argv[2]
+pref = sys.argv[3] if len(sys.argv) > 3 else "k_extend<false"
+CUS, XCDS = 256, 8
+
+
+def launches(i):
+    out = collections.OrderedDict()
+    for f in sorted(glob.glob("%s/l1_%s_%d/*/*_counter_collection.csv" % (d, tag, i))):
+        for r in csv.DictReader(open(f)):
+            m = re.search(r"(k_\w+)(<[^>]*>)?", r["Kernel_Name"])
+            if not m:
+                continue
+            e = out.setdefault(int(r["Dispatch_Id"]), {"kernel": m.group(1) + (m.group(2) or ""),
+                                                       "ns": int(r["End_Timestamp"]) - int(r["Start_Timestamp"])})
+            e[r["Counter_Name"]] = e.get(r["Counter_Name"], 0.0) + float(r["Counter_Value"])
+    return list(out.values())
+
+
+def steps(i):
+    out = []
+    for e in launches(i):
+        if e["kernel"].startswith("k_generate"):
+            out.append([])
+        elif e["kernel"].startswith(pref) and out:
+            out[-1].append(e)
+    return out
+
+
+bench = json.loads(open("%s/l1_%s_1.log" % (d, tag)).read().strip().splitlines()[-1])
+n_steps = bench["steps"]
+rs = bench.get("ray_stats") or bench["detail"]["ray_stats"] if "ray_stats" in bench or "detail" in bench else None
+if rs is None:
+    rs = next(v["ray_stats"] for v in bench.values() if isinstance(v, dict) and "ray_stats" in v)
+cam = rs["camera_rays"] / n_steps
+rays = {"camera": cam, "bounce": rs["closest_hit"] / n_steps - cam}
+P = [steps(1), steps(2), steps(3)]
+res = {}
+for part in ("camera", "bounce"):
+    tot = collections.Counter()
+    for i, st in enumerate(P):
+        for launches_of_step in st[-n_steps:]:
+            sel = launches_of_step[:1] if part == "camera" else launches_of_step[1:]
+            for e in sel:
+                for k, v in e.items():
+                    if k != "kernel":
+                        tot[k if k != "ns" else "ns%d" % i] += v
+    n = rays[part] * n_steps
+    cyc = tot["GRBM_GUI_ACTIVE"]
+    clk = cyc / XCDS / tot["ns2"]
+    cu = lambda key, ns: tot[key] / (tot[ns] * clk * CUS)
+    res[part] = {
+        "rays_per_step": int(rays[part]), "ms_per_step": round(tot["ns0"] / 1e6 / n_steps, 2), "clock_ghz": round(clk, 3),
+        "tag_lookups_per_ray": round(tot["TCP_TOTAL_CACHE_ACCESSES_sum"] / n, 2),
+        "lane_accesses_per_ray": round(tot["TCP_TOTAL_ACCESSES_sum"] / n, 2),
+        "vmem_rd_wave_insts_per_ray": round(tot["SQ_INSTS_VMEM_RD"] / n, 3),
+        "l1_lookups_per_cycle_cu": round(cu("TCP_TOTAL_CACHE_ACCESSES_sum", "ns0"), 3),
+        "tcp_core_busy": round(cu("TCP_GATE_EN2_sum", "ns0"), 3),
+        "tcp_pending_stall": round(cu("TCP_PENDING_STALL_CYCLES_sum", "ns1"), 3),
+        "tcp_ta_data_stall": round(cu("TCP_TCP_TA_DATA_STALL_CYCLES_sum", "ns1"), 3),
+        "tcp_tagconflict_stall": round(cu("TCP_READ_TAGCONFLICT_STALL_CYCLES_sum", "ns1"), 3),
+        "ta_busy": round(cu("TA_TA_BUSY_sum", "ns2"), 3),
+        "ta_addr_stalled_by_tc": round(cu("TA_ADDR_STALLED_BY_TC_CYCLES_sum", "ns2"), 3),
+        "state_reads_per_ray": round(tot["TCP_TA_TCP_STATE_READ_sum"] / n, 3),
+    }
+print(json.dumps({"tag": tag, "kernel": pref, "steps": n_steps, **res}, indent=1))
```

Result: faster. 10730 Mray/s (median of 6 runs) (+1.0%).
